# pvangoor/eqvio

Measured on AMD Instinct MI355X. Metric: EqF vision updates/sec @ N=200 landmarks, higher is better.
Workload: dtype f64; 1 GPU; synthetic 'hover' world, 200 tracked landmarks (state dim 621, 400 measurement rows), InvDepth chart, fast Riccati, IMU 200 Hz / camera 20 Hz (10 observer steps per frame), EuRoC pinhole intrinsics, one independent filter per GPU (replicas); landmarks=200, state_dim=621, parallelism=replicas x1

## Files before the change

eqvio_amd/capi.py:

```python
import ctypes as C
import os

import numpy as np

_HERE = os.path.dirname(os.path.abspath(__file__))
LIB_DIR = os.environ.get("EQVIO_AMD_LIB_DIR") or os.path.join(_HERE, "lib")

COORD_EUCLIDEAN, COORD_INVDEPTH, COORD_NORMAL = 0, 1, 2
OPT_RICCATI_DENSE, OPT_CHECK_FINITE, OPT_SIGMA_FP32, OPT_DOORBELL, OPT_SPECULATIVE, OPT_EARLY_LIFT, OPT_TRACE, OPT_FUSED_ASSEMBLY, OPT_LOOKAHEAD, OPT_LA_TIMEOUT_US, OPT_Z_IN_LOOKAHEAD, OPT_LA_SPLIT_ROWS, OPT_MEASURE_IN_PROPAGATE, OPT_LIFT_WITH_SYRK, OPT_LA_HOME, OPT_TILES_PER_WORKGROUP, OPT_GATHER_IN_PROPAGATE, OPT_HOLD_NEW_LANDMARKS, OPT_SELECT_ONE_WORKGROUP, OPT_LIVE_COLUMNS_FIRST, OPT_EARLY_DOORBELL, OPT_QUIET_DOOR_WAIT, OPT_TIMING = 1, 2, 3, 6, 7, 8, 9, 11, 12, 15, 17, 18, 19, 20, 21, 22, 23, 24, 25, 26, 27, 29, 100

c_double_p = C.POINTER(C.c_double)
c_int_p = C.POINTER(C.c_int)


class Camera(C.Structure):

    _fields_ = [
        ("model", C.c_int),
        ("width", C.c_int),
        ("height", C.c_int),
        ("fx", C.c_double),
        ("fy", C.c_double),
        ("cx", C.c_double),
        ("cy", C.c_double),
        ("dist", C.c_double * 5),
    ]

    @staticmethod
    def pinhole(fx, fy, cx, cy, width, height):
        cam = Camera()
        cam.model, cam.width, cam.height = 0, int(width), int(height)
        cam.fx, cam.fy, cam.cx, cam.cy = fx, fy, cx, cy
        return cam

    @staticmethod
    def radtan(fx, fy, cx, cy, width, height, k1, k2, p1, p2, k3=0.0):
        cam = Camera.pinhole(fx, fy, cx, cy, width, height)
        cam.model = 1
        cam.dist[:] = [k1, k2, p1, p2, k3]
        return cam

    @staticmethod
    def equidistant(fx, fy, cx, cy, width, height, k1, k2, k3, k4):
        cam = Camera.pinhole(fx, fy, cx, cy, width, height)
        cam.model = 2
        cam.dist[:] = [k1, k2, k3, k4, 0.0]
        return cam

    def project(self, p):
        out = np.zeros(2)
        _load_sim_protos().eqvio_camera_project(C.byref(self), _dp(_f64(p)), _dp(out))
        return out

    def undistort(self, y):
        out = np.zeros(3)
        _load_sim_protos().eqvio_camera_undistort(C.byref(self), _dp(_f64(y)), _dp(out))
        return out

    def jacobian(self, p):
        out = np.zeros(6)
        _load_sim_protos().eqvio_camera_jacobian(C.byref(self), _dp(_f64(p)), _dp(out))
        return out.reshape(2, 3)


_SETTINGS_DOUBLES = [
    "biasOmegaProcessVariance", "biasAccelProcessVariance", "attitudeProcessVariance", "positionProcessVariance",
    "velocityProcessVariance", "cameraAttitudeProcessVariance", "cameraPositionProcessVariance", "pointProcessVariance",
    "velGyrNoise", "velAccNoise", "velGyrBiasWalk", "velAccBiasWalk",
    "measurementNoise", "outlierThresholdAbs", "outlierThresholdProb", "featureRetention",
    "initialAttitudeVariance", "initialPositionVariance", "initialVelocityVariance", "initialCameraAttitudeVariance",
    "initialCameraPositionVariance", "initialPointVariance", "initialPointDepthVariance", "initialBiasOmegaVariance",
    "initialBiasAccelVariance", "initialSceneDepth",
]
_SETTINGS_INTS = [
    "useDiscreteInnovationLift", "useDiscreteVelocityLift", "useDiscreteStateMatrix", "fastRiccati", "useMedianDepth",
    "useFeaturePredictions", "useEquivariantOutput", "removeLostLandmarks", "coordinateChoice",
]


class Settings(C.Structure):

    _fields_ = [(n, C.c_double) for n in _SETTINGS_DOUBLES] + [(n, C.c_int) for n in _SETTINGS_INTS] + [("cameraOffset", C.c_double * 7)]

    @staticmethod
    def defaults():
        s = Settings()
        vals = dict(
            biasOmegaProcessVariance=0.001, biasAccelProcessVariance=0.001, attitudeProcessVariance=0.001, positionProcessVariance=0.001,
            velocityProcessVariance=0.001, cameraAttitudeProcessVariance=0.001, cameraPositionProcessVariance=0.001, pointProcessVariance=0.001,
            velGyrNoise=1e-4, velAccNoise=1e-3, velGyrBiasWalk=1e-5, velAccBiasWalk=1e-3,
            measurementNoise=2.0, outlierThresholdAbs=1e8, outlierThresholdProb=1e8, featureRetention=0.3,
            initialAttitudeVariance=1e-4, initialPositionVariance=1e-4, initialVelocityVariance=1e-2, initialCameraAttitudeVariance=1e-5,
            initialCameraPositionVariance=1e-4, initialPointVariance=1.0, initialPointDepthVariance=-1.0, initialBiasOmegaVariance=0.1,
            initialBiasAccelVariance=0.1, initialSceneDepth=1.0,
            useDiscreteInnovationLift=1, useDiscreteVelocityLift=1, useDiscreteStateMatrix=0, fastRiccati=0, useMedianDepth=1,
            useFeaturePredictions=0, useEquivariantOutput=1, removeLostLandmarks=1, coordinateChoice=COORD_EUCLIDEAN,
        )
        for k, v in vals.items():
            setattr(s, k, v)
        s.cameraOffset[:] = [1, 0, 0, 0, 0, 0, 0]
        return s

    def state_gain_diag8(self):
        return np.array([self.biasOmegaProcessVariance, self.biasAccelProcessVariance, self.attitudeProcessVariance, self.positionProcessVariance,
                         self.velocityProcessVariance, self.cameraAttitudeProcessVariance, self.cameraPositionProcessVariance, self.pointProcessVariance])

    def input_gain_diag12(self):
        v = [self.velGyrNoise**2, self.velAccNoise**2, self.velGyrBiasWalk**2, self.velAccBiasWalk**2]
        return np.repeat(np.array(v), 3)

    def initial_cov_diag(self, N):
        v = [self.initialBiasOmegaVariance, self.initialBiasAccelVariance, self.initialAttitudeVariance, self.initialPositionVariance,
             self.initialVelocityVariance, self.initialCameraAttitudeVariance, self.initialCameraPositionVariance]
        d = np.concatenate([np.repeat(np.array(v), 3), np.full(3 * N, self.initialPointVariance)])
        if self.initialPointDepthVariance > 0:
            d[21 + 2::3] = self.initialPointDepthVariance
        return d


def _dp(a):
    return a.ctypes.data_as(c_double_p)


def _ip(a):
    return a.ctypes.data_as(c_int_p)


def _f64(a):
    return np.ascontiguousarray(a, dtype=np.float64)


def _i32(a):
    return np.ascontiguousarray(a, dtype=np.int32)


class EqfError(RuntimeError):
    def __init__(self, code, msg):
        super().__init__(f"eqf_hip error {code}: {msg}")
        self.code = code


_lib = None


def load_eqf_lib():
    global _lib
    if _lib is not None:
        return _lib
    path = os.path.join(LIB_DIR, "libeqf_hip.so")
    if not os.path.exists(path):
        raise RuntimeError(f"{path} not found: run `python -c 'import __graft_entry__ as g; g.build()'` — the EqF path has no CPU fallback")
    lib = C.CDLL(path)
    vp = C.c_void_p
    P = C.POINTER
    protos = {
        "eqf_error_string": (C.c_char_p, [C.c_int]),
        "eqf_kernel_name": (C.c_char_p, [C.c_int]),
        "eqf_create": (C.c_int, [P(vp), C.c_int, C.c_int, C.c_int]),
        "eqf_destroy": (None, [vp]),
        "eqf_set_option": (C.c_int, [vp, C.c_int, C.c_int]),
        "eqf_get_option": (C.c_int, [vp, C.c_int, C.POINTER(C.c_int)]),
        "eqf_lookahead_selftest": (C.c_int, [vp]),
        "eqf_lookahead_home": (C.c_int, [vp, C.POINTER(C.c_int), C.POINTER(C.c_long)]),
        "eqf_device_to_itself": (C.c_int, [vp]),
        "eqf_early_doorbell_stats": (C.c_int, [vp, C.POINTER(C.c_long), C.c_int]),
        "eqf_synchronize": (C.c_int, [vp]),
        "eqf_num_landmarks": (C.c_int, [vp]),
        "eqf_get_ids": (C.c_int, [vp, c_int_p, C.c_int]),
        "eqf_stream": (vp, [vp]),
        "eqf_set_state": (C.c_int, [vp, c_double_p, c_double_p, c_int_p, c_double_p, c_double_p, C.c_int]),
        "eqf_get_state": (C.c_int, [vp, c_double_p, c_double_p, c_int_p, c_double_p, c_double_p, C.c_int]),
        "eqf_set_sigma": (C.c_int, [vp, c_double_p, C.c_int]),
        "eqf_set_sigma_diag": (C.c_int, [vp, c_double_p, C.c_int]),
        "eqf_get_sigma": (C.c_int, [vp, c_double_p, C.c_int]),
        "eqf_get_sigma_block": (C.c_int, [vp, C.c_int, C.c_int, C.c_int, C.c_int, c_double_p]),
        "eqf_state_estimate": (C.c_int, [vp, c_double_p, c_int_p, c_double_p, C.c_int]),
        "eqf_add_landmarks": (C.c_int, [vp, c_int_p, c_double_p, C.c_int, C.c_double]),
        "eqf_remove_landmarks": (C.c_int, [vp, c_int_p, C.c_int]),
        "eqf_remove_unmeasured_landmarks": (C.c_int, [vp, c_int_p, C.c_int, c_int_p, c_int_p]),
        "eqf_find_unknown_ids": (C.c_int, [vp, c_int_p, C.c_int, c_int_p, c_int_p]),
        "eqf_same_as_mapped": (C.c_int, [vp, c_int_p, C.c_int]),
        "eqf_update_unsettled": (C.c_int, [vp]),
        "eqf_remove_invalid_at_update": (C.c_int, [vp]),
        "eqf_add_landmarks_held": (C.c_int, [vp, c_int_p, c_double_p, C.c_int, C.c_double]),
        "eqf_hold_supported": (C.c_int, [vp]),
        "eqf_hold_stats": (C.c_int, [vp, C.POINTER(C.c_long), C.c_int]),
        "eqf_live_columns_stats": (C.c_int, [vp, C.POINTER(C.c_long), C.c_int]),
        "eqf_own_hardware_queue": (C.c_int, [vp]),
        "eqf_remove_invalid_landmarks": (C.c_int, [vp]),
        "eqf_integrate_riccati_fast": (C.c_int, [vp, c_double_p, C.c_double, c_double_p, c_double_p]),
        "eqf_integrate_riccati_accurate": (C.c_int, [vp, c_double_p, C.c_double, c_double_p, c_double_p]),
        "eqf_integrate_riccati_discrete": (C.c_int, [vp, c_double_p, C.c_double, c_double_p, c_double_p]),
        "eqf_integrate_observer": (C.c_int, [vp, c_double_p, c_double_p, C.c_int, C.c_int]),
        "eqf_outlier_stats": (C.c_int, [vp, P(Camera), c_int_p, c_double_p, C.c_int, c_double_p, c_double_p, c_double_p]),
        "eqf_propagate_fast": (C.c_int, [vp, c_double_p, C.c_double, c_double_p, c_double_p, c_double_p, c_double_p, C.c_int, C.c_int]),
        "eqf_stage_measurement": (C.c_int, [vp, c_int_p, c_double_p, C.c_int]),
        "eqf_trace_read": (C.c_int, [vp, C.POINTER(C.c_ulonglong), C.POINTER(C.c_longlong), C.POINTER(C.c_uint)]),
        "eqf_host_wait_stats": (C.c_int, [vp, C.POINTER(C.c_long), c_double_p, C.c_int]),
        "eqf_stats_then_update": (C.c_int, [vp, C.POINTER(Camera), c_int_p, c_double_p, C.c_int, C.c_double, C.c_double, C.c_double, C.c_int, C.c_int, c_double_p, c_double_p,
                                  c_double_p, c_int_p]),
        "eqf_stats_select_update": (C.c_int, [vp, C.POINTER(Camera), c_int_p, c_double_p, C.c_int, C.c_double, C.c_double, C.c_int, C.c_double, C.c_int, C.c_int, c_double_p,
                                    c_double_p, c_double_p, c_int_p, c_int_p, c_int_p]),
        "eqf_vision_update": (C.c_int, [vp, P(Camera), c_int_p, c_double_p, C.c_int, C.c_double, C.c_int, C.c_int]),
        "eqf_last_gamma": (C.c_int, [vp, c_double_p, C.c_int]),
        "eqf_compute_nees": (C.c_int, [vp, c_double_p, c_int_p, c_double_p, C.c_int, c_double_p]),
        "eqf_nees_lu_fallbacks": (C.c_int, [vp, C.POINTER(C.c_long)]),
        "eqf_speculation_stats": (C.c_int, [vp, C.POINTER(C.c_long), C.POINTER(C.c_long), C.POINTER(C.c_long), C.c_int]),
        "eqf_measure_in_propagate_stats": (C.c_int, [vp, C.POINTER(C.c_long), C.c_int]),
        "eqf_z_in_lookahead_stats": (C.c_int, [vp, C.POINTER(C.c_long), C.c_int]),
        "eqf_gather_stats": (C.c_int, [vp, C.POINTER(C.c_long), C.c_int]),
        "eqf_selection_stats": (C.c_int, [vp, C.POINTER(C.c_long), C.POINTER(C.c_long), C.c_int]),
        "eqf_output_cov_all": (C.c_int, [vp, P(Camera), c_double_p]),
        "eqf_lookahead_stats": (C.c_int, [vp, C.POINTER(C.c_long), C.POINTER(C.c_long), C.c_int]),
        "eqf_debug_matrices_AB": (C.c_int, [vp, c_double_p, c_double_p, c_double_p]),
        "eqf_debug_get_W": (C.c_int, [vp, c_double_p, C.c_int, C.c_int]),
        "eqf_debug_syrk_order": (C.c_int, [C.c_int, c_int_p]),
        "eqf_debug_lookahead_stamps": (C.c_int, [vp, C.POINTER(C.c_ulonglong)]),
        "eqf_debug_matrix_C": (C.c_int, [vp, P(Camera), c_int_p, c_double_p, C.c_int, C.c_int, c_double_p, c_double_p]),
        "eqf_mfma_f64_peak": (C.c_int, [vp, c_double_p]),
        "eqf_mfma_f64_peak_clock": (C.c_int, [vp, C.POINTER(C.c_double), C.POINTER(C.c_double)]),
        "eqf_last_kernel_times": (C.c_int, [vp, c_int_p, P(C.c_float), C.c_int]),
    }
    for name, (res, args) in protos.items():
        if os.environ.get("EQVIO_AMD_LIB_DIR") and name in ("eqf_lookahead_home", "eqf_device_to_itself", "eqf_early_doorbell_stats", "eqf_update_unsettled", "eqf_remove_invalid_at_update", "eqf_gather_stats", "eqf_remove_unmeasured_landmarks", "eqf_find_unknown_ids", "eqf_add_landmarks_held", "eqf_hold_supported", "eqf_hold_stats", "eqf_same_as_mapped", "eqf_live_columns_stats", "eqf_own_hardware_queue") and not hasattr(lib, name):
            continue
        fn = getattr(lib, name)
        fn.restype = res
        fn.argtypes = args
    lib._declared = sorted(protos)
    _lib = lib
    return lib


class EqfCore:

    def __init__(self, max_landmarks, coordinate_choice=COORD_EUCLIDEAN, device=0):
        self.lib = load_eqf_lib()
        self.h = C.c_void_p()
        self._chk0(self.lib.eqf_create(C.byref(self.h), device, max_landmarks, coordinate_choice))
        self._cap0 = max_landmarks + 16

    def _chk0(self, rc):
        if rc != 0:
            raise EqfError(rc, self.lib.eqf_error_string(rc).decode())

    def close(self):
        if self.h:
            self.lib.eqf_destroy(self.h)
            self.h = C.c_void_p()

    def __del__(self):
        try:
            self.close()
        except Exception:
            pass

    @property
    def N(self):
        return self.lib.eqf_num_landmarks(self.h)

    @property
    def n(self):
        return 21 + 3 * self.N

    @property
    def cap(self):
        return max(self._cap0, self.N + 16)

    def set_option(self, opt, val):
        self._chk0(self.lib.eqf_set_option(self.h, opt, val))

    def get_option(self, opt):
        v = C.c_int()
        self._chk0(self.lib.eqf_get_option(self.h, opt, C.byref(v)))
        return v.value

    def lookahead_selftest(self):
        return self.lib.eqf_lookahead_selftest(self.h)

    def synchronize(self):
        self._chk0(self.lib.eqf_synchronize(self.h))

    def stream(self):
        return self.lib.eqf_stream(self.h)

    def set_state(self, xi0_sensor, X_sensor, ids, q0, Q):
        xi0_sensor, X_sensor, ids, q0, Q = _f64(xi0_sensor), _f64(X_sensor), _i32(ids), _f64(q0), _f64(Q)
        self._chk0(self.lib.eqf_set_state(self.h, _dp(xi0_sensor), _dp(X_sensor), _ip(ids), _dp(q0), _dp(Q), len(ids)))

    def get_state(self):
        xi0, Xs = np.zeros(23), np.zeros(23)
        ids, q0, Q = np.zeros(self.cap, np.int32), np.zeros(3 * self.cap), np.zeros(5 * self.cap)
        N = self.lib.eqf_get_state(self.h, _dp(xi0), _dp(Xs), _ip(ids), _dp(q0), _dp(Q), self.cap)
        if N < 0:
            self._chk0(N)
        return xi0, Xs, ids[:N].copy(), q0[: 3 * N].reshape(N, 3).copy(), Q[: 5 * N].reshape(N, 5).copy()

    def set_sigma(self, S):
        S = np.asfortranarray(S, dtype=np.float64)
        self._chk0(self.lib.eqf_set_sigma(self.h, S.ctypes.data_as(c_double_p), S.shape[0]))

    def set_sigma_diag(self, d):
        d = _f64(d)
        self._chk0(self.lib.eqf_set_sigma_diag(self.h, _dp(d), len(d)))

    def get_sigma(self):
        n = self.n
        out = np.zeros((n, n), order="F")
        self._chk0(self.lib.eqf_get_sigma(self.h, out.ctypes.data_as(c_double_p), n))
        return out

    def get_sigma_block(self, r0, c0, rows, cols):
        out = np.zeros((rows, cols), order="F")
        self._chk0(self.lib.eqf_get_sigma_block(self.h, r0, c0, rows, cols, out.ctypes.data_as(c_double_p)))
        return out

    def state_estimate(self):
        s = np.zeros(23)
        ids, p = np.zeros(self.cap, np.int32), np.zeros(3 * self.cap)
        N = self.lib.eqf_state_estimate(self.h, _dp(s), _ip(ids), _dp(p), self.cap)
        if N < 0:
            self._chk0(N)
        return s, ids[:N].copy(), p[: 3 * N].reshape(N, 3).copy()

    def add_landmarks(self, ids, p, var):
        ids, p = _i32(ids), _f64(p)
        self._chk0(self.lib.eqf_add_landmarks(self.h, _ip(ids), _dp(p), len(ids), var))

    def add_landmarks_held(self, ids, p, var):
        ids, p = _i32(ids), _f64(p)
        rc = self.lib.eqf_add_landmarks_held(self.h, _ip(ids), _dp(p), len(ids), var)
        if rc == -6:
            return False
        self._chk0(rc)
        return True

    def remove_landmarks(self, indices):
        indices = _i32(indices)
        self._chk0(self.lib.eqf_remove_landmarks(self.h, _ip(indices), len(indices)))

    def remove_invalid_landmarks(self):
        rc = self.lib.eqf_remove_invalid_landmarks(self.h)
        if rc < 0:
            self._chk0(rc)
        return rc

    def integrate_riccati_fast(self, imu13, dt, Qdiag12, Pdiag8):
        imu13, Qd, Pd = _f64(imu13), _f64(Qdiag12), _f64(Pdiag8)
        self._chk0(self.lib.eqf_integrate_riccati_fast(self.h, _dp(imu13), dt, _dp(Qd), _dp(Pd)))

    def integrate_riccati_accurate(self, imu13, dt, Qdiag12, Pdiag8):
        imu13, Qd, Pd = _f64(imu13), _f64(Qdiag12), _f64(Pdiag8)
        self._chk0(self.lib.eqf_integrate_riccati_accurate(self.h, _dp(imu13), dt, _dp(Qd), _dp(Pd)))

    def integrate_riccati_discrete(self, imu13, dt, Qdiag12, Pdiag8):
        imu13, Qdiag12, Pdiag8 = _f64(imu13), _f64(Qdiag12), _f64(Pdiag8)
        self._chk0(self.lib.eqf_integrate_riccati_discrete(self.h, _dp(imu13), dt, _dp(Qdiag12), _dp(Pdiag8)))

    def integrate_observer(self, imu13_k, dt_k, discrete=True):
        imu13_k, dt_k = _f64(imu13_k).reshape(-1, 13), _f64(dt_k).reshape(-1)
        self._chk0(self.lib.eqf_integrate_observer(self.h, _dp(imu13_k), _dp(dt_k), len(dt_k), int(discrete)))

    def outlier_stats(self, cam, ids, y):
        ids, y = _i32(ids), _f64(y)
        N = self.N
        a, p, d = np.zeros(N), np.zeros(N), np.zeros(N)
        self._chk0(self.lib.eqf_outlier_stats(self.h, C.byref(cam), _ip(ids), _dp(y), len(ids), _dp(a), _dp(p), _dp(d)))
        return a, p, d

    def output_cov_all(self, cam):
        out = np.zeros(4 * self.N)
        self._chk0(self.lib.eqf_output_cov_all(self.h, C.byref(cam), _dp(out)))
        return out.reshape(self.N, 2, 2)

    def vision_update(self, cam, ids, y, meas_var, use_equivariant=True, discrete=False):
        ids, y = _i32(ids), _f64(y)
        self._chk0(self.lib.eqf_vision_update(self.h, C.byref(cam), _ip(ids), _dp(y), len(ids), meas_var, int(use_equivariant), int(discrete)))
# ... 402 lines not shown
```

eqvio_amd/csrc/eqf_hip.hip:

```cpp
#include "eqf_hip.h"
#include "eqf_kernels.hpp"
#include "eqf_lookahead.hpp"
#include "eqf_batch.hpp"
#include "eqf_batch.h"
#include "host_prof.hpp"
#include <algorithm>
#include <atomic>
#include <chrono>
#include <condition_variable>
#include <mutex>
#include <cstdio>
#include <cstdlib>
#include <cstring>
#include <string>
#include <vector>
#include <unistd.h>
#include <fcntl.h>
#include <signal.h>
#include <sys/mman.h>
#include <cerrno>

using namespace eqf;

namespace {
// ... 5 lines not shown
    KN_PROP_MAIN,
    KN_MEASURE,
    KN_STATS,
    KN_BUILD_Z,
    KN_CHOL_PANEL,
    KN_CHOL_UPDATE,
    KN_GAMMA,
    KN_SYRK,
    KN_LIFT,
    KN_DENSE_GEMM,
    KN_MISC,
    KN_CHOL_LOOKAHEAD,
    KN_COUNT
};
const char* kNames[KN_COUNT] = {"k_assemble_AB", "k_observer",    "k_propagate_G", "k_propagate_main", "k_measure", "k_outlier_stats", "k_build_Z",
                                "k_chol_step",   "k_chol_first", "k_gamma",       "k_syrk_sub",       "k_lift",    "k_gemm_nt",       "misc", "k_chol_lookahead"};

int roundup(int x, int m) { return (x + m - 1) / m * m; }
int pick_ld(int x) {
    int ld = roundup(x, 16);
    if (ld % 128 == 0)
        ld += 16;
    return ld;
}

struct SensorState {
    V3 bgyr, bacc;
    Pose pose;
    V3 vel;
    Pose cam;
};
struct GroupSensor {
    V3 bgyr, bacc;
    Pose A;
    V3 w;
    Pose B;
};
SensorState unpack_sensor(const double* s) {
    SensorState r;
    r.bgyr = v3(s[0], s[1], s[2]);
    r.bacc = v3(s[3], s[4], s[5]);
    r.pose = Pose{Qt{s[6], s[7], s[8], s[9]}, v3(s[10], s[11], s[12])};
    r.vel = v3(s[13], s[14], s[15]);
    r.cam = Pose{Qt{s[16], s[17], s[18], s[19]}, v3(s[20], s[21], s[22])};
    return r;
}
void pack_pose(const Pose& p, double* q, double* x) {
    q[0] = p.R.w;
    q[1] = p.R.x;
    q[2] = p.R.y;
    q[3] = p.R.z;
    x[0] = p.x.x;
    x[1] = p.x.y;
    x[2] = p.x.z;
}
void pack_v3(V3 v, double* d) {
    d[0] = v.x;
    d[1] = v.y;
    d[2] = v.z;
}
void pack_sensor(const SensorState& r, double* s) {
    pack_v3(r.bgyr, s);
    pack_v3(r.bacc, s + 3);
    pack_pose(r.pose, s + 6, s + 10);
    pack_v3(r.vel, s + 13);
    pack_pose(r.cam, s + 16, s + 20);
}
GroupSensor unpack_group(const double* s) {
    GroupSensor g;
    g.bgyr = v3(s[0], s[1], s[2]);
    g.bacc = v3(s[3], s[4], s[5]);
    g.A = Pose{Qt{s[6], s[7], s[8], s[9]}, v3(s[10], s[11], s[12])};
    g.w = v3(s[13], s[14], s[15]);
    g.B = Pose{Qt{s[16], s[17], s[18], s[19]}, v3(s[20], s[21], s[22])};
    return g;
}
void pack_group(const GroupSensor& g, double* s) {
    pack_v3(g.bgyr, s);
    pack_v3(g.bacc, s + 3);
    pack_pose(g.A, s + 6, s + 10);
    pack_v3(g.w, s + 13);
    pack_pose(g.B, s + 16, s + 20);
}
SensorState sensor_action(const GroupSensor& X, const SensorState& s) {
    SensorState r;
    r.bgyr = s.bgyr + X.bgyr;
    r.bacc = s.bacc + X.bacc;
    r.pose = pose_mul(s.pose, X.A);
    r.vel = q_rot(q_inv(X.A.R), s.vel - X.w);
    r.cam = pose_mul(pose_mul(pose_inv(X.A), s.cam), X.B);
    return r;
}
GroupSensor group_mul(const GroupSensor& a, const GroupSensor& b) {
    GroupSensor r;
    r.bgyr = a.bgyr + b.bgyr;
    r.bacc = a.bacc + b.bacc;
    r.A = pose_mul(a.A, b.A);
    r.B = pose_mul(a.B, b.B);
    r.w = a.w + q_rot(a.A.R, b.w);
    return r;
}

}

struct eqf_ctx {
    int device = 0;
    hipStream_t stream = nullptr;
    hipStream_t stream2 = nullptr;
    hipEvent_t ev_assembled = nullptr, ev_observer = nullptr, ev_early = nullptr;
    bool ev_assembled_early = false;
    bool obs_pending = false;
    bool busy_common = false, busy_steps = false, busy_meas = false;
    int chart = 0;
    int Ncap = 0, ncap = 0, ld = 0;
    int mcap = 0, ldz = 0;
    int N = 0;
    std::vector<int> ids;
    SensorState xi0;
    GroupSensor X;
    double* d_st[2] = {nullptr, nullptr};
    double* d_lm[2] = {nullptr, nullptr};
    int stcur = 0, lmcur = 0;
    double* d_sigma[2] = {nullptr, nullptr};
    int cur = 0;
    double *d_Al = nullptr, *d_Bl = nullptr;
    Common* d_common = nullptr;
    ObsStep* d_steps = nullptr;
    double *d_C = nullptr, *d_ytil = nullptr, *d_y = nullptr;
    int *d_lmidx = nullptr, *d_measof = nullptr;
    double *d_Ebuf = nullptr, *d_Yl = nullptr, *d_Fl = nullptr, *d_PhiB = nullptr;
    int* d_expinfo = nullptr;
    double *d_Zn = nullptr, *d_Wn = nullptr;
    double* d_pub = nullptr;
    int* d_pubf = nullptr;
    int* d_pubfl = nullptr;
    int la_home = 0;
    long la_home_refused = 0;
    int opt_la_home = 1;
    long la_home_launches = 0;
    bool la_home_force = false;
    int reg_slot = -1;
    unsigned reg_checks = 0;
    char* d_puby = nullptr;
    int la_njcap = 0, la_seq = 0;
    unsigned long long* d_ladbg = nullptr;
    int opt_lookahead = 1;
    int opt_zb = 1;
    int opt_zb_large = 1;
    int opt_la_split = 1;
    int opt_prop_tpw = 1;
    int opt_gather = 1;
    int opt_early_door = 1;
    int opt_quiet_wait = 1;
    int opt_la_watch_ahead = 1;
    int early_seq_next = 0, early_armed_seq = 0;
    bool early_allowed = false;
    long early_rings = 0;
    bool unsettled = false, unsettled_wait = false;
    int settle_seq = 0, settle_N = 0;
    unsigned settle_gen = 0, settle_epoch = 0, est_epoch = 0;
    std::vector<int> settle_ids;
    std::vector<int> invalid_ids;
    int opt_hold = 1;
    int opt_sel_one = 1;
    int opt_live_first = 1;
    const int* la_live_cols = nullptr;
    long live_first_launches = 0;
    int n_held = 0;
    double held_var = 0.0;
    bool held_in_memory = false;
    double* h_held = nullptr;
    bool held_busy = false;
    long held_launches = 0;
    long gather_launches = 0;
    int opt_measure_prop = 1;
    int opt_lift_syrk = 1;
    bool pred_valid = false, me_valid = false;
    Cam pred_cam{}, me_cam{};
    int pred_star = 0, me_star = 0, me_M = 0;
    unsigned long me_gen = 0;
    long me_used = 0;
    bool obs_one_chunk = false;
    bool tail_zb = false;
    double tail_var = 0.0;
    long zb_launches = 0;
    int cu_count = 256;
    long la_book_timeouts = 0;
    std::vector<char> rm_drop;
    std::vector<int> rm_ids, rm_map;
    std::vector<double> rm_est;
    bool own_queue = false;
    bool counted_alive = false;
    int la_cus_held = 0;
    int la_selftest = 0;
    long long la_timeout_ticks = LA_TIMEOUT_TICKS;
    long la_launches = 0, la_fallbacks = 0;
    int la_consecutive_stalls = 0;
    int tail_M = 0;
    bool tail_la = false;
    int* d_perm = nullptr;
    static constexpr int kRing = 8;
    int ring_pos = 0;
    int ring_inflight = 0;
    bool reshape_pending = false;
    int dev_N = 0;
    std::vector<int> pend_map;
    std::vector<double> pend_p;
    std::vector<double> pend_var;
    char* h_rs_ring = nullptr;
    char* d_rs = nullptr;
    size_t rs_bytes = 0;
    int spec_backoff = 0, spec_backoff_len = 0;
    long spec_calls = 0, spec_queued = 0, spec_cancelled = 0;
    long nees_lu_fallbacks = 0;
    int ldzn = 0;
    double *d_Z = nullptr, *d_W = nullptr, *d_Linv = nullptr, *d_gamma = nullptr, *d_gpart = nullptr, *d_est = nullptr, *d_stats = nullptr, *d_scratch = nullptr, *d_F = nullptr, *d_tmp = nullptr;
    int* d_flags = nullptr;
    int* d_syrk_order = nullptr;
    std::vector<int> syrk_off;
    Common* h_common = nullptr;
    ObsStep* h_steps = nullptr;
    double* h_buf = nullptr;
    bool ocov_valid = false;
    Cam ocov_cam{};
    bool ocov_hint_valid = false;
    Cam ocov_hint{};
    size_t hbuf_doubles = 0;
    int* h_ibuf = nullptr;
    int* h_flags = nullptr;
    int* h_lmidx = nullptr;
    double* h_y = nullptr;
    double* h_ylm = nullptr;
    double* d_meas = nullptr;
    int* d_meas_idx = nullptr;
    bool stage_requested = false, stage_pending = false, staged_valid = false;
    int staged_M = 0;
    unsigned lm_gen = 0, staged_gen = 0;
    std::vector<int> staged_ids;
    std::vector<double> staged_y;
    std::vector<int> map_ids;
    unsigned map_gen = ~0u;
    int map_N = -1;
    bool map_all = false;
    bool map_ident = false;
    bool tail_ident = false;
    std::vector<std::pair<int, int>> lookup;
    std::vector<int> renum_scratch;
    unsigned lookup_gen = ~0u;
    trace_t* d_trace = nullptr;
    unsigned trace_frame = 0;
    std::vector<long long> h_trace;
    long wait_calls = 0, launch_calls = 0;
    double wait_seconds = 0.0, launch_seconds = 0.0;
    double* h_res = nullptr;
    double* h_ocov = nullptr;
    int* h_resflags = nullptr;
    int* h_sel = nullptr;
    long sel_frames = 0, sel_discarded = 0;
    static constexpr int kMaxSteps = kObsChunk;
    CommonK ck;
    int opt_dense = 0, opt_check = 0, opt_timing = 0, opt_f32 = 0, opt_early = 1, opt_fuse_asm = 1;
    bool sig32 = false;
    int opt_door = 1;
    int* d_door = nullptr;
    int* h_door = nullptr;
    unsigned door_seq = 0;
    int opt_spec = 1;
    int* d_spec = nullptr;
    std::vector<double> last_gamma;
    int n_at_update = 0;
    bool gamma_stale = false;
    std::vector<double> est_cache;
    bool est_valid = false;
    bool meas_valid = false;
    int meas_star = 0;
    std::vector<int> meas_ids;
    std::vector<std::pair<int, std::pair<hipEvent_t, hipEvent_t>>> tev;
    std::vector<int> tev_n;
    std::vector<hipEvent_t> evpool;
    size_t evused = 0;

    double* q0() { return d_st[stcur]; }
    double* Qq() { return d_lm[lmcur]; }
    double* Qa() { return d_lm[lmcur] + 4 * (size_t)Ncap; }
    double* sigma() { return d_sigma[cur]; }
    int n() const { return 21 + 3 * N; }
};

#define HIPCHK(expr)                                                                                   \
    do {                                                                                               \
        hipError_t _e = (expr);                                                                        \
        if (_e != hipSuccess) {                                                                        \
            std::fprintf(stderr, "[eqf_hip] %s failed: %s (%s:%d)\n", #expr, hipGetErrorString(_e), __FILE__, __LINE__); \
            return (int)_e;                                                                            \
        }                                                                                              \
    } while (0)

namespace {

hipEvent_t get_event(eqf_ctx* c) {
    if (c->evused == c->evpool.size()) {
        hipEvent_t e;
        hipEventCreate(&e);
        c->evpool.push_back(e);
    }
    return c->evpool[c->evused++];
}
constexpr int TR_FRAMES = 1024, TR_SLOTS = 48;
enum { TR_ASSEMBLE = 0, TR_PROPAGATE = 1, TR_BUILD_Z = 2, TR_STEP0 = 3, TR_LIFT = 40, TR_SYRK = 42 };
constexpr int TR_HOST = 8;
enum { TH_DOOR = 0, TH_PROP_ENTRY = 1, TH_ASSEMBLE_OUT = 2, TH_PROP_OUT = 3, TH_TAIL_ENTRY = 4, TH_BUILD_Z_OUT = 5, TH_TAIL_OUT = 6 };
void host_stamp(eqf_ctx* c, int k) {
    if (c->d_trace)
        c->h_trace[(size_t)(c->trace_frame % TR_FRAMES) * TR_HOST + k] = std::chrono::duration_cast<std::chrono::nanoseconds>(std::chrono::steady_clock::now().time_since_epoch()).count();
}
trace_t* trace_slot(eqf_ctx* c, int slot) { return c->d_trace ? c->d_trace + (size_t)(c->trace_frame % TR_FRAMES) * TR_SLOTS + slot : nullptr; }
struct KTimer {
    eqf_ctx* c;
    int which;
    hipEvent_t e0 = nullptr, e1 = nullptr;
    std::chrono::steady_clock::time_point h0;
    int nlaunch;
    bool on() const { return c->opt_timing == 1 || (c->opt_timing == 2 && (which == KN_CHOL_LOOKAHEAD || which == KN_CHOL_PANEL || which == KN_CHOL_UPDATE)); }
    KTimer(eqf_ctx* ctx, int w, int n = 1) : c(ctx), which(w), h0(std::chrono::steady_clock::now()), nlaunch(n) {
        if (on()) {
            e0 = get_event(c);
            e1 = get_event(c);
            hipEventRecord(e0, c->stream);
        }
    }
    ~KTimer() {
        if (on()) {
            hipEventRecord(e1, c->stream);
            c->tev.push_back({which, {e0, e1}});
            c->tev_n.push_back(nlaunch);
        }
        c->launch_calls += nlaunch - 1;
        ++c->launch_calls;
        c->launch_seconds += std::chrono::duration<double>(std::chrono::steady_clock::now() - h0).count();
    }
};
void timing_reset(eqf_ctx* c) {
    c->tev.clear();
    c->tev_n.clear();
    c->evused = 0;
}

int blocks(int n, int b) { return (n + b - 1) / b; }

int spin_stream(hipStream_t st) {
    for (;;) {
        const hipError_t e = hipStreamQuery(st);
        if (e == hipSuccess)
            return 0;
        if (e != hipErrorNotReady) {
            std::fprintf(stderr, "[eqf_hip] stream error: %s\n", hipGetErrorString(e));
            return (int)e;
        }
    }
}
namespace {
std::atomic<int> ctx_alive[64];
thread_local bool replaces_own_queue = false;
std::mutex la_gate_mutex;
std::condition_variable la_gate_cv;
int la_cus_booked[64] = {0};
}
namespace {
constexpr int REG_SLOTS = 64;
struct DeviceRegistry {
    std::atomic<int> pid[REG_SLOTS];
};
DeviceRegistry* registry_of(int device) {
    static std::mutex mu;
    static DeviceRegistry* maps[64] = {};
    std::lock_guard<std::mutex> g(mu);
    DeviceRegistry*& r = maps[device & 63];
    if (r)
        return r;
    char name[96];
    std::snprintf(name, sizeof(name), "/eqf_hip_contexts_u%u_d%d", (unsigned)getuid(), device);
    const int fd = shm_open(name, O_CREAT | O_RDWR, 0600);
    if (fd < 0)
        return nullptr;
    if (ftruncate(fd, sizeof(DeviceRegistry)) != 0) {
        close(fd);
        return nullptr;
    }
    void* p = mmap(nullptr, sizeof(DeviceRegistry), PROT_READ | PROT_WRITE, MAP_SHARED, fd, 0);
    close(fd);
    if (p == MAP_FAILED)
        return nullptr;
    r = static_cast<DeviceRegistry*>(p);
    return r;
}
bool pid_alive(int pid) { return pid > 0 && (kill(pid, 0) == 0 || errno == EPERM); }
}
static void registry_enter(eqf_ctx* c) {
    DeviceRegistry* r = registry_of(c->device);
    c->reg_slot = -1;
    if (!r)
        return;
    const int me = (int)getpid();
    for (int pass = 0; pass < 2 && c->reg_slot < 0; ++pass)
        for (int i = 0; i < REG_SLOTS && c->reg_slot < 0; ++i) {
            int cur = r->pid[i].load(std::memory_order_relaxed);
            if (cur != 0 && (pass == 0 || pid_alive(cur)))
                continue;
            if (r->pid[i].compare_exchange_strong(cur, me))
                c->reg_slot = i;
        }
}
static void registry_leave(eqf_ctx* c) {
    DeviceRegistry* r = c->reg_slot >= 0 ? registry_of(c->device) : nullptr;
    if (r)
        r->pid[c->reg_slot].store(0, std::memory_order_relaxed);
    c->reg_slot = -1;
}
static bool device_to_itself(eqf_ctx* c) {
    DeviceRegistry* r = c->reg_slot >= 0 ? registry_of(c->device) : nullptr;
    if (!r)
        return false;
    int others = 0;
    for (int i = 0; i < REG_SLOTS; ++i)
        others += (i != c->reg_slot && r->pid[i].load(std::memory_order_relaxed) != 0) ? 1 : 0;
    if (others == 0)
        return true;
    if ((++c->reg_checks & 0xfff) == 1) {
        for (int i = 0; i < REG_SLOTS; ++i) {
            int cur = r->pid[i].load(std::memory_order_relaxed);
            if (i != c->reg_slot && cur != 0 && cur != (int)getpid() && !pid_alive(cur))
                r->pid[i].compare_exchange_strong(cur, 0);
        }
    }
    return false;
}
static void la_release(eqf_ctx* c) {
    if (!c->la_cus_held)
        return;
    {
        std::lock_guard<std::mutex> g(la_gate_mutex);
        la_cus_booked[c->device & 63] -= c->la_cus_held;
    }
    c->la_cus_held = 0;
    la_gate_cv.notify_all();
}
static bool la_book(eqf_ctx* c, int workgroups) {
    la_release(c);
    std::unique_lock<std::mutex> g(la_gate_mutex);
    int& booked = la_cus_booked[c->device & 63];
    const auto bound = std::chrono::microseconds(std::max<long>(2000, 2 * (long)(c->la_timeout_ticks / 100)));
    if (!la_gate_cv.wait_for(g, bound, [&] { return booked == 0 || booked + workgroups <= c->cu_count; }))
        return false;
    booked += workgroups;
    c->la_cus_held = workgroups;
    return true;
}
struct LaBookingGuard {
    eqf_ctx* c;
    bool keep = false;
    ~LaBookingGuard() {
        if (!keep)
            la_release(c);
    }
};
int sync_ctx(eqf_ctx* c) {
    {
        int r = spin_stream(c->stream);
        if (r)
            return r;
    }
    if (c->obs_pending) {
        int r = spin_stream(c->stream2);
        if (r)
            return r;
        c->obs_pending = false;
    }
    c->busy_common = c->busy_steps = c->busy_meas = false;
    c->ring_inflight = 0;
    c->held_busy = false;
    la_release(c);
    return 0;
}
int door_wait(eqf_ctx* c, int which, int seq, bool* early = nullptr) {
    HP_SCOPE("abi.door_wait");
    volatile int* bell = reinterpret_cast<volatile int*>(c->h_door) + which;
    long spins_after_done = 0;
    const auto t0 = std::chrono::steady_clock::now();
    constexpr auto kQuietWait = std::chrono::milliseconds(2);
    volatile int* bell_early = (which == 1 && early && c->early_armed_seq == seq) ? reinterpret_cast<volatile int*>(c->h_door) + 3 : nullptr;
    if (early)
        *early = false;
    for (long it = 1;; ++it) {
        const bool rang_early = bell_early && *bell_early == seq && *bell != seq;
        if (rang_early)
            *early = true;
        if (*bell == seq || rang_early) {
            std::atomic_thread_fence(std::memory_order_acquire);
            c->busy_common = c->busy_steps = c->busy_meas = false;
            c->ring_inflight = 0;
            c->held_busy = false;
            if (!(which == 1 && c->unsettled_wait))
                ++c->wait_calls;
            c->wait_seconds += std::chrono::duration<double>(std::chrono::steady_clock::now() - t0).count();
            if (which == 1) {
                if (!c->unsettled_wait)
                    host_stamp(c, TH_DOOR);
                la_release(c);
            }
            return 0;
        }
        if (spins_after_done || ((it & 0xfff) == 0 && (!c->opt_quiet_wait || std::chrono::steady_clock::now() - t0 >= kQuietWait))) {
            const hipError_t e = hipStreamQuery(c->stream);
            if (e == hipSuccess) {
                if (++spins_after_done > 1000000) {
                    std::fprintf(stderr, "[eqf_hip] doorbell %d never rang (expected %d, have %d)\n", which, seq, (int)*bell);
                    la_release(c);
                    return (int)hipErrorUnknown;
                }
            } else if (e != hipErrorNotReady) {
                std::fprintf(stderr, "[eqf_hip] stream error: %s\n", hipGetErrorString(e));
                la_release(c);
                return (int)e;
            }
        }
    }
}
int join_observer(eqf_ctx* c) {
    c->ev_assembled_early = false;
    if (c->obs_pending) {
        HIPCHK(hipStreamWaitEvent(c->stream, c->ev_observer, 0));
        c->obs_pending = false;
    }
    return 0;
}

Cam make_cam(const eqvio_camera* c) {
    Cam k{c->fx, c->fy, c->cx, c->cy};
    k.model = c->model;
    for (int i = 0; i < 5; ++i)
        k.d[i] = c->dist[i];
    return k;
}
bool camera_ok(const eqvio_camera* c) { return c->model >= EQVIO_CAMERA_PINHOLE && c->model <= EQVIO_CAMERA_EQUIDISTANT; }

void compute_common_at(const GroupSensor& X, const SensorState& xi0, const double* imu13, Common& cm, CommonK& ck) {
    const SensorState xh = sensor_action(X, xi0);
    const V3 gyr = v3(imu13[1], imu13[2], imu13[3]) - xh.bgyr;
    const V6 U_I{gyr, xh.vel};
    const M3 R_A = q_mat(X.A.R);
    const M3 R_IC = q_mat(xh.cam.R);
    const M3 RTic = transpose(R_IC);
    auto put = [](const M3& A, double* d) {
        const double a[9] = {A.a00, A.a01, A.a02, A.a10, A.a11, A.a12, A.a20, A.a21, A.a22};
        std::memcpy(d, a, sizeof(a));
    };
    put(RTic * transpose(R_A), cm.Mv);
    put(RTic, cm.RTic);
    put(RTic * skew(xh.cam.x), cm.RTicSx);
    const V6 U1 = Ad_apply(pose_inv(xi0.cam), Ad_apply(X.A, U_I));
    const M6 adT = se3_adjoint(U1);
    const M6 CT = m6_mul(se3_Adjoint(pose_inv(X.B)), adT);
    std::memcpy(cm.CT, CT.a, sizeof(cm.CT));
    const V6 U_C = Ad_apply(pose_inv(xh.cam), U_I);
    pack_v3(U_C.v, cm.vC);
    std::memset(cm.Bs, 0, sizeof(cm.Bs));
    auto setB = [&](int r0, int c0, const M3& A) {
        const double a[9] = {A.a00, A.a01, A.a02, A.a10, A.a11, A.a12, A.a20, A.a21, A.a22};
        for (int i = 0; i < 3; ++i)
            for (int j = 0; j < 3; ++j)
                cm.Bs[(r0 + i) * 12 + c0 + j] = a[3 * i + j];
    };
    for (int i = 0; i < 6; ++i)
        cm.Bs[i * 12 + 6 + i] = 1.0;
    setB(6, 0, R_A);
    setB(9, 0, skew(X.A.x) * R_A);
    setB(12, 0, R_A * skew(xh.vel));
    setB(12, 3, R_A);
    std::memset(cm.Ass, 0, sizeof(cm.Ass));
    for (int r = 0; r < 21; ++r)
        for (int cc = 0; cc < 6; ++cc)
            cm.Ass[r * 21 + cc] = -cm.Bs[r * 12 + cc];
    for (int i = 0; i < 3; ++i)
        cm.Ass[(9 + i) * 21 + 12 + i] = 1.0;
    const V3 gdir = q_rot(q_inv(xi0.pose.R), v3(0, 0, 1));
    const M3 Gs = (-kGravity) * skew(gdir);
    const double g[9] = {Gs.a00, Gs.a01, Gs.a02, Gs.a10, Gs.a11, Gs.a12, Gs.a20, Gs.a21, Gs.a22};
    for (int i = 0; i < 3; ++i)
        for (int j = 0; j < 3; ++j)
            cm.Ass[(12 + i) * 21 + 6 + j] = g[3 * i + j];
    for (int i = 0; i < 6; ++i)
        for (int j = 0; j < 6; ++j)
            cm.Ass[(15 + i) * 21 + 15 + j] = adT.a[i * 6 + j];
    std::memcpy(ck.lm, cm.Mv, sizeof(double) * 66);
    put(R_A, ck.RA);
    put(skew(X.A.x) * R_A, ck.SxRA);
    put(R_A * skew(xh.vel), ck.RAsv);
    std::memcpy(ck.G, g, sizeof(g));
    std::memcpy(ck.adT, adT.a, sizeof(ck.adT));
}

void compute_common(const eqf_ctx* c, const double* imu13, Common& cm) { compute_common_at(c->X, c->xi0, imu13, cm, const_cast<eqf_ctx*>(c)->ck); }

int upload_common(eqf_ctx* c, const double* imu13) {
    compute_common(c, imu13, *c->h_common);
    return 0;
}
int launch_assemble(eqf_ctx* c, bool record_early = true) {
    KTimer t(c, KN_ASSEMBLE);
    int r = join_observer(c);
    if (r)
        return r;
    hipLaunchKernelGGL(k_assemble_AB, dim3(std::max(1, blocks(c->N, 64))), dim3(64), 0, c->stream, c->ck, c->N, c->Ncap, c->chart, c->d_common, c->q0(), c->Qq(),
                       c->Qa(), c->d_Al, c->d_Bl, trace_slot(c, TR_ASSEMBLE));
    if (record_early) {
        HIPCHK(hipEventRecord(c->ev_early, c->stream));
        c->ev_assembled_early = true;
    }
    return (int)hipGetLastError();
}
int keep_last_gamma(eqf_ctx* c) {
    if (!c->gamma_stale)
        return 0;
    const int ng = c->n_at_update;
    HIPCHK(hipMemcpyAsync(c->h_buf, c->d_gamma, sizeof(double) * ng, hipMemcpyDeviceToHost, c->stream));
    { int _r = sync_ctx(c); if (_r) return _r; }
    c->last_gamma.assign(c->h_buf, c->h_buf + ng);
    c->gamma_stale = false;
    return 0;
}
int read_flags(eqf_ctx* c) {
    HIPCHK(hipMemcpyAsync(c->h_flags, c->d_flags, 4 * sizeof(int), hipMemcpyDeviceToHost, c->stream));
    { int _r = sync_ctx(c); if (_r) return _r; }
    return 0;
}
void ensure_lookup(eqf_ctx* c) {
    if (c->lookup_gen != c->lm_gen || (int)c->lookup.size() != c->N) {
        c->lookup.resize(c->N);
        for (int i = 0; i < c->N; ++i)
            c->lookup[i] = {c->ids[i], i};
        std::sort(c->lookup.begin(), c->lookup.end());
        c->lookup_gen = c->lm_gen;
    }
}
int index_of(eqf_ctx* c, int id) {
    ensure_lookup(c);
    const auto it = std::lower_bound(c->lookup.begin(), c->lookup.end(), std::make_pair(id, -1));
    return (it != c->lookup.end() && it->first == id) ? it->second : -1;
}
// ... 258 lines not shown
            ctx_alive[c->device & 63].fetch_sub(1);
        c->counted_alive = false;
    }
    if (c && std::getenv("EQF_DEBUG_STATS"))
        std::fprintf(stderr, "[eqf_hip] look-ahead launches %ld (stalled %ld), of them with Z built inside %ld\n", c->la_launches, c->la_fallbacks, c->zb_launches);
    if (c && std::getenv("EQF_DEBUG_STATS") && c->early_rings)
        std::fprintf(stderr, "[eqf_hip] updates taken from the early doorbell: %ld\n", c->early_rings);
    if (!c)
        return;
    hipSetDevice(c->device);
    if (c->stream)
        hipStreamSynchronize(c->stream);
    if (c->stream2)
        hipStreamSynchronize(c->stream2);
    for (int b = 0; b < 2; ++b) {
        hipFree(c->d_sigma[b]);
        hipFree(c->d_lm[b]);
        hipFree(c->d_st[b]);
    }
    hipFree(c->d_Al);
    hipFree(c->d_Bl);
    hipFree(c->d_common);
    hipFree(c->d_steps);
    hipFree(c->d_C);
    hipFree(c->d_ytil);
    hipFree(c->d_y);
    hipFree(c->d_lmidx);
    hipFree(c->d_measof);
    hipFree(c->d_Z);
    hipFree(c->d_W);
    hipFree(c->d_Linv);
    hipFree(c->d_gamma);
    hipFree(c->d_gpart);
    hipFree(c->d_pub);
    hipFree(c->d_pubf);
    hipFree(c->d_pubfl);
    hipFree(c->d_puby);
    if (c->d_ladbg)
        hipFree(c->d_ladbg);
    if (c->d_trace)
        hipFree(c->d_trace);
    hipFree(c->d_est);
    hipFree(c->d_stats);
    hipFree(c->d_scratch);
    hipFree(c->d_flags);
    hipFree(c->d_syrk_order);
    if (c->d_Ebuf) {
        hipFree(c->d_Ebuf);
        hipFree(c->d_Yl);
        hipFree(c->d_Fl);
        hipFree(c->d_PhiB);
        hipFree(c->d_expinfo);
    }
    if (c->d_Zn)
        hipFree(c->d_Zn);
    if (c->d_Wn)
        hipFree(c->d_Wn);
    if (c->d_perm)
        hipFree(c->d_perm);
    if (c->d_F)
        hipFree(c->d_F);
    if (c->d_tmp)
        hipFree(c->d_tmp);
    hipHostFree(c->h_common);
    hipHostFree(c->h_steps);
    hipHostFree(c->h_buf);
    hipHostFree(c->h_ibuf);
    hipHostFree(c->h_rs_ring);
    hipFree(c->d_rs);
    hipHostFree(c->h_flags);
    hipHostFree(c->h_lmidx);
    hipHostFree(c->h_y);
    hipHostFree(c->h_ylm);
    hipFree(c->d_meas);
    hipFree(c->d_meas_idx);
    hipHostFree(c->h_res);
    if (c->h_ocov)
        hipHostFree(c->h_ocov);
    c->h_ocov = nullptr;
    hipHostFree(c->h_resflags);
    hipHostFree(c->h_sel);
    hipHostFree(c->h_held);
    hipHostFree(c->h_door);
    hipFree(c->d_door);
    hipFree(c->d_spec);
    if (c->ev_assembled)
        hipEventDestroy(c->ev_assembled);
    if (c->ev_observer)
        hipEventDestroy(c->ev_observer);
    if (c->ev_early)
        hipEventDestroy(c->ev_early);
    if (c->stream2)
        hipStreamDestroy(c->stream2);
    for (auto e : c->evpool)
        hipEventDestroy(e);
    if (c->stream)
        hipStreamDestroy(c->stream);
    delete c;
}

#define LAUNCH_TS(c, KERNEL, grid, block, stream, ...)                                                        \
    do {                                                                                                      \
        if ((c)->sig32) {                                                                                     \
            using TS = float;                                                                                 \
            hipLaunchKernelGGL(HIP_KERNEL_NAME(KERNEL<TS>), grid, block, 0, stream, __VA_ARGS__);             \
        } else {                                                                                              \
            using TS = double;                                                                                \
            hipLaunchKernelGGL(HIP_KERNEL_NAME(KERNEL<TS>), grid, block, 0, stream, __VA_ARGS__);             \
        }                                                                                                     \
    } while (0)

static int set_sigma_storage(eqf_ctx* c, bool f32) {
    if (c->sig32 == f32)
        return 0;
    const int n = c->n();
    double* in = c->d_sigma[c->cur];
    double* out = c->d_sigma[1 - c->cur];
    if (f32)
        hipLaunchKernelGGL(HIP_KERNEL_NAME(k_convert_sigma<double, float>), dim3(blocks(n, 256), n), dim3(256), 0, c->stream, n, c->ld, in, (float*)out);
    else
        hipLaunchKernelGGL(HIP_KERNEL_NAME(k_convert_sigma<float, double>), dim3(blocks(n, 256), n), dim3(256), 0, c->stream, n, c->ld, (const float*)in, out);
    HIPCHK(hipGetLastError());
    c->cur = 1 - c->cur;
    c->sig32 = f32;
    return 0;
}

static int round_sigma(eqf_ctx* c, const int* spec, int spec_seq) {
    if ((c->opt_f32 != 1 && c->opt_f32 != 3) || c->n() == 0)
        return 0;
    const int n = c->n();
    hipLaunchKernelGGL(k_round_f32, dim3(blocks(n, 256), n), dim3(256), 0, c->stream, n, c->ld, c->sigma(), spec, spec_seq, c->opt_f32 == 3 ? 1 : 0);
    HIPCHK(hipGetLastError());
    return 0;
}

int eqf_get_option(const eqf_ctx* c, int option, int* value) {
    if (!c || !value)
        return EQF_E_BAD_ARG;
    switch (option) {
    case EQF_OPT_RICCATI_DENSE: *value = c->opt_dense; return 0;
    case EQF_OPT_CHECK_FINITE: *value = c->opt_check; return 0;
    case EQF_OPT_SPECULATIVE: *value = c->opt_spec; return 0;
    case EQF_OPT_DOORBELL: *value = c->opt_door; return 0;
    case EQF_OPT_EARLY_LIFT: *value = c->opt_early; return 0;
    case EQF_OPT_FUSED_ASSEMBLY: *value = c->opt_fuse_asm; return 0;
    case EQF_OPT_Z_IN_LOOKAHEAD: *value = c->opt_zb ? (c->opt_zb_large ? 1 : 2) : 0; return 0;
    case EQF_OPT_LA_SPLIT_ROWS: *value = c->opt_la_split; return 0;
    case EQF_OPT_TILES_PER_WORKGROUP: *value = c->opt_prop_tpw; return 0;
    case EQF_OPT_GATHER_IN_PROPAGATE: *value = c->opt_gather; return 0;
    case EQF_OPT_HOLD_NEW_LANDMARKS: *value = c->opt_hold; return 0;
    case EQF_OPT_EARLY_DOORBELL: *value = c->opt_early_door; return 0;
    case EQF_OPT_QUIET_DOOR_WAIT: *value = c->opt_quiet_wait; return 0;
    case EQF_OPT_SELECT_ONE_WORKGROUP: *value = c->opt_sel_one; return 0;
    case EQF_OPT_LIVE_COLUMNS_FIRST: *value = c->opt_live_first; return 0;
    case EQF_OPT_LA_HOME: *value = c->opt_la_home; return 0;
    case EQF_OPT_MEASURE_IN_PROPAGATE: *value = c->opt_measure_prop; return 0;
    case EQF_OPT_LIFT_WITH_SYRK: *value = c->opt_lift_syrk; return 0;
    case EQF_OPT_LOOKAHEAD: *value = c->opt_lookahead; return 0;
    case EQF_OPT_LA_TIMEOUT_US: *value = (int)(c->la_timeout_ticks / 100); return 0;
    case EQF_OPT_TRACE: *value = c->d_trace ? 1 : 0; return 0;
    case EQF_OPT_SIGMA_FP32: *value = c->opt_f32; return 0;
    case 100: *value = c->opt_timing; return 0;
    case 102: *value = c->opt_la_watch_ahead; return 0;
    default: return EQF_E_BAD_ARG;
    }
}
int eqf_set_option(eqf_ctx* c, int option, int value) {
    if (!c)
        return EQF_E_BAD_ARG;
    switch (option) {
    case EQF_OPT_RICCATI_DENSE:
        if (value && c->sig32)
            return EQF_E_UNSUPPORTED;
        c->opt_dense = value;
        return 0;
    case EQF_OPT_CHECK_FINITE:
        c->opt_check = value;
        return 0;
    case EQF_OPT_SPECULATIVE:
        c->opt_spec = value;
        return 0;
    case EQF_OPT_DOORBELL:
        c->opt_door = value;
        return 0;
    case EQF_OPT_EARLY_LIFT:
        c->opt_early = value;
        return 0;
    case EQF_OPT_FUSED_ASSEMBLY:
        c->opt_fuse_asm = value;
        return 0;
    case EQF_OPT_Z_IN_LOOKAHEAD:
        c->opt_zb = value ? 1 : 0, c->opt_zb_large = value == 2 ? 0 : 1;
        return 0;
    case EQF_OPT_LA_SPLIT_ROWS:
        c->opt_la_split = value ? 1 : 0;
        return 0;
    case EQF_OPT_LA_HOME:
        c->opt_la_home = value < 0 ? 0 : std::min(value, 2);
        return 0;
    case EQF_OPT_TILES_PER_WORKGROUP:
        if (value < 0 || value > 8)
            return EQF_E_BAD_ARG;
        c->opt_prop_tpw = value;
        return 0;
    case EQF_OPT_GATHER_IN_PROPAGATE:
        c->opt_gather = value ? 1 : 0;
        return 0;
    case EQF_OPT_HOLD_NEW_LANDMARKS:
        c->opt_hold = value ? 1 : 0;
        return 0;
    case EQF_OPT_SELECT_ONE_WORKGROUP:
        c->opt_sel_one = value ? 1 : 0;
        return 0;
    case EQF_OPT_LIVE_COLUMNS_FIRST:
        c->opt_live_first = value ? 1 : 0;
        return 0;
    case EQF_OPT_EARLY_DOORBELL:
        c->opt_early_door = value ? 1 : 0;
        return 0;
    case EQF_OPT_QUIET_DOOR_WAIT:
        c->opt_quiet_wait = value ? 1 : 0;
        return 0;
    case EQF_OPT_MEASURE_IN_PROPAGATE:
        c->opt_measure_prop = value ? 1 : 0;
        c->me_valid = false;
        return 0;
    case EQF_OPT_LIFT_WITH_SYRK:
        c->opt_lift_syrk = value ? 1 : 0;
        return 0;
    case EQF_OPT_LOOKAHEAD:
        c->opt_lookahead = value;
        c->la_consecutive_stalls = 0;
        return 0;
    case EQF_OPT_LA_TIMEOUT_US:
        if (value < 0)
            return EQF_E_BAD_ARG;
        c->la_timeout_ticks = 100ll * value;
        return 0;
    case EQF_OPT_TRACE: {
        { int _r = sync_ctx(c); if (_r) return _r; }
        if (value && !c->d_trace) {
            HIPCHK(hipMalloc(&c->d_trace, sizeof(trace_t) * TR_FRAMES * TR_SLOTS));
            HIPCHK(hipMemset(c->d_trace, 0, sizeof(trace_t) * TR_FRAMES * TR_SLOTS));
            if (!c->d_ladbg) {
                HIPCHK(hipMalloc(&c->d_ladbg, 96 * 8 * sizeof(unsigned long long)));
                HIPCHK(hipMemset(c->d_ladbg, 0, 96 * 8 * sizeof(unsigned long long)));
            }
            c->h_trace.assign((size_t)TR_FRAMES * TR_HOST, 0);
        } else if (!value && c->d_trace) {
            hipFree(c->d_trace);
            c->d_trace = nullptr;
        }
        return 0;
    }
    case EQF_OPT_SIGMA_FP32: {
        if (value < 0 || value > 3)
            return EQF_E_BAD_ARG;
        if (value == 2 && c->opt_dense)
            return EQF_E_UNSUPPORTED;
        c->opt_f32 = value;
        { int _e = enter(c); if (_e) return _e; }
        const int rc = set_sigma_storage(c, value == 2);
        return rc ? rc : round_sigma(c);
    }
    case 100:
        c->opt_timing = value;
        timing_reset(c);
        return 0;
    case 102:
        c->opt_la_watch_ahead = value ? 1 : 0;
        return 0;
    default:
        return EQF_E_BAD_ARG;
    }
}
int eqf_synchronize(eqf_ctx* c) {
    if (!c)
        return EQF_E_BAD_ARG;
    { int _r = settle_update(c); if (_r) return _r; }
    { int _r = sync_ctx(c); if (_r) return _r; }
    return 0;
}
int eqf_num_landmarks(const eqf_ctx* c) { return c->N; }
int eqf_get_ids(const eqf_ctx* c, int* ids, int cap) {
    if (!c || (!ids && c->N > 0))
        return EQF_E_BAD_ARG;
    if (c->N > cap)
        return EQF_E_CAPACITY;
    for (int i = 0; i < c->N; ++i)
        ids[i] = c->ids[i];
    return c->N;
}
void* eqf_stream(eqf_ctx* c) { return (void*)c->stream; }

int eqf_set_state(eqf_ctx* c, const double* xi0_sensor, const double* X_sensor, const int* ids, const double* q0, const double* Q, int N) {
    if (!c || N < 0 || (N > 0 && (!ids || !q0 || !Q)))
        return EQF_E_BAD_ARG;
    { int _e = enter(c); if (_e) return _e; }
    if (N > c->Ncap) {
        const int rc = grow_capacity(c, std::max(N, 2 * c->Ncap));
        if (rc)
            return rc;
    }
    { int _r = sync_ctx(c); if (_r) return _r; }
    c->est_valid = false, ++c->est_epoch;
    c->meas_valid = false;
    c->n_held = 0, c->held_in_memory = false;
    c->xi0 = unpack_sensor(xi0_sensor);
    c->X = unpack_group(X_sensor);
    c->ids.assign(ids, ids + N);
    c->N = N;
    c->dev_N = N;
    ++c->lm_gen;
    if (N > 0) {
        std::memcpy(c->h_buf, q0, sizeof(double) * 3 * N);
        std::memcpy(c->h_buf + 3 * N, Q, sizeof(double) * 5 * N);
        HIPCHK(hipMemcpyAsync(c->d_scratch, c->h_buf, sizeof(double) * 8 * N, hipMemcpyHostToDevice, c->stream));
        hipLaunchKernelGGL(k_scatter_landmarks, dim3(blocks(N, 64)), dim3(64), 0, c->stream, N, 0, c->Ncap, c->d_scratch, c->d_scratch + 3 * N, c->q0(), c->Qq(),
                           c->Qa());
        HIPCHK(hipGetLastError());
        { int _r = sync_ctx(c); if (_r) return _r; }
    }
    return 0;
}

int eqf_get_state(eqf_ctx* c, double* xi0_sensor, double* X_sensor, int* ids, double* q0, double* Q, int cap) {
    if (!c)
        return EQF_E_BAD_ARG;
    if (xi0_sensor)
        pack_sensor(c->xi0, xi0_sensor);
    if (X_sensor)
        pack_group(c->X, X_sensor);
    const int N = c->N;
    if (N > cap)
        return EQF_E_CAPACITY;
    if (N > 0) {
        { int _e = enter(c); if (_e) return _e; }
        { int _r = join_observer(c); if (_r) return _r; }
        hipLaunchKernelGGL(k_gather_landmarks_aos, dim3(blocks(N, 64)), dim3(64), 0, c->stream, N, c->Ncap, c->q0(), c->Qq(), c->Qa(), c->d_scratch);
        HIPCHK(hipGetLastError());
        HIPCHK(hipMemcpyAsync(c->h_buf, c->d_scratch, sizeof(double) * 8 * N, hipMemcpyDeviceToHost, c->stream));
        { int _r = sync_ctx(c); if (_r) return _r; }
        for (int i = 0; i < N; ++i) {
            if (ids)
                ids[i] = c->ids[i];
            if (q0)
                std::memcpy(q0 + 3 * i, c->h_buf + 8 * i, sizeof(double) * 3);
            if (Q)
                std::memcpy(Q + 5 * i, c->h_buf + 8 * i + 3, sizeof(double) * 5);
        }
    }
    return N;
}

int eqf_set_sigma(eqf_ctx* c, const double* sig, int n) {
    if (!c || !sig || n != c->n())
        return EQF_E_BAD_ARG;
    { int _e = enter(c); if (_e) return _e; }
    { int _r = sync_ctx(c); if (_r) return _r; }
    std::memcpy(c->h_buf, sig, sizeof(double) * (size_t)n * n);
    if (c->sig32) {
        double* stage = c->d_sigma[1 - c->cur];
        HIPCHK(hipMemcpy2DAsync(stage, sizeof(double) * c->ld, c->h_buf, sizeof(double) * n, sizeof(double) * n, n, hipMemcpyHostToDevice, c->stream));
        hipLaunchKernelGGL(HIP_KERNEL_NAME(k_convert_sigma<double, float>), dim3(blocks(n, 256), n), dim3(256), 0, c->stream, n, c->ld, stage, (float*)c->sigma());
        HIPCHK(hipGetLastError());
    } else {
        HIPCHK(hipMemcpy2DAsync(c->sigma(), sizeof(double) * c->ld, c->h_buf, sizeof(double) * n, sizeof(double) * n, n, hipMemcpyHostToDevice, c->stream));
    }
    { int _r = round_sigma(c); if (_r) return _r; }
    { int _r = sync_ctx(c); if (_r) return _r; }
    return 0;
}
int eqf_set_sigma_diag(eqf_ctx* c, const double* diag, int n) {
    if (!c || !diag || n != c->n())
        return EQF_E_BAD_ARG;
    { int _e = enter(c); if (_e) return _e; }
    { int _r = sync_ctx(c); if (_r) return _r; }
    { int _r = keep_last_gamma(c); if (_r) return _r; }
    std::memcpy(c->h_buf, diag, sizeof(double) * n);
    HIPCHK(hipMemcpyAsync(c->d_gamma, c->h_buf, sizeof(double) * n, hipMemcpyHostToDevice, c->stream));
    LAUNCH_TS(c, k_set_diag, dim3(blocks(n, 256), n), dim3(256), c->stream, n, c->ld, c->d_gamma, (TS*)c->sigma());
    HIPCHK(hipGetLastError());
    { int _r = round_sigma(c); if (_r) return _r; }
    { int _r = sync_ctx(c); if (_r) return _r; }
    return 0;
}
int eqf_get_sigma_block(eqf_ctx* c, int r0, int c0, int rows, int cols, double* out) {
    if (!c || !out || r0 < 0 || c0 < 0 || rows < 0 || cols < 0 || r0 + rows > c->n() || c0 + cols > c->n())
        return EQF_E_BAD_ARG;
    if (rows == 0 || cols == 0)
        return 0;
    { int _e = enter(c); if (_e) return _e; }
    const double* src = c->sigma();
    if (c->sig32) {
        const int n = c->n();
        double* stage = c->d_sigma[1 - c->cur];
        hipLaunchKernelGGL(HIP_KERNEL_NAME(k_convert_sigma<float, double>), dim3(blocks(n, 256), n), dim3(256), 0, c->stream, n, c->ld, (const float*)c->sigma(), stage);
        HIPCHK(hipGetLastError());
        src = stage;
    }
    HIPCHK(hipMemcpy2DAsync(c->h_buf, sizeof(double) * rows, src + r0 + (size_t)c0 * c->ld, sizeof(double) * c->ld, sizeof(double) * rows, cols,
                            hipMemcpyDeviceToHost, c->stream));
    { int _r = sync_ctx(c); if (_r) return _r; }
    std::memcpy(out, c->h_buf, sizeof(double) * (size_t)rows * cols);
    return 0;
}
int eqf_get_sigma(eqf_ctx* c, double* sig, int n) {
    if (!c || n != c->n())
        return EQF_E_BAD_ARG;
    return eqf_get_sigma_block(c, 0, 0, n, n, sig);
}

static int fetch_estimates(eqf_ctx* c) {
    { int _r = settle_update(c); if (_r) return _r; }
    const int N = c->N;
    if (N == 0)
        return 0;
    if (c->est_valid && (int)c->est_cache.size() == 4 * N) {
        std::memcpy(c->h_buf, c->est_cache.data(), sizeof(double) * 4 * N);
        return 0;
    }
    { int _e = enter(c); if (_e) return _e; }
    { int _r = join_observer(c); if (_r) return _r; }
    const bool with_ocov = c->ocov_hint_valid && !c->sig32;
    const bool use_door = c->opt_door && !c->opt_check && !c->obs_pending;
    const int door_seq = use_door ? (int)(++c->door_seq) : 0;
    int* const dcount = use_door ? c->d_door + 2 : nullptr;
    hipLaunchKernelGGL(k_estimate, dim3(blocks(N, 64)), dim3(64), 0, c->stream, N, c->Ncap, c->q0(), c->Qq(), c->Qa(), c->h_buf, with_ocov ? (int*)nullptr : dcount, c->h_door + 2, door_seq);
    HIPCHK(hipGetLastError());
    if (with_ocov) {
        if (!c->h_ocov)
            HIPCHK(hipHostMalloc(&c->h_ocov, sizeof(double) * 4 * (size_t)c->Ncap));
        hipLaunchKernelGGL(HIP_KERNEL_NAME(k_output_cov<double>), dim3(blocks(N, 64)), dim3(64), 0, c->stream, N, c->Ncap, c->ld, c->chart, c->ocov_hint, c->q0(), c->Qq(), c->Qa(),
                           (const double*)c->sigma(), c->h_ocov, dcount, c->h_door + 2, door_seq);
        HIPCHK(hipGetLastError());
    }
    { int _r = use_door ? door_wait(c, 2, door_seq) : sync_ctx(c); if (_r) return _r; }
    if (with_ocov)
        c->ocov_valid = true, c->ocov_cam = c->ocov_hint;
    return 0;
}

int eqf_state_estimate(eqf_ctx* c, double* sensor, int* ids, double* p, int cap) {
    if (!c)
        return EQF_E_BAD_ARG;
    if (sensor)
        pack_sensor(sensor_action(c->X, c->xi0), sensor);
    const int N = c->N;
    if (N > cap)
        return EQF_E_CAPACITY;
    if (N > 0 && (ids || p)) {
        HIPCHK(hipSetDevice(c->device));
        int rc = fetch_estimates(c);
        if (rc)
            return rc;
        for (int i = 0; i < N; ++i) {
            if (ids)
                ids[i] = c->ids[i];
            if (p) {
                p[3 * i] = c->h_buf[i];
                p[3 * i + 1] = c->h_buf[N + i];
                p[3 * i + 2] = c->h_buf[2 * N + i];
            }
        }
    }
    return N;
}

static int grow_capacity(eqf_ctx* c, int new_cap) {
    int rc = keep_last_gamma(c);
    if (rc)
        return rc;
    const int N = c->N, n = c->n();
    double xi0s[23], Xs[23];
    std::vector<int> ids(std::max(N, 1));
    std::vector<double> q0(3 * (size_t)std::max(N, 1)), Q(5 * (size_t)std::max(N, 1)), S((size_t)n * n);
    rc = eqf_get_state(c, xi0s, Xs, ids.data(), q0.data(), Q.data(), std::max(N, 1));
    if (rc < 0)
        return rc;
    rc = eqf_get_sigma(c, S.data(), n);
    if (rc)
        return rc;
    eqf_ctx* t = nullptr;
    replaces_own_queue = c->own_queue;
    rc = eqf_create(&t, c->device, new_cap, c->chart);
    replaces_own_queue = false;
    if (rc)
        return rc == EQF_E_NO_DEVICE ? rc : EQF_E_CAPACITY;
    const int opts[][2] = {{EQF_OPT_SIGMA_FP32, c->opt_f32}, {EQF_OPT_RICCATI_DENSE, c->opt_dense}, {EQF_OPT_CHECK_FINITE, c->opt_check}, {EQF_OPT_SPECULATIVE, c->opt_spec},
                           {EQF_OPT_DOORBELL, c->opt_door}, {EQF_OPT_EARLY_LIFT, c->opt_early}, {EQF_OPT_FUSED_ASSEMBLY, c->opt_fuse_asm}, {EQF_OPT_LOOKAHEAD, c->opt_lookahead},
                           {EQF_OPT_LA_TIMEOUT_US, (int)(c->la_timeout_ticks / 100)}, {EQF_OPT_Z_IN_LOOKAHEAD, c->opt_zb ? (c->opt_zb_large ? 1 : 2) : 0}, {EQF_OPT_LA_SPLIT_ROWS, c->opt_la_split}, {EQF_OPT_LA_HOME, c->opt_la_home}, {EQF_OPT_TILES_PER_WORKGROUP, c->opt_prop_tpw}, {EQF_OPT_GATHER_IN_PROPAGATE, c->opt_gather}, {EQF_OPT_HOLD_NEW_LANDMARKS, c->opt_hold}, {EQF_OPT_EARLY_DOORBELL, c->opt_early_door}, {EQF_OPT_QUIET_DOOR_WAIT, c->opt_quiet_wait}, {EQF_OPT_SELECT_ONE_WORKGROUP, c->opt_sel_one}, {EQF_OPT_LIVE_COLUMNS_FIRST, c->opt_live_first}, {EQF_OPT_MEASURE_IN_PROPAGATE, c->opt_measure_prop}, {EQF_OPT_LIFT_WITH_SYRK, c->opt_lift_syrk}, {EQF_OPT_TRACE, c->d_trace ? 1 : 0}, {100, c->opt_timing}};
    for (const auto& o : opts)
        if ((rc = eqf_set_option(t, o[0], o[1])) != 0)
            break;
    if (!rc)
        rc = eqf_set_state(t, xi0s, Xs, ids.data(), q0.data(), Q.data(), N);
    if (!rc)
        rc = eqf_set_sigma(t, S.data(), n);
    if (rc) {
        eqf_destroy(t);
        return rc;
    }
    t->last_gamma = c->last_gamma, t->n_at_update = c->n_at_update;
    t->spec_calls = c->spec_calls, t->spec_queued = c->spec_queued, t->spec_cancelled = c->spec_cancelled, t->spec_backoff = c->spec_backoff, t->spec_backoff_len = c->spec_backoff_len;
    t->nees_lu_fallbacks = c->nees_lu_fallbacks, t->wait_calls = c->wait_calls, t->launch_calls = c->launch_calls, t->wait_seconds = c->wait_seconds, t->launch_seconds = c->launch_seconds;
    t->la_launches = c->la_launches, t->la_fallbacks = c->la_fallbacks, t->la_home_launches = c->la_home_launches, t->la_home_refused = c->la_home_refused, t->la_book_timeouts = c->la_book_timeouts, t->zb_launches = c->zb_launches, t->la_consecutive_stalls = c->la_consecutive_stalls, t->early_rings = c->early_rings;
    t->la_selftest = c->la_selftest < 0 ? -1 : (t->la_selftest != 0 ? t->la_selftest : c->la_selftest);
    t->me_used = c->me_used, t->pred_valid = c->pred_valid, t->pred_cam = c->pred_cam, t->pred_star = c->pred_star;
    t->n_held = c->n_held, t->held_var = c->held_var, t->held_in_memory = c->n_held > 0;
    t->lm_gen = c->lm_gen + 1;
    std::swap(*c, *t);
    eqf_destroy(t);
    return 0;
}

static void pend_begin(eqf_ctx* c) {
    if (!c->reshape_pending) {
        c->pend_map.resize(c->dev_N);
        for (int i = 0; i < c->dev_N; ++i)
            c->pend_map[i] = i;
        c->pend_p.clear();
        c->pend_var.clear();
        c->reshape_pending = true;
    }
}
static void materialise_held(eqf_ctx* c) {
    if (c->n_held == 0 || c->held_in_memory)
        return;
    pend_begin(c);
    for (int t = 0; t < c->n_held; ++t) {
        c->pend_map.push_back(-((int)c->pend_var.size() + 1));
        c->pend_p.insert(c->pend_p.end(), c->h_held + 1 + 3 * t, c->h_held + 4 + 3 * t);
        c->pend_var.push_back(c->held_var);
    }
    c->held_in_memory = true;
}
static int flush_reshape(eqf_ctx* c) {
    if (!c->reshape_pending)
        return 0;
    HP_SCOPE("abi.flush_reshape");
    const int Nnew = (int)c->pend_map.size(), knew = (int)c->pend_var.size();
    bool identity = knew == 0 && Nnew == c->dev_N;
    for (int i = 0; identity && i < Nnew; ++i)
        identity = c->pend_map[i] == i;
    if (identity) {
        c->reshape_pending = false;
        return 0;
    }
    { int _r = join_observer(c); if (_r) return _r; }
    bool pure_append = knew > 0 && knew <= APPEND_MAX && Nnew - knew == c->dev_N;
    for (int i = 0; pure_append && i < Nnew; ++i)
        pure_append = c->pend_map[i] == (i < c->dev_N ? i : -(i - c->dev_N + 1));
    if (pure_append) {
        AppendArgs aa;
        for (int t = 0; t < knew; ++t) {
            aa.p[t][0] = c->pend_p[3 * t], aa.p[t][1] = c->pend_p[3 * t + 1], aa.p[t][2] = c->pend_p[3 * t + 2];
            aa.var[t] = c->pend_var[t];
        }
        {
            KTimer t(c, KN_MISC);
            const int nn = 21 + 3 * Nnew;
            LAUNCH_TS(c, k_append_inplace, dim3(blocks(nn, 256), 3 * knew + 1), dim3(256), c->stream, c->dev_N, knew, c->Ncap, c->ld, aa, (TS*)c->sigma(), c->d_st[c->stcur], c->d_lm[c->lmcur]);
            HIPCHK(hipGetLastError());
        }
        c->dev_N = Nnew;
        c->reshape_pending = false;
        return round_sigma(c);
    }
    if (Nnew <= RESHAPE_ARG_MAP && knew <= RESHAPE_ARG_NEW && c->Ncap < 32768) {
        ReshapeArgs ra;
        for (int i = 0; i < Nnew; ++i)
            ra.map[i] = (short)c->pend_map[i];
        for (int t = 0; t < knew; ++t) {
            ra.p[3 * t] = c->pend_p[3 * t], ra.p[3 * t + 1] = c->pend_p[3 * t + 1], ra.p[3 * t + 2] = c->pend_p[3 * t + 2];
            ra.var[t] = c->pend_var[t];
        }
        const int nnew = 21 + 3 * Nnew;
        {
            KTimer t(c, KN_MISC);
            LAUNCH_TS(c, k_reshape_args, dim3(blocks(nnew, 256), nnew + blocks(Nnew, 256)), dim3(256), c->stream, Nnew, c->Ncap, c->ld, ra, (const TS*)c->d_sigma[c->cur],
                      (TS*)c->d_sigma[1 - c->cur], (const double*)c->d_st[c->stcur], (const double*)c->d_lm[c->lmcur], c->d_st[1 - c->stcur], c->d_lm[1 - c->lmcur]);
            HIPCHK(hipGetLastError());
        }
        c->cur = 1 - c->cur;
        c->lmcur = 1 - c->lmcur;
        c->stcur = 1 - c->stcur;
        c->dev_N = Nnew;
        c->reshape_pending = false;
        return knew ? round_sigma(c) : 0;
    }
    if (c->ring_inflight >= eqf_ctx::kRing) {
        const int r = sync_ctx(c);
        if (r)
            return r;
    }
    ++c->ring_inflight;
    char* slot = c->h_rs_ring + (size_t)(c->ring_pos++ % eqf_ctx::kRing) * c->rs_bytes;
    const size_t off_p = (sizeof(int) * (size_t)c->Ncap + 15) & ~(size_t)15, off_v = off_p + sizeof(double) * 3 * (size_t)c->Ncap;
    std::memcpy(slot, c->pend_map.data(), sizeof(int) * Nnew);
    if (knew) {
        std::memcpy(slot + off_p, c->pend_p.data(), sizeof(double) * 3 * knew);
        std::memcpy(slot + off_v, c->pend_var.data(), sizeof(double) * knew);
    }
    HIPCHK(hipMemcpyAsync(c->d_rs, slot, knew ? off_v + sizeof(double) * knew : sizeof(int) * std::max(Nnew, 1), hipMemcpyHostToDevice, c->stream));
    const int nnew = 21 + 3 * Nnew;
    {
        KTimer t(c, KN_MISC);
        LAUNCH_TS(c, k_reshape, dim3(blocks(nnew, 256), nnew + blocks(Nnew, 256)), dim3(256), c->stream, Nnew, c->Ncap, c->ld, (const int*)c->d_rs, (const double*)(c->d_rs + off_p),
                  (const double*)(c->d_rs + off_v), (const TS*)c->d_sigma[c->cur], (TS*)c->d_sigma[1 - c->cur], (const double*)c->d_st[c->stcur], (const double*)c->d_lm[c->lmcur],
                  c->d_st[1 - c->stcur], c->d_lm[1 - c->lmcur]);
        HIPCHK(hipGetLastError());
    }
    c->cur = 1 - c->cur;
    c->lmcur = 1 - c->lmcur;
    c->stcur = 1 - c->stcur;
    c->dev_N = Nnew;
    c->reshape_pending = false;
    return knew ? round_sigma(c) : 0;
}

int eqf_add_landmarks(eqf_ctx* c, const int* ids, const double* p, int k, double var) {
    HP_SCOPE("abi.add_landmarks");
    if (!c || k < 0 || (k > 0 && (!ids || !p)))
        return EQF_E_BAD_ARG;
    if (k == 0)
        return 0;
    if (c->n_held > 0)
        return EQF_E_UNSUPPORTED;
    HIPCHK(hipSetDevice(c->device));
    if (c->N + k > c->Ncap) {
        const int rc = grow_capacity(c, std::max(c->N + k, 2 * c->Ncap));
        if (rc)
            return rc;
    }
    pend_begin(c);
    for (int t = 0; t < k; ++t) {
        c->pend_map.push_back(-((int)c->pend_var.size() + 1));
        c->pend_p.insert(c->pend_p.end(), p + 3 * t, p + 3 * t + 3);
        c->pend_var.push_back(var);
    }
    if (c->est_valid) {
        const int N = c->N;
        std::vector<double> e(4 * (size_t)(N + k));
        for (int pl = 0; pl < 4; ++pl) {
// ... 640 lines not shown
        rc = normal_congruence(c, +1, dt, Pdiag8);
        if (rc)
            return rc;
    }
    return round_sigma(c);
}

static void observer_host_step(GroupSensor& X, const SensorState& xi0, const double* imu, double dt, int discreteLift, ObsStep& st) {
    {
        const SensorState xh = sensor_action(X, xi0);
        const V3 gyr = v3(imu[1], imu[2], imu[3]) - xh.bgyr;
        const V3 acc = v3(imu[4], imu[5], imu[6]) - xh.bacc;
        const V3 gbv = v3(imu[7], imu[8], imu[9]), abv = v3(imu[10], imu[11], imu[12]);
        const V3 gdir = q_rot(q_inv(xh.pose.R), v3(0, 0, 1));
        GroupSensor L;
        st.discrete = discreteLift ? 1 : 0;
        st.dt = dt;
        if (discreteLift) {
            L.bgyr = dt * gbv;
            L.bacc = dt * abv;
            L.A.R = so3_exp(dt * gyr);
            V3 x = dt * q_rot(xh.pose.R, xh.vel) + (0.5 * dt * dt) * (q_rot(xh.pose.R, acc) + v3(0, 0, -kGravity));
            L.A.x = q_rot(q_inv(xh.pose.R), x);
            L.B = pose_mul(pose_mul(pose_inv(xh.cam), L.A), xh.cam);
            const V3 bodyVelDiff = acc - kGravity * gdir;
            L.w = xh.vel - (xh.vel + dt * bodyVelDiff);
            st.Tinv = pose_mul(pose_mul(pose_inv(xh.cam), pose_inv(L.A)), xh.cam);
            st.omC = v3(0, 0, 0);
            st.vC = v3(0, 0, 0);
        } else {
            const V6 U_A{gyr, xh.vel};
            const V6 U_B = Ad_apply(pose_inv(xh.cam), U_A);
            const V3 u_w = -acc + kGravity * gdir;
            L.bgyr = dt * gbv;
            L.bacc = dt * abv;
            const M3 V = so3_V(dt * U_A.w);
            L.A = Pose{so3_exp(dt * U_A.w), V * (dt * U_A.v)};
            L.w = V * (dt * u_w);
            L.B = se3_exp(dt * U_B.w, dt * U_B.v);
            st.Tinv = pose_identity();
            st.omC = U_B.w;
            st.vC = U_B.v;
        }
        X = group_mul(X, L);
    }
}
static void observer_host_steps(eqf_ctx* c, const double* imu13_k, const double* dt_k, int chunk, int discreteLift, ObsSteps& steps_arg) {
    for (int s = 0; s < chunk; ++s)
        observer_host_step(c->X, c->xi0, imu13_k + 13 * s, dt_k[s], discreteLift, steps_arg.s[s]);
}
static int observer_launch(eqf_ctx* c, const ObsSteps& steps_arg, int chunk) {
    if (c->N == 0)
        return 0;
    if (!c->stream2)
        HIPCHK(hipStreamCreateWithFlags(&c->stream2, hipStreamNonBlocking));
    if (c->obs_pending)
        HIPCHK(hipStreamWaitEvent(c->stream2, c->ev_observer, 0));
    if (!c->ev_assembled_early)
        HIPCHK(hipEventRecord(c->ev_assembled, c->stream));
    HIPCHK(hipStreamWaitEvent(c->stream2, c->ev_assembled_early ? c->ev_early : c->ev_assembled, 0));
    c->ev_assembled_early = false;
    hipLaunchKernelGGL(k_observer, dim3(blocks(c->N, 64)), dim3(64), 0, c->stream2, steps_arg, c->N, c->Ncap, chunk, c->q0(), c->Qq(), c->Qa());
    HIPCHK(hipGetLastError());
    HIPCHK(hipEventRecord(c->ev_observer, c->stream2));
    c->obs_pending = true;
    return 0;
}
int eqf_integrate_observer(eqf_ctx* c, const double* imu13_k, const double* dt_k, int k, int discreteLift) {
    if (c && c->n_held > 0)
        return EQF_E_UNSUPPORTED;
    if (!c || k < 0 || (k > 0 && (!imu13_k || !dt_k)))
        return EQF_E_BAD_ARG;
    if (k == 0)
        return 0;
    { int _e = enter(c); if (_e) return _e; }
    c->est_valid = false, ++c->est_epoch;
    c->meas_valid = false;
    c->me_valid = false;
    int done = 0;
    while (done < k) {
        const int chunk = std::min(k - done, eqf_ctx::kMaxSteps);
        ObsSteps steps_arg;
        observer_host_steps(c, imu13_k + 13 * done, dt_k + done, chunk, discreteLift, steps_arg);
        const int rc = observer_launch(c, steps_arg, chunk);
        if (rc)
            return rc;
        done += chunk;
    }
    return 0;
}

static int stage_prepare(eqf_ctx* c);
int eqf_propagate_fast(eqf_ctx* c, const double* imu13_mean, double dt_total, const double* Qdiag12, const double* Pdiag8, const double* imu13_k, const double* dt_k,
                       int k, int discreteLift) {
    HP_SCOPE("abi.propagate_fast");
    if (!c || !imu13_mean || !Qdiag12 || !Pdiag8 || k < 0 || (k > 0 && (!imu13_k || !dt_k)))
        return EQF_E_BAD_ARG;
    GatherArgs gather{};
    bool use_gather = false;
    const bool fused_kernel = c->opt_fuse_asm && !c->opt_dense && !c->sig32 && c->chart != EQVIO_COORD_NORMAL && k > 0 && c->N > 0;
    if (c->n_held > 0 && !fused_kernel)
        return EQF_E_UNSUPPORTED;
    const int Nprop = c->N - c->n_held;
    const bool hold_here = c->n_held > 0 && !c->held_in_memory;
    if (fused_kernel && c->opt_gather && (c->reshape_pending || hold_here) && c->pend_var.empty() && c->dev_N <= GATHER_MAXN &&
        (!c->reshape_pending || ((int)c->pend_map.size() == Nprop && c->dev_N >= Nprop))) {
        bool ok = true;
        if (c->reshape_pending) {
            int prev = -1;
            for (int i = 0; i < Nprop && ok; ++i) {
                const int o = c->pend_map[i];
                ok = o > prev && o < c->dev_N;
                if (ok)
                    gather.surv[o >> 6] |= 1ull << (o & 63);
                prev = o;
            }
            gather.n = c->dev_N - Nprop;
        } else
            ok = c->dev_N == Nprop;
        if (ok && (gather.n > 0 || hold_here)) {
            use_gather = true;
            if (hold_here)
                gather.held = c->h_held;
        }
    }
    if (use_gather) {
        HIPCHK(hipSetDevice(c->device));
        c->ocov_valid = false;
    } else {
        int _e = enter(c, false);
        if (_e)
            return _e;
    }
    ++c->trace_frame;
    host_stamp(c, TH_PROP_ENTRY);
    int rc;
    {
        HP_SCOPE("pf.upload_common");
        rc = upload_common(c, imu13_mean);
    }
    if (rc)
        return rc;
    const bool fuse = c->opt_fuse_asm && !c->opt_dense;
    rc = fuse ? join_observer(c) : launch_assemble(c, false);
    if (rc)
        return rc;
    host_stamp(c, TH_ASSEMBLE_OUT);
    {
        HP_SCOPE("pf.stage_prepare");
        rc = stage_prepare(c);
    }
    if (rc)
        return rc;
    std::vector<ObsSteps> chunks;
    std::vector<int> counts;
    HP_SCOPE("pf.observer_steps_and_launch");
    for (int done = 0; done < k;) {
        const int chunk = std::min(k - done, eqf_ctx::kMaxSteps);
        chunks.emplace_back();
        observer_host_steps(c, imu13_k + 13 * done, dt_k + done, chunk, discreteLift, chunks.back());
        counts.push_back(chunk);
        done += chunk;
    }
    if (k > 0) {
        c->est_valid = false, ++c->est_epoch;
        c->meas_valid = false;
    }
    const bool ride = !c->opt_dense && !chunks.empty() && c->N > 0;
    c->obs_one_chunk = chunks.size() == 1;
    {
        HP_SCOPE("pf.launch");
        if (use_gather && !(ride && fuse)) {
            materialise_held(c);
            rc = flush_reshape(c);
            if (rc)
                return rc;
            use_gather = false;
        }
        rc = riccati_after_assemble(c, dt_total, Qdiag12, Pdiag8, ride ? &chunks[0] : nullptr, ride ? counts[0] : 0, fuse, use_gather ? &gather : nullptr);
    }
    if (rc)
        return rc;
    host_stamp(c, TH_PROP_OUT);
    for (size_t q = ride ? 1 : 0; q < chunks.size() && Nprop > 0; ++q) {
        c->ev_assembled_early = false;
        hipLaunchKernelGGL(k_observer, dim3(blocks(Nprop, 64)), dim3(64), 0, c->stream, chunks[q], Nprop, c->Ncap, counts[q], c->q0(), c->Qq(), c->Qa());
        HIPCHK(hipGetLastError());
    }
    return settle_update(c);
}

static int launch_chain(eqf_ctx* c, int rows, int m, int ldz, double* Z, double* W, bool first_tile_done = false, const int* spec = nullptr, int spec_seq = 0,
                        double* gpart = nullptr) {
    constexpr int NB = 32;
    if (!first_tile_done) {
        KTimer t(c, KN_CHOL_UPDATE);
        hipLaunchKernelGGL(k_chol_first, dim3(1), dim3(256), 0, c->stream, std::min(NB, m), ldz, Z, c->d_Linv, c->d_flags);
        HIPCHK(hipGetLastError());
    }
    int step = 0;
    KTimer t(c, KN_CHOL_PANEL, blocks(m, NB));
    for (int kb = 0; kb < m; kb += NB, ++step) {
        const int w = std::min(NB, m - kb);
        const int c0 = kb + w;
        double* Lin = c->d_Linv + 1024 * (step & 1);
        double* Lout = c->d_Linv + 1024 * ((step + 1) & 1);
        const int gx = blocks(rows - c0, 32);
        const int nyS = c0 < m ? blocks(m - c0, 32) : 1;
        double* gp = (gpart && c0 >= m) ? gpart : nullptr;
        {
            auto launch = [&](auto kern) {
                hipLaunchKernelGGL(kern, dim3(gx, nyS + (gp ? GAMMA_G : 0)), dim3(256), 0, c->stream, rows, m, kb, w, ldz, Z, W, Lin, Lout, c->d_flags, c0 < m ? 1 : 0, nyS, spec,
                                   spec_seq, gp, c->ld, gpart && step < 32 ? trace_slot(c, TR_STEP0 + step) : nullptr);
            };
            if (gp)
                launch(k_chol_step<true>);
            else
                launch(k_chol_step<false>);
        }
        HIPCHK(hipGetLastError());
    }
    return 0;
}

static bool lookahead_eligible(const eqf_ctx* c, int m) {
    const int NJ = blocks(m, 32);
    const int NI = (2 * NJ - 1) + blocks(c->n() + 1, 16) + 1;
    return c->opt_lookahead && c->la_selftest >= 0 && c->d_pub && NJ >= 3 && NJ <= c->la_njcap && NI <= c->cu_count;
}
constexpr int LA_SPLIT_FROM = 16;
static int la_split_extra(const eqf_ctx* c, int NJ, int base) {
    const int extra = NJ > LA_SPLIT_FROM + 1 ? 2 * (NJ - LA_SPLIT_FROM) : 0;
    return (c->opt_la_split && base + extra <= c->cu_count) ? extra : 0;
}
static int launch_lookahead(eqf_ctx* c, int rows, int m, int ldz, const int* spec, int spec_seq, int zb = 0, const MeasFuse* zb_mf = nullptr) {
    LaArgs a{};
    a.rows = rows;
    a.m = m;
    a.ldz = ldz;
    a.NJ = blocks(m, 32);
    a.NI = (2 * a.NJ - 1) + blocks(rows - m, 16);
    const int extra = la_split_extra(c, a.NJ, a.NI);
    a.split_from = extra ? LA_SPLIT_FROM : a.NJ;
    a.watch_ahead = c->opt_la_watch_ahead;
    const int nT = a.NI - (2 * a.NJ - 1);
    const bool home = c->opt_la_home && a.NJ <= 16 && c->cu_count == 256 && c->d_pubfl &&
                      (c->opt_la_home == 2 || c->la_home_force || (a.NJ >= 6 && device_to_itself(c)));
    a.home = home ? c->la_home : -1;
    a.pubfl = c->d_pubfl;
    const int home_grid = 8 * std::max(2 * a.NJ - 1, blocks(nT + (zb >= 2 ? 1 : 0), 7));
    if (home)
        ++c->la_home_launches;
    if (++c->la_seq <= 0)
        c->la_seq = 1;
    a.seq = c->la_seq;
    if (c->opt_early_door && c->early_seq_next) {
        a.early_cnt = c->d_door + 3, a.early_door = c->h_door + 3, a.early_gamma_host = c->h_res + 7 * (size_t)c->Ncap;
        a.early_seq = c->early_seq_next, a.early_spec = spec, a.early_spec_seq = spec_seq;
        c->early_armed_seq = c->early_seq_next;
    }
    c->early_seq_next = 0;
    a.timeout_ticks = c->la_timeout_ticks;
    a.Z = c->d_Z;
    a.W = c->d_W;
    a.Linv0 = c->d_Linv;
    a.pub = c->d_pub;
    a.pubf = c->d_pubf;
    a.puby = c->d_puby;
    a.gamma = c->d_gamma;
    a.flags = c->d_flags;
    a.spec = spec;
    a.spec_seq = spec_seq;
    a.live_cols = a.NJ <= 16 ? c->la_live_cols : nullptr;
    if (a.live_cols)
        ++c->live_first_launches;
    a.tr_steps = trace_slot(c, TR_STEP0);
    a.dbg = c->d_trace ? c->d_ladbg : nullptr;
    KTimer t(c, KN_CHOL_LOOKAHEAD);
    if (zb) {
        const bool large = a.NJ > 16;
        a.zb_sig = (const double*)c->sigma(), a.zb_ld = c->ld, a.zb_M = m / 2, a.zb_Mcap = c->Ncap, a.zb_var = c->tail_var;
        a.zb_C = c->d_C, a.zb_ytil = c->d_ytil, a.zb_lmidx = c->d_lmidx, a.zb_linv0 = c->d_Linv;
        a.zb_ident = (zb != 2 && c->tail_ident) ? 1 : 0;
        a.tr_zb = trace_slot(c, TR_BUILD_Z);
        ++c->zb_launches;
        if (zb == 2) {
            a.zb_mf = *zb_mf;
            a.spec = nullptr;
            if (home)
                hipLaunchKernelGGL(HIP_KERNEL_NAME(k_chol_lookahead<4, 2, true>), dim3(home_grid), dim3(LA_T), 0, c->stream, a);
            else
                hipLaunchKernelGGL(HIP_KERNEL_NAME(k_chol_lookahead<4, 2>), dim3(a.NI + 1), dim3(LA_T), 0, c->stream, a);
        } else if (zb == 3) {
            a.zb_mf = *zb_mf;
            a.spec = nullptr;
            if (large)
                hipLaunchKernelGGL(HIP_KERNEL_NAME(k_chol_lookahead<8, 3>), dim3(a.NI + extra + 1), dim3(LA_T), 0, c->stream, a);
            else if (home)
                hipLaunchKernelGGL(HIP_KERNEL_NAME(k_chol_lookahead<4, 3, true>), dim3(home_grid), dim3(LA_T), 0, c->stream, a);
            else
                hipLaunchKernelGGL(HIP_KERNEL_NAME(k_chol_lookahead<4, 3>), dim3(a.NI + 1), dim3(LA_T), 0, c->stream, a);
        } else if (large)
            hipLaunchKernelGGL(HIP_KERNEL_NAME(k_chol_lookahead<8, 1>), dim3(a.NI + extra), dim3(LA_T), 0, c->stream, a);
        else if (home)
            hipLaunchKernelGGL(HIP_KERNEL_NAME(k_chol_lookahead<4, 1, true>), dim3(home_grid), dim3(LA_T), 0, c->stream, a);
        else
            hipLaunchKernelGGL(HIP_KERNEL_NAME(k_chol_lookahead<4, 1>), dim3(a.NI), dim3(LA_T), 0, c->stream, a);
    } else if (a.NJ <= 16) {
// ... 533 lines not shown
    } else if (discreteCorr) {
        D.A = se3_exp(gw, gv);
        D.w = xi0.vel - q_rot(D.A.R, xi0.vel + gvel);
        D.B = pose_mul(pose_mul(pose_mul(pose_inv(xi0.cam), D.A), xi0.cam), se3_exp(cw, cv));
    } else {
        const V3 u_w = -gvel - cross(gw, xi0.vel);
        const V6 UB0 = Ad_apply(pose_inv(xi0.cam), V6{gw, gv});
        const M3 V = so3_V(gw);
        D.A = Pose{so3_exp(gw), V * gv};
        D.w = V * u_w;
        D.B = se3_exp(cw + UB0.w, cv + UB0.v);
    }
    return D;
}
static int apply_sensor_lift(eqf_ctx* c, int discreteCorr) {
    std::memcpy(c->h_buf, c->h_res + 7 * (size_t)c->Ncap, sizeof(double) * 21);
    const double* g = c->h_buf;
    const GroupSensor D = sensor_lift_delta(g, c->xi0, c->chart, discreteCorr);
    c->X = group_mul(D, c->X);
    if (c->opt_check) {
        const int r = read_flags(c);
        if (r)
            return r;
    }
    if (c->h_flags[1])
        return EQF_E_NONFINITE;
    for (int i = 0; i < 21; ++i)
        if (!(g[i] - g[i] == 0.0))
            return EQF_E_NONFINITE;
    return 0;
}

int eqf_vision_update(eqf_ctx* c, const eqvio_camera* cam, const int* ids, const double* y, int M, double meas_var, int useEqv, int discreteCorr) {
    if (!c || !cam || M < 0 || (M > 0 && (!ids || !y)) || !camera_ok(cam))
        return EQF_E_BAD_ARG;
    if (M == 0)
        return 0;
    if (M > c->N)
        return EQF_E_BAD_ARG;
    { int _e = enter(c); if (_e) return _e; }
    const bool reuse = c->meas_valid && c->meas_star == (useEqv ? 1 : 0) && (int)c->meas_ids.size() == M && std::equal(ids, ids + M, c->meas_ids.begin()) &&
                       std::memcmp(c->h_y, y, sizeof(double) * 2 * M) == 0;
    int rc = 0;
    if (!reuse) {
        rc = stage_measurement(c, ids, y, M);
        if (rc)
            return rc;
    }
    c->meas_valid = false;
    if (!reuse) {
        KTimer t(c, KN_MEASURE);
        hipLaunchKernelGGL(k_measure, dim3(blocks(M, 64)), dim3(64), 0, c->stream, M, c->Ncap, c->Ncap, c->chart, make_cam(cam), useEqv, c->h_lmidx, c->h_y, c->q0(), c->Qq(),
                           c->Qa(), c->d_C, c->d_ytil, c->d_lmidx, c->d_flags);
        HIPCHK(hipGetLastError());
    }
    const bool use_door = c->opt_door && !c->opt_check && !c->obs_pending;
    const int door_seq = (int)(++c->door_seq);
    rc = launch_update_tail(c, ids, M, meas_var, discreteCorr, nullptr, 0, use_door, door_seq);
    if (rc)
        return rc;
    rc = use_door ? door_wait(c, 1, door_seq) : sync_ctx(c);
    if (rc)
        return rc;
    return finish_update(c, discreteCorr);
}

int eqf_stage_measurement(eqf_ctx* c, const int* ids, const double* y, int M) {
    HP_SCOPE("abi.stage_measurement");
    if (!c || M < 0 || (M > 0 && (!ids || !y)))
        return EQF_E_BAD_ARG;
    c->stage_requested = c->stage_pending = c->staged_valid = false;
    if (M == 0 || c->N == 0 || M > c->N)
        return 0;
    c->staged_ids.assign(ids, ids + M);
    c->staged_y.assign(y, y + 2 * M);
    c->staged_M = M;
    c->stage_requested = true;
    return 0;
}
static int stage_prepare(eqf_ctx* c) {
    if (!c->stage_requested)
        return 0;
    c->stage_requested = false;
    const int M = c->staged_M;
    if (c->N == 0 || M > c->N)
        return 0;
    if (c->busy_meas) {
        int r = sync_ctx(c);
        if (r)
            return r;
    }
    int* lmidx = c->h_lmidx;
    int* measof = c->h_lmidx + c->Ncap;
    const int rc = map_measurement(c, c->staged_ids.data(), M, false, lmidx, measof);
    if (rc)
        return 0;
    for (int j = 0; j < M; ++j)
        if (lmidx[j] < 0)
            return 0;
    std::memcpy(c->h_y, c->staged_y.data(), sizeof(double) * 2 * M);
    pack_by_landmark(c, measof, c->staged_y.data());
    c->staged_gen = c->lm_gen;
    c->stage_pending = true;
    return 0;
}

static int stats_then_update(eqf_ctx* c, const eqvio_camera* cam, const int* ids, const double* y, int M, double thrAbs, double thrProb, double meas_var, int useEqv,
                             int discreteCorr, double* absErr, double* probErr, double* depth2, int* updated, int max_outliers, int* removed_idx, int* n_removed) {
    HP_SCOPE("abi.stats_then_update");
    if (!c || !cam || !updated || M <= 0 || !ids || !y || !camera_ok(cam))
        return EQF_E_BAD_ARG;
    ++c->spec_calls;
    *updated = 0;
    c->pred_cam = make_cam(cam), c->pred_star = useEqv ? 1 : 0, c->pred_valid = true;
    const int N = c->N;
    if (N == 0 || M > N) {
        *updated = -1;
        return 0;
    }
    { int _e = enter(c); if (_e) return _e; }
    host_stamp(c, TH_TAIL_ENTRY);
    { int _r = join_observer(c); if (_r) return _r; }
    bool speculate = c->opt_spec && !c->opt_check && !c->obs_pending;
    if (speculate && c->opt_spec == 1 && c->spec_backoff > 0) {
        --c->spec_backoff;
        speculate = false;
    }
    const bool use_door = c->opt_door && !c->opt_check && !c->obs_pending;
    const bool same_as_staged = c->staged_valid && c->staged_gen == c->lm_gen && c->staged_M == M && std::equal(ids, ids + M, c->staged_ids.begin()) &&
                                std::memcmp(c->staged_y.data(), y, sizeof(double) * 2 * M) == 0;
    const bool staged = speculate && same_as_staged;
    c->staged_valid = c->stage_pending = c->stage_requested = false;
    int* lmidx = c->h_lmidx;
    int* measof = c->h_lmidx + c->Ncap;
    int rc = 0;
    if (!same_as_staged) {
        if (c->busy_meas) {
            int r = sync_ctx(c);
            if (r)
                return r;
        }
        rc = map_measurement(c, ids, M, false, lmidx, measof);
        if (rc)
            return rc;
        for (int j = 0; j < M; ++j)
            if (lmidx[j] < 0) {
                *updated = -1;
                return 0;
            }
        std::memcpy(c->h_y, y, sizeof(double) * 2 * M);
    }
    HP_SCOPE("stu.after_map");
    const int seq = (int)(++c->door_seq);
    auto copy_stats = [&]() {
        if (absErr)
            std::memcpy(absErr, c->h_res, sizeof(double) * N);
        if (probErr)
            std::memcpy(probErr, c->h_res + N, sizeof(double) * N);
        if (depth2)
            std::memcpy(depth2, c->h_res + 2 * N, sizeof(double) * N);
    };
    c->meas_star = useEqv ? 1 : 0;
    c->meas_ids.assign(ids, ids + M);
    c->busy_meas = true;
    if (!speculate && max_outliers >= 0 && N <= SEL_MAXN) {
        const bool live_first = N <= SEL_ONE_WG && c->opt_sel_one && c->opt_live_first && blocks(2 * M, 32) <= 16 && blocks(2 * M, 32) >= 3;
        if (N <= SEL_ONE_WG && c->opt_sel_one) {
            KTimer t(c, KN_STATS);
            LAUNCH_TS(c, k_stats_select, dim3(1), dim3(512), c->stream, N, c->Ncap, c->ld, c->chart, make_cam(cam),
                      same_as_staged ? (const double*)(c->d_meas + 2 * (size_t)c->Ncap)  : pack_by_landmark(c, measof, y), c->q0(), c->Qq(), c->Qa(),
                      (const TS*)c->sigma(), c->h_res, useEqv ? 1 : 0, c->d_C, c->d_ytil, c->d_lmidx, c->d_flags, thrAbs, thrProb, max_outliers, M, c->h_sel, live_first ? c->d_spec + 2 : (int*)nullptr);
            HIPCHK(hipGetLastError());
        } else {
            KTimer t(c, KN_STATS);
            LAUNCH_TS(c, k_outlier_stats, dim3(blocks(N, 64)), dim3(64), c->stream, N, c->Ncap, c->ld, c->chart, make_cam(cam), same_as_staged ? (const double*)c->h_ylm : pack_by_landmark(c, measof, y), c->q0(), c->Qq(),
                      c->Qa(), (const TS*)c->sigma(), c->h_res, useEqv ? 1 : 0, c->d_C, c->d_ytil, c->d_lmidx, c->d_flags, (int*)nullptr, c->h_door, seq, thrAbs, thrProb,
                      (int*)nullptr, seq, c->d_stats);
            HIPCHK(hipGetLastError());
            hipLaunchKernelGGL(k_select_outliers, dim3(1), dim3(256), 0, c->stream, N, c->Ncap, M, c->d_stats, thrAbs, thrProb, max_outliers, c->d_lmidx, c->d_C, c->d_ytil, c->h_sel);
            HIPCHK(hipGetLastError());
        }
        c->meas_valid = false;
        c->early_allowed = c->opt_early_door != 0;
        rc = launch_update_tail(c, ids, M, meas_var, discreteCorr, nullptr, 0, use_door, seq, nullptr, live_first);
        if (rc)
            return rc;
        host_stamp(c, TH_TAIL_OUT);
        bool early = false;
        rc = use_door ? door_wait(c, 1, seq, &early) : sync_ctx(c);
        if (rc)
            return rc;
        copy_stats();
        ++c->sel_frames;
        if (c->h_sel[c->Ncap] == 0)
            c->spec_backoff = c->spec_backoff_len = 0;
        rc = early ? finish_update_early(c, discreteCorr, seq) : finish_update(c, discreteCorr);
        if (rc)
            return rc;
        *updated = 1;
        std::vector<int> idx;
        for (int i = 0; i < N; ++i)
            if (c->h_sel[i])
                idx.push_back(i);
        if (n_removed)
            *n_removed = (int)idx.size();
        if (removed_idx)
            std::copy(idx.begin(), idx.end(), removed_idx);
        c->sel_discarded += (long)idx.size();
        return idx.empty() ? 0 : eqf_remove_landmarks(c, idx.data(), (int)idx.size());
    }
    if (!speculate) {
        {
            KTimer t(c, KN_STATS);
            LAUNCH_TS(c, k_outlier_stats, dim3(blocks(N, 64)), dim3(64), c->stream, N, c->Ncap, c->ld, c->chart, make_cam(cam), same_as_staged ? (const double*)c->h_ylm : pack_by_landmark(c, measof, y), c->q0(), c->Qq(),
                      c->Qa(), (const TS*)c->sigma(), c->h_res, useEqv ? 1 : 0, c->d_C, c->d_ytil, c->d_lmidx, c->d_flags, use_door ? c->d_door : nullptr, c->h_door, seq, thrAbs,
                      thrProb, (int*)nullptr, seq, (double*)nullptr);
            HIPCHK(hipGetLastError());
        }
        c->meas_valid = true;
        rc = use_door ? door_wait(c, 0, seq) : sync_ctx(c);
        if (rc)
            return rc;
        copy_stats();
        bool candidate = false;
        for (int i = 0; i < N && !candidate; ++i)
            candidate = c->h_res[i] > thrAbs || c->h_res[N + i] > thrProb;
        if (!candidate)
            c->spec_backoff = c->spec_backoff_len = 0;
        return 0;
    }
    MeasFuse mf{};
    mf.enabled = 1;
    mf.N = N, mf.Ncap = c->Ncap, mf.chart = c->chart, mf.star = useEqv ? 1 : 0;
    mf.cam = make_cam(cam);
    if (staged)
        mf.y = c->d_meas, mf.lmidx = c->d_meas_idx, mf.ylm = c->d_meas + 2 * (size_t)c->Ncap;
    else
        mf.y = c->h_y, mf.lmidx = lmidx, mf.ylm = pack_by_landmark(c, measof, y);
    mf.q0 = c->q0(), mf.Qq = c->Qq(), mf.Qa = c->Qa();
    mf.out = c->h_res;
    mf.C = c->d_C, mf.ytil = c->d_ytil, mf.lmidx_dev = c->d_lmidx;
    mf.thrAbs = thrAbs, mf.thrProb = thrProb;
    mf.spec_w = c->d_spec, mf.spec_seq = seq;
    c->meas_valid = false;
    c->early_allowed = c->opt_early_door != 0;
    rc = launch_update_tail(c, ids, M, meas_var, discreteCorr, c->d_spec, seq, use_door, seq, &mf);
    if (rc)
        return rc;
    host_stamp(c, TH_TAIL_OUT);
    bool early = false;
    rc = use_door ? door_wait(c, 1, seq, &early) : sync_ctx(c);
    if (rc)
        return rc;
    copy_stats();
    ++c->spec_queued;
    if (early) {
        c->spec_backoff = c->spec_backoff_len = 0;
        rc = finish_update_early(c, discreteCorr, seq);
        if (rc == 0)
            *updated = 1;
        return rc;
    }
    if (c->h_resflags[2]) {
        ++c->spec_cancelled;
        c->spec_backoff_len = std::min(max_outliers >= 0 ? 256 : 16, std::max(1, 2 * c->spec_backoff_len));
        c->spec_backoff = c->spec_backoff_len;
        c->meas_valid = true;
        return 0;
    }
    c->spec_backoff = c->spec_backoff_len = 0;
    rc = finish_update(c, discreteCorr);
    if (rc == 0)
        *updated = 1;
    return rc;
}

int eqf_stats_then_update(eqf_ctx* c, const eqvio_camera* cam, const int* ids, const double* y, int M, double thrAbs, double thrProb, double meas_var, int useEqv,
                          int discreteCorr, double* absErr, double* probErr, double* depth2, int* updated) {
    return stats_then_update(c, cam, ids, y, M, thrAbs, thrProb, meas_var, useEqv, discreteCorr, absErr, probErr, depth2, updated, -1, nullptr, nullptr);
}
int eqf_stats_select_update(eqf_ctx* c, const eqvio_camera* cam, const int* ids, const double* y, int M, double thrAbs, double thrProb, int max_outliers, double meas_var,
                            int useEqv, int discreteCorr, double* absErr, double* probErr, double* depth2, int* updated, int* removed_idx, int* n_removed) {
    if (max_outliers < 0 || !n_removed)
        return EQF_E_BAD_ARG;
    *n_removed = 0;
    return stats_then_update(c, cam, ids, y, M, thrAbs, thrProb, meas_var, useEqv, discreteCorr, absErr, probErr, depth2, updated, max_outliers, removed_idx, n_removed);
}
int eqf_selection_stats(eqf_ctx* c, long* frames, long* discarded, int reset) {
    if (!c)
        return EQF_E_BAD_ARG;
    if (frames)
        *frames = c->sel_frames;
    if (discarded)
        *discarded = c->sel_discarded;
    if (reset)
        c->sel_frames = c->sel_discarded = 0;
    return 0;
}

int eqf_last_gamma(eqf_ctx* c, double* out, int cap) {
    if (!c || !out)
        return EQF_E_BAD_ARG;
    { int _r = keep_last_gamma(c); if (_r) return _r; }
    if ((int)c->last_gamma.size() > cap)
        return EQF_E_CAPACITY;
    std::memcpy(out, c->last_gamma.data(), sizeof(double) * c->last_gamma.size());
    return (int)c->last_gamma.size();
}

int eqf_compute_nees(eqf_ctx* c, const double* ts, const int* tids, const double* tp, int ntrue, double* nees) {
    if (!c || !ts || !nees || ntrue < 0 || (ntrue > 0 && (!tids || !tp)))
        return EQF_E_BAD_ARG;
    { int _e = enter(c); if (_e) return _e; }
    const int N = c->N, n = c->n();
    const int np = n + (n & 1);
    std::vector<double> q0(3 * (size_t)N + 3), Q(5 * (size_t)N + 5);
    std::vector<int> ids(N + 1);
    double s0[23], g0[23];
    int rc = eqf_get_state(c, s0, g0, ids.data(), q0.data(), Q.data(), N);
    if (rc < 0)
        return rc;
    std::vector<double> eps(np, 0.0);
    nees_sensor_error(c->xi0, c->X, c->chart, ts, eps.data());
    for (int i = 0; i < N; ++i) {
        int jt = -1;
        for (int t = 0; t < ntrue; ++t)
            if (tids[t] == ids[i]) {
                jt = t;
                break;
            }
        if (jt < 0)
            return EQF_E_BAD_ARG;
        const V3 ptrue = v3(tp[3 * jt], tp[3 * jt + 1], tp[3 * jt + 2]);
        const Qt qi{Q[5 * i], Q[5 * i + 1], Q[5 * i + 2], Q[5 * i + 3]};
        const V3 pe = Q[5 * i + 4] * q_rot(qi, ptrue);
        const V3 q0i = v3(q0[3 * i], q0[3 * i + 1], q0[3 * i + 2]);
        const V3 e = c->chart == EQVIO_COORD_NORMAL ? normal_chart(pe, q0i) : point_chart(c->chart == EQVIO_COORD_INVDEPTH, pe, q0i);
        pack_v3(e, eps.data() + 21 + 3 * i);
    }
    if (!c->d_Zn) {
        const int npcap = c->ncap + 1;
        c->ldzn = pick_ld(npcap + 1);
        HIPCHK(hipMalloc(&c->d_Zn, sizeof(double) * (size_t)c->ldzn * npcap));
        HIPCHK(hipMalloc(&c->d_Wn, sizeof(double) * (size_t)c->ldzn * npcap));
        HIPCHK(hipMalloc(&c->d_perm, sizeof(int) * 2 * (size_t)(c->ncap + 2)));
    }
    { int _r = keep_last_gamma(c); if (_r) return _r; }
    { int _r = sync_ctx(c); if (_r) return _r; }
    std::memcpy(c->h_buf, eps.data(), sizeof(double) * np);
    HIPCHK(hipMemcpyAsync(c->d_gamma, c->h_buf, sizeof(double) * np, hipMemcpyHostToDevice, c->stream));
    HIPCHK(hipMemsetAsync(c->d_flags, 0, sizeof(int) * 4, c->stream));
    LAUNCH_TS(c, k_build_nees, dim3(blocks(np + 1, 256), np), dim3(256), c->stream, n, np, c->ld, c->ldzn, (const TS*)c->sigma(), c->d_gamma, c->d_Zn);
    HIPCHK(hipGetLastError());
    rc = launch_chain(c, np + 1, np, c->ldzn, c->d_Zn, c->d_Wn);
    if (rc)
        return rc;
    hipLaunchKernelGGL(k_sumsq_row, dim3(1), dim3(256), 0, c->stream, np, c->ldzn, c->d_Wn, np, c->d_stats);
    HIPCHK(hipGetLastError());
    HIPCHK(hipMemcpyAsync(c->h_buf, c->d_stats, sizeof(double), hipMemcpyDeviceToHost, c->stream));
    rc = read_flags(c);
    if (rc)
        return rc;
    if (c->h_flags[0]) {
        ++c->nees_lu_fallbacks;
        std::memcpy(c->h_buf, eps.data(), sizeof(double) * np);
        HIPCHK(hipMemcpyAsync(c->d_gamma, c->h_buf, sizeof(double) * np, hipMemcpyHostToDevice, c->stream));
        LAUNCH_TS(c, k_build_nees, dim3(blocks(np + 1, 256), np), dim3(256), c->stream, n, np, c->ld, c->ldzn, (const TS*)c->sigma(), c->d_gamma, c->d_Zn);
        hipLaunchKernelGGL(k_iota, dim3(blocks(np, 256)), dim3(256), 0, c->stream, np, c->d_perm);
        const int pstride = c->ncap + 2;
        for (int k = 0; k < np; ++k)
            hipLaunchKernelGGL(k_ge_step, dim3(std::max(1, blocks(np - k - 1, GE_ROWS))), dim3(256), 0, c->stream, np, c->ldzn, k, c->d_Zn, c->d_perm + (k & 1) * pstride,
                               c->d_perm + ((k + 1) & 1) * pstride);
        hipLaunchKernelGGL(k_ge_back, dim3(1), dim3(1024), sizeof(double) * (np + 16), c->stream, n, np, c->ldzn, c->d_Zn, c->d_perm + (np & 1) * pstride, c->d_gamma, c->d_stats);
        HIPCHK(hipGetLastError());
        HIPCHK(hipMemcpyAsync(c->h_buf, c->d_stats, sizeof(double), hipMemcpyDeviceToHost, c->stream));
        { int _r = sync_ctx(c); if (_r) return _r; }
    }
    *nees = c->h_buf[0] / (double)n;
    return 0;
}

int eqf_debug_get_W(eqf_ctx* c, double* out, int rows, int cols) {
    if (!c || !out || rows <= 0 || cols <= 0 || rows > c->ldz || cols > c->mcap)
        return EQF_E_BAD_ARG;
    { int _r = sync_ctx(c); if (_r) return _r; }
    HIPCHK(hipMemcpy2D(out, sizeof(double) * rows, c->d_W, sizeof(double) * c->ldz, sizeof(double) * rows, cols, hipMemcpyDeviceToHost));
    return 0;
}

int eqf_debug_lookahead_stamps(eqf_ctx* c, unsigned long long* out768) {
    if (!c || !out768 || !c->d_ladbg)
        return EQF_E_BAD_ARG;
    { int _r = sync_ctx(c); if (_r) return _r; }
    HIPCHK(hipMemcpy(out768, c->d_ladbg, 96 * 8 * sizeof(unsigned long long), hipMemcpyDeviceToHost));
    return 0;
}

int eqf_measure_in_propagate_stats(eqf_ctx* c, long* used, int reset) {
    if (!c || !used)
        return EQF_E_BAD_ARG;
    *used = c->me_used;
    if (reset)
        c->me_used = 0;
    return 0;
}
int eqf_z_in_lookahead_stats(eqf_ctx* c, long* launches, int reset) {
    if (!c || !launches)
        return EQF_E_BAD_ARG;
    *launches = c->zb_launches;
    if (reset)
        c->zb_launches = 0;
    return 0;
}
int eqf_gather_stats(eqf_ctx* c, long* launches, int reset) {
    if (!c || !launches)
        return EQF_E_BAD_ARG;
    *launches = c->gather_launches;
    if (reset)
        c->gather_launches = 0;
    return 0;
}
int eqf_speculation_stats(eqf_ctx* c, long* calls, long* queued, long* cancelled, int reset) {
    if (!c || !calls || !queued || !cancelled)
        return EQF_E_BAD_ARG;
    *calls = c->spec_calls;
    *queued = c->spec_queued;
    *cancelled = c->spec_cancelled;
    if (reset)
        c->spec_calls = c->spec_queued = c->spec_cancelled = 0;
    return 0;
}

int eqf_debug_syrk_order(int nt, int* tile_of_block) {
    if (nt < 1 || nt > 4095 || !tile_of_block)
        return EQF_E_BAD_ARG;
    build_syrk_order(nt, tile_of_block);
    return 0;
}
int eqf_lookahead_stats(eqf_ctx* c, long* launches, long* fallbacks, int reset) {
// ... 916 lines not shown
```

eqvio_amd/host/VIOFilter.cpp:

```cpp
#include "VIOFilter.hpp"
#include "../csrc/host_prof.hpp"
#include <optional>
#include <algorithm>
#include <cmath>
#include <cstring>
#include <numeric>

namespace eqvio_amd {
namespace { constexpr double GRAVITY_CONSTANT_ = 9.80665; }

using namespace eqf;

thread_local LoopTimer loopTimer;

void LoopTimer::startTiming(const std::string& label) { timerStartPoints.at(label) = timer_clock::now(); }
void LoopTimer::endTiming(const std::string& label) {
    const timer_clock::time_point now = timer_clock::now();
    currentLoopTimingData.timings[label] = now - timerStartPoints.at(label);
}
void LoopTimer::startLoop() {
    for (const auto& kv : timerStartPoints)
        currentLoopTimingData.timings[kv.first] = timer_duration(0);
    currentLoopTimingData.loopTimeStart = timer_clock::now() - timerOrigin;
}
// ... 186 lines not shown
    check(eqf_get_sigma(ctx, S.d.data(), S.r), "eqf_get_sigma");
    return S;
}
void VIO_eqf::setSigma(const MatrixXd& S) { settleInvalid(); check(eqf_set_sigma(ctx, S.d.data(), S.r), "eqf_set_sigma"); }
void VIO_eqf::setSigmaDiag(const std::vector<double>& diag) { settleInvalid(); check(eqf_set_sigma_diag(ctx, diag.data(), (int)diag.size()), "eqf_set_sigma_diag"); }

bool VIO_eqf::addNewLandmarks(std::vector<Landmark>& newLandmarks, double var, bool held) {
    if (!held)
        settleInvalid();
    const int k = (int)newLandmarks.size();
    if (k == 0)
        return true;
    std::vector<int> ids(k);
    std::vector<double> p(3 * k);
    for (int i = 0; i < k; ++i) {
        ids[i] = newLandmarks[i].id;
        p[3 * i] = newLandmarks[i].p.x;
        p[3 * i + 1] = newLandmarks[i].p.y;
        p[3 * i + 2] = newLandmarks[i].p.z;
    }
    if (held) {
        const int rc = eqf_add_landmarks_held(ctx, ids.data(), p.data(), k, var);
        if (rc == EQF_E_UNSUPPORTED)
            return false;
        check(rc, "eqf_add_landmarks_held");
    } else
        check(eqf_add_landmarks(ctx, ids.data(), p.data(), k, var), "eqf_add_landmarks");
    ids_.insert(ids_.end(), ids.begin(), ids.end());
    return true;
}
void VIO_eqf::removeLandmarksByIndex(const std::vector<int>& idx) {
    settleInvalid();
    if (idx.empty())
        return;
    check(eqf_remove_landmarks(ctx, idx.data(), (int)idx.size()), "eqf_remove_landmarks");
    std::vector<char> drop(ids_.size(), 0);
    for (int i : idx)
        drop[i] = 1;
    std::vector<int> kept;
    for (size_t i = 0; i < ids_.size(); ++i)
        if (!drop[i])
            kept.push_back(ids_[i]);
    ids_ = kept;
}
bool VIO_eqf::removeUnmeasured(const std::vector<int>& measurementIds) {
    scratchIdx_.resize(ids_.size() + 1);
    int n = 0;
    const int rc = eqf_remove_unmeasured_landmarks(ctx, measurementIds.data(), (int)measurementIds.size(), scratchIdx_.data(), &n);
    if (rc == EQF_E_BAD_ARG)
        return false;
    check(rc, "eqf_remove_unmeasured_landmarks");
    if (n > 0) {
        size_t w = 0;
        int t = 0;
        for (size_t i = 0; i < ids_.size(); ++i) {
            if (t < n && scratchIdx_[t] == (int)i) {
                ++t;
                continue;
            }
            ids_[w++] = ids_[i];
        }
        ids_.resize(w);
    }
    return true;
}
bool VIO_eqf::sameAsMapped(const std::vector<int>& measurementIds) const { return eqf_same_as_mapped(ctx, measurementIds.data(), (int)measurementIds.size()) == 1; }
bool VIO_eqf::findUnknownIds(const std::vector<int>& measurementIds, std::vector<int>& unknownJ, int& n) const {
    unknownJ.resize(measurementIds.size() + 1);
    const int rc = eqf_find_unknown_ids(ctx, measurementIds.data(), (int)measurementIds.size(), unknownJ.data(), &n);
    if (rc == EQF_E_BAD_ARG)
        return false;
    check(rc, "eqf_find_unknown_ids");
    return true;
}
void VIO_eqf::removeLandmarkByIndex(const int& idx) { removeLandmarksByIndex({idx}); }
void VIO_eqf::removeLandmarkById(const int& id) {
    const auto it = std::find(ids_.begin(), ids_.end(), id);
    if (it == ids_.end())
        throw std::out_of_range("VIO_eqf::removeLandmarkById: unknown id");
    removeLandmarkByIndex((int)std::distance(ids_.begin(), it));
}
int VIO_eqf::settleInvalid() const {
    if (!invalidPending_)
        return 0;
    invalidPending_ = false;
    const int rc = eqf_remove_invalid_at_update(ctx);
    if (rc < 0)
        check(rc, "eqf_remove_invalid_at_update");
    if (rc > 0) {
        ids_.resize(eqf_num_landmarks(ctx));
        eqf_get_ids(ctx, ids_.data(), (int)ids_.size());
    }
    return rc;
}
void VIO_eqf::removeInvalidLandmarks() {
    if (eqf_update_unsettled(ctx) == 1) {
        invalidPending_ = true;
        return;
    }
    settleInvalid();
    const int rc = eqf_remove_invalid_landmarks(ctx);
    if (rc < 0)
        check(rc, "eqf_remove_invalid_landmarks");
    if (rc > 0) {
        ids_.resize(eqf_num_landmarks(ctx));
        eqf_get_ids(ctx, ids_.data(), (int)ids_.size());
    }
}
std::array<double, 9> VIO_eqf::getLandmarkCovById(const int& id) const {
    settleInvalid();
    const auto it = std::find(ids_.begin(), ids_.end(), id);
    if (it == ids_.end())
        throw std::out_of_range("VIO_eqf::getLandmarkCovById: unknown id");
    const int i = (int)std::distance(ids_.begin(), it);
    std::array<double, 9> blk{};
    check(eqf_get_sigma_block(ctx, 21 + 3 * i, 21 + 3 * i, 3, 3, blk.data()), "eqf_get_sigma_block");
    return blk;
}
void VIO_eqf::integrateObserverStates(const std::vector<IMUVelocity>& imus, const std::vector<double>& dts, bool discreteLift) {
    settleInvalid();
    const int k = (int)imus.size();
    if (k == 0)
        return;
    std::vector<double> flat(13 * (size_t)k);
    for (int i = 0; i < k; ++i)
        imus[i].pack(flat.data() + 13 * i);
    check(eqf_integrate_observer(ctx, flat.data(), dts.data(), k, discreteLift ? 1 : 0), "eqf_integrate_observer");
}
void VIO_eqf::integrateObserverState(const IMUVelocity& imu, const double& dt, const bool& discreteLift) {
    settleInvalid();
    integrateObserverStates({imu}, {dt}, discreteLift);
}
void VIO_eqf::integrateRiccatiStateAccurate(const IMUVelocity& v, const double& dt, const std::array<double, 12>& Qd, const std::array<double, 8>& Pd8) {
    settleInvalid();
    double imu[13];
    v.pack(imu);
    check(eqf_integrate_riccati_accurate(ctx, imu, dt, Qd.data(), Pd8.data()), "integrateRiccatiStateAccurate");
}
void VIO_eqf::integrateRiccatiStateDiscrete(const IMUVelocity& v, const double& dt, const std::array<double, 12>& Qd, const std::array<double, 8>& Pd8) {
    settleInvalid();
    double imu[13];
    v.pack(imu);
    check(eqf_integrate_riccati_discrete(ctx, imu, dt, Qd.data(), Pd8.data()), "integrateRiccatiStateDiscrete");
}
void VIO_eqf::propagateFast(const IMUVelocity& mean, const double& dtTotal, const std::array<double, 12>& Qd, const std::array<double, 8>& Pd8,
                            const std::vector<IMUVelocity>& imus, const std::vector<double>& dts, bool discreteLift) {
    double m13[13];
    mean.pack(m13);
    std::vector<double> all(13 * imus.size());
    for (size_t i = 0; i < imus.size(); ++i)
        imus[i].pack(all.data() + 13 * i);
    check(eqf_propagate_fast(ctx, m13, dtTotal, Qd.data(), Pd8.data(), all.data(), dts.data(), (int)imus.size(), discreteLift ? 1 : 0), "eqf_propagate_fast");
}
void VIO_eqf::integrateRiccatiStateFast(const IMUVelocity& imu, const double& dt, const std::array<double, 12>& Qd, const std::array<double, 8>& Pd8) {
    settleInvalid();
    double v[13];
    imu.pack(v);
    check(eqf_integrate_riccati_fast(ctx, v, dt, Qd.data(), Pd8.data()), "eqf_integrate_riccati_fast");
}
void VIO_eqf::performVisionUpdate(const VisionMeasurement& m, double var, const bool& useEqv, const bool& discreteCorrection) {
    settleInvalid();
    if (m.camCoordinates.empty())
        return;
    const FlatMeas fm(m);
    const std::vector<int>& ids = fm.ids;
    const std::vector<double>& y = fm.y;
    check(eqf_vision_update(ctx, &m.cameraPtr->c, ids.data(), y.data(), (int)ids.size(), var, useEqv ? 1 : 0, discreteCorrection ? 1 : 0), "eqf_vision_update");
}
VIOState VIO_eqf::stateEstimate() const {
    settleInvalid();
    const int N = numLandmarks();
    double s[23];
    std::vector<int> ids(N + 1);
    std::vector<double> p(3 * N + 3);
    const int rc = eqf_state_estimate(ctx, s, ids.data(), p.data(), N);
    if (rc < 0)
        check(rc, "eqf_state_estimate");
    VIOState xi;
    xi.sensor = unpackSensor(s);
    xi.cameraLandmarks.resize(N);
    for (int i = 0; i < N; ++i)
        xi.cameraLandmarks[i] = Landmark{V3{p[3 * i], p[3 * i + 1], p[3 * i + 2]}, ids[i]};
    return xi;
}
double VIO_eqf::computeNEES(const VIOState& trueState) const {
    settleInvalid();
    double s[23];
    packSensor(trueState.sensor, s);
    const int Nt = (int)trueState.cameraLandmarks.size();
    std::vector<int> ids(Nt + 1);
    std::vector<double> p(3 * Nt + 3);
    for (int i = 0; i < Nt; ++i) {
        ids[i] = trueState.cameraLandmarks[i].id;
        p[3 * i] = trueState.cameraLandmarks[i].p.x;
        p[3 * i + 1] = trueState.cameraLandmarks[i].p.y;
        p[3 * i + 2] = trueState.cameraLandmarks[i].p.z;
    }
    double nees = 0;
    check(eqf_compute_nees(ctx, s, ids.data(), p.data(), Nt, &nees), "eqf_compute_nees");
    return nees;
}
void VIO_eqf::outlierStats(const VisionMeasurement& m, std::vector<double>& absErr, std::vector<double>& probErr, std::vector<double>& depth2) const {
    settleInvalid();
    const int N = numLandmarks();
    absErr.assign(N, -1.0);
    probErr.assign(N, -1.0);
    depth2.assign(N, 0.0);
    if (N == 0)
        return;
    const FlatMeas fm(m);
    const std::vector<int>& ids = fm.ids;
    const std::vector<double>& y = fm.y;
    check(eqf_outlier_stats(ctx, &m.cameraPtr->c, ids.data(), y.data(), (int)ids.size(), absErr.data(), probErr.data(), depth2.data()), "eqf_outlier_stats");
}
void VIO_eqf::stageMeasurement(const VisionMeasurement& m) {
    if (m.camCoordinates.empty() || numLandmarks() == 0)
        return;
    const FlatMeas fm(m.flatHint());
    const std::vector<int>& ids = fm.ids;
    const std::vector<double>& y = fm.y;
    check(eqf_stage_measurement(ctx, ids.data(), y.data(), (int)ids.size()), "eqf_stage_measurement");
}
int VIO_eqf::statsThenUpdate(const VisionMeasurement& m, double thrAbs, double thrProb, double var, bool useEqv, bool discreteCorrection, std::vector<double>& absErr,
                              std::vector<double>& probErr, std::vector<double>& depth2, long maxOutliers) {
    settleInvalid();
    const int N = numLandmarks();
    absErr.assign(N, -1.0);
    probErr.assign(N, -1.0);
    depth2.assign(N, 0.0);
    const FlatMeas fm(m);
    const std::vector<int>& ids = fm.ids;
    const std::vector<double>& y = fm.y;
    int updated = 0;
    if (maxOutliers < 0) {
        check(eqf_stats_then_update(ctx, &m.cameraPtr->c, ids.data(), y.data(), (int)ids.size(), thrAbs, thrProb, var, useEqv ? 1 : 0, discreteCorrection ? 1 : 0,
                                    absErr.data(), probErr.data(), depth2.data(), &updated),
              "eqf_stats_then_update");
        return updated;
    }
    std::vector<int> removed(N + 1);
    int nRemoved = 0;
    check(eqf_stats_select_update(ctx, &m.cameraPtr->c, ids.data(), y.data(), (int)ids.size(), thrAbs, thrProb, (int)std::min<long>(maxOutliers, 1 << 30), var, useEqv ? 1 : 0,
                                  discreteCorrection ? 1 : 0, absErr.data(), probErr.data(), depth2.data(), &updated, removed.data(), &nRemoved),
          "eqf_stats_select_update");
    if (nRemoved > 0) {
        std::vector<char> drop(ids_.size(), 0);
        for (int t = 0; t < nRemoved; ++t)
            drop[removed[t]] = 1;
        std::vector<int> kept;
        for (size_t i = 0; i < ids_.size(); ++i)
            if (!drop[i])
                kept.push_back(ids_[i]);
        ids_ = kept;
    }
    return updated;
}

VIOFilter::Settings::Settings(const eqvio_settings& s) {
    biasOmegaProcessVariance = s.biasOmegaProcessVariance;
    biasAccelProcessVariance = s.biasAccelProcessVariance;
    attitudeProcessVariance = s.attitudeProcessVariance;
    positionProcessVariance = s.positionProcessVariance;
    velocityProcessVariance = s.velocityProcessVariance;
    cameraAttitudeProcessVariance = s.cameraAttitudeProcessVariance;
    cameraPositionProcessVariance = s.cameraPositionProcessVariance;
    pointProcessVariance = s.pointProcessVariance;
    velGyrNoise = s.velGyrNoise;
    velAccNoise = s.velAccNoise;
    velGyrBiasWalk = s.velGyrBiasWalk;
    velAccBiasWalk = s.velAccBiasWalk;
    measurementNoise = s.measurementNoise;
    outlierThresholdAbs = s.outlierThresholdAbs;
    outlierThresholdProb = s.outlierThresholdProb;
    featureRetention = s.featureRetention;
    initialAttitudeVariance = s.initialAttitudeVariance;
    initialPositionVariance = s.initialPositionVariance;
    initialVelocityVariance = s.initialVelocityVariance;
    initialCameraAttitudeVariance = s.initialCameraAttitudeVariance;
    initialCameraPositionVariance = s.initialCameraPositionVariance;
    initialPointVariance = s.initialPointVariance;
    initialPointDepthVariance = s.initialPointDepthVariance;
    initialBiasOmegaVariance = s.initialBiasOmegaVariance;
    initialBiasAccelVariance = s.initialBiasAccelVariance;
    initialSceneDepth = s.initialSceneDepth;
    useDiscreteInnovationLift = s.useDiscreteInnovationLift != 0;
    useDiscreteVelocityLift = s.useDiscreteVelocityLift != 0;
    useDiscreteStateMatrix = s.useDiscreteStateMatrix != 0;
    fastRiccati = s.fastRiccati != 0;
    useMedianDepth = s.useMedianDepth != 0;
    useFeaturePredictions = s.useFeaturePredictions != 0;
    useEquivariantOutput = s.useEquivariantOutput != 0;
    removeLostLandmarks = s.removeLostLandmarks != 0;
    if (s.coordinateChoice < 0 || s.coordinateChoice > 2)
        throw std::runtime_error("Invalid coordinate choice. Valid choices are Euclidean, InvDepth, Normal.");
    coordinateChoice = (CoordinateChoice)s.coordinateChoice;
    cameraOffset = unpackPose(s.cameraOffset);
}
std::vector<double> VIOFilter::Settings::constructInitialStateCovarianceDiag(const size_t& N) const {
    std::vector<double> d(21 + 3 * N, initialPointVariance);
    const double v[7] = {initialBiasOmegaVariance, initialBiasAccelVariance, initialAttitudeVariance, initialPositionVariance,
                         initialVelocityVariance,  initialCameraAttitudeVariance, initialCameraPositionVariance};
    for (int b = 0; b < 7; ++b)
        for (int k = 0; k < 3; ++k)
            d[3 * b + k] = v[b];
    if (initialPointDepthVariance > 0)
        for (size_t i = 0; i < N; ++i)
            d[21 + 3 * i + 2] = initialPointDepthVariance;
    return d;
}
std::array<double, 8> VIOFilter::Settings::constructStateGainDiag8() const {
    return {biasOmegaProcessVariance, biasAccelProcessVariance,      attitudeProcessVariance,       positionProcessVariance,
            velocityProcessVariance,  cameraAttitudeProcessVariance, cameraPositionProcessVariance, pointProcessVariance};
}
std::array<double, 12> VIOFilter::Settings::constructInputGainDiag() const {
    std::array<double, 12> q{};
    const double v[4] = {velGyrNoise * velGyrNoise, velAccNoise * velAccNoise, velGyrBiasWalk * velGyrBiasWalk, velAccBiasWalk * velAccBiasWalk};
    for (int b = 0; b < 4; ++b)
        for (int k = 0; k < 3; ++k)
            q[3 * b + k] = v[b];
    return q;
}

VIOFilter::~VIOFilter() = default;

VIOFilter::VIOFilter(const VIOFilter::Settings& s) {
    settings = std::make_unique<VIOFilter::Settings>(s);
    filterState.create(s.device, s.maxLandmarks, s.coordinateChoice);
    VIOState xi0;
    xi0.sensor.cameraOffset = s.cameraOffset;
    filterState.set(xi0, VIOGroup());
    filterState.setSigmaDiag(settings->constructInitialStateCovarianceDiag());
}
VIOFilter::VIOFilter(const VIOState& xi0, const VIOFilter::Settings& s, const double& time) {
    settings = std::make_unique<VIOFilter::Settings>(s);
    filterState.create(s.device, std::max<int>(s.maxLandmarks, (int)xi0.cameraLandmarks.size()), s.coordinateChoice);
    VIOGroup X;
    for (const Landmark& lm : xi0.cameraLandmarks) {
        X.Q.emplace_back(SOT3());
        X.id.emplace_back(lm.id);
    }
    filterState.set(xi0, X);
    filterState.setSigmaDiag(settings->constructInitialStateCovarianceDiag(xi0.cameraLandmarks.size()));
    filterState.currentTime = time;
    initialisedFlag = true;
}
void VIOFilter::processIMUData(const IMUVelocity& imu) {
    if (!initialisedFlag)
        initialiseFromIMUData(imu);
    velocityBuffer.emplace_back(imu);
}
void VIOFilter::initialiseFromIMUData(const IMUVelocity& imu) {
    VIOState xi0 = filterState.xi0();
    const VIOGroup X = filterState.X();
    xi0.sensor.inputBias.fill(0.0);
    xi0.sensor.pose = pose_identity();
    xi0.sensor.velocity = V3{0, 0, 0};
    initialisedFlag = true;
    xi0.sensor.pose.R = so3_from_vectors(normalized(imu.acc), V3{0, 0, 1});
    filterState.set(xi0, X);
    filterState.currentTime = imu.stamp;
}
void VIOFilter::setState(const VIOState& xi) {
    VIOGroup X;
    X.id = xi.getIds();
    X.Q.assign(X.id.size(), SOT3());
    filterState.set(xi, X);
    const int N = (int)xi.cameraLandmarks.size();
    std::vector<double> d = settings->constructInitialStateCovarianceDiag(0);
    d.resize(21 + 3 * N, 1.0 * settings->initialPointVariance);
    filterState.setSigmaDiag(d);
    initialisedFlag = true;
}
void VIOFilter::setLandmarks(const std::vector<Landmark>& lms) {
    MatrixXd S = filterState.Sigma();
    const std::vector<double> full = settings->constructInitialStateCovarianceDiag(lms.size());
    const int k = 3 * (int)lms.size();
    if (21 + k != S.r)
        throw std::invalid_argument("VIOFilter::setLandmarks: landmark count differs from the filter state");
    for (int j = 0; j < k; ++j)
        for (int i = 0; i < k; ++i)
            S(21 + i, 21 + j) = (i == j) ? full[21 + i] : 0.0;
    VIOState xi0 = filterState.xi0();
    VIOGroup X = filterState.X();
    xi0.cameraLandmarks = lms;
    X.Q.assign(lms.size(), SOT3());
    X.id.clear();
    for (const Landmark& lm : lms)
        X.id.emplace_back(lm.id);
    filterState.set(xi0, X);
    filterState.setSigma(S);
}
void VIOFilter::augmentLandmarkStates(const std::vector<int>& newIds, const VIOState& provided) {
    removeOldLandmarks(newIds);
    std::vector<Landmark> newLandmarks;
    const std::vector<int>& have = filterState.ids();
    for (const int& id : newIds) {
        if (std::find(have.begin(), have.end(), id) != have.end())
            continue;
        const auto it2 = std::find_if(provided.cameraLandmarks.begin(), provided.cameraLandmarks.end(), [&id](const Landmark& lm) { return lm.id == id; });
        if (it2 == provided.cameraLandmarks.end())
            throw std::out_of_range("augmentLandmarkStates: id missing from the provided state");
        newLandmarks.emplace_back(*it2);
    }
    filterState.addNewLandmarks(newLandmarks, settings->initialPointVariance);
}
bool VIOFilter::integrateUpToTime(const double& newTime) {
    if (newTime <= filterState.currentTime || filterState.currentTime < 0 || velocityBuffer.empty())
        return false;
    std::vector<double> dts(velocityBuffer.size());
    for (size_t i = 0; i < velocityBuffer.size(); ++i) {
        const double t0 = std::max(velocityBuffer.at(i).stamp, filterState.currentTime);
        const double t1 = i + 1 < velocityBuffer.size() ? std::min(velocityBuffer.at(i + 1).stamp, newTime) : newTime;
        dts[i] = std::max(t1 - t0, 0.0);
    }
    if (settings->fastRiccati) {
        double accumulatedTime = 0;
        IMUVelocity accumulatedVelocity = IMUVelocity::Zero();
        for (size_t i = 0; i < velocityBuffer.size(); ++i) {
            accumulatedTime += dts[i];
            accumulatedVelocity = accumulatedVelocity + velocityBuffer.at(i) * dts[i];
        }
        accumulatedVelocity = accumulatedVelocity * (1.0 / accumulatedTime);
        filterState.propagateFast(accumulatedVelocity, accumulatedTime, settings->constructInputGainDiag(), settings->constructStateGainDiag8(), velocityBuffer, dts,
                                  settings->useDiscreteVelocityLift);
    } else {
        for (size_t i = 0; i < velocityBuffer.size(); ++i) {
            if (dts[i] > 0) {
                if (settings->useDiscreteStateMatrix)
                    filterState.integrateRiccatiStateDiscrete(velocityBuffer.at(i), dts[i], settings->constructInputGainDiag(), settings->constructStateGainDiag8());
                else
                    filterState.integrateRiccatiStateAccurate(velocityBuffer.at(i), dts[i], settings->constructInputGainDiag(), settings->constructStateGainDiag8());
            }
            filterState.integrateObserverState(velocityBuffer.at(i), dts[i], settings->useDiscreteVelocityLift);
        }
    }
    filterState.currentTime = newTime;
    auto it = std::find_if(velocityBuffer.begin(), velocityBuffer.end(), [this](const IMUVelocity& v) { return v.stamp >= this->filterState.currentTime; });
    if (it != velocityBuffer.begin()) {
        --it;
        velocityBuffer.erase(velocityBuffer.begin(), it);
    }
    return true;
}
void VIOFilter::processVisionData(const VisionMeasurement& measurement) {
    HP_SCOPE("processVisionData");
    std::optional<VisionMeasurement::Validated> oneWalk;
    loopTimer.startTiming("propagation");
    const bool willIntegrate = !(measurement.stamp <= filterState.currentTime || filterState.currentTime < 0 || velocityBuffer.empty());
    bool quiet = false;
    if (initialisedFlag && willIntegrate && settings->fastRiccati)
        quiet = filterState.sameAsMapped(*measurement.flatHint().first);
    if (!quiet)
        oneWalk.emplace(measurement);
    bool removedEarly = initialisedFlag && willIntegrate && settings->removeLostLandmarks;
    if (removedEarly && !quiet) {
        HP_SCOPE("pv.removeOldLandmarks");
        removeOldLandmarks(measurement.flatIds());
    }
    bool heldAdd = quiet;
    if (!quiet && initialisedFlag && willIntegrate && settings->fastRiccati && !settings->useMedianDepth && filterState.holdSupported()) {
        HP_SCOPE("pv.addNewLandmarks");
        heldAdd = addNewLandmarks(measurement, nullptr, true);
    }
    if (initialisedFlag && settings->fastRiccati) {
        HP_SCOPE("pv.stageMeasurement");
        filterState.stageMeasurement(measurement);
    }
    bool integrationFlag;
    {
        HP_SCOPE("pv.integrateUpToTime");
        integrationFlag = integrateUpToTime(measurement.stamp);
    }
    if (quiet) {
        const size_t before = measurement.flatRebuilds();
        oneWalk.emplace(measurement);
        if (measurement.flatRebuilds() != before)
            removedEarly = false, heldAdd = false;
    }
    if (filterState.settleInvalid() > 0)
        heldAdd = false;
    if (!integrationFlag || !initialisedFlag)
        return;
    loopTimer.endTiming("propagation");

    loopTimer.startTiming("preprocessing");
    if (settings->removeLostLandmarks && !removedEarly) {
        HP_SCOPE("pv.removeOldLandmarks");
        removeOldLandmarks(measurement.flatIds());
    }
    const bool earlyAdd = !settings->useMedianDepth;
    if (earlyAdd && !heldAdd) {
        HP_SCOPE("pv.addNewLandmarks");
        addNewLandmarks(measurement, nullptr);
    }
    std::vector<double> depth2;
    bool haveStats = false;
    std::vector<double> absErr, probErr;
    if (!measurement.camCoordinates.empty() && filterState.numLandmarks() > 0) {
        HP_SCOPE("pv.statsThenUpdate");
        const long maxOutliers = earlyAdd ? (long)(size_t)((1.0 - settings->featureRetention) * measurement.camCoordinates.size()) : -1;
        const int r = filterState.statsThenUpdate(measurement, settings->outlierThresholdAbs, settings->outlierThresholdProb, settings->constructOutputGainVar(),
                                                  settings->useEquivariantOutput, settings->useDiscreteInnovationLift, absErr, probErr, depth2, maxOutliers);
        if (r == 1) {
            loopTimer.endTiming("preprocessing");
            loopTimer.startTiming("correction");
            filterState.removeInvalidLandmarks();
            loopTimer.endTiming("correction");
            return;
        }
        haveStats = (r == 0);
    }
    VisionMeasurement matchedMeasurement = measurement;
    removeOutliers(matchedMeasurement, depth2, haveStats ? &absErr : nullptr, haveStats ? &probErr : nullptr);
    if (!earlyAdd)
        addNewLandmarks(matchedMeasurement, &depth2);
    loopTimer.endTiming("preprocessing");

    if (matchedMeasurement.camCoordinates.empty())
        return;

    loopTimer.startTiming("correction");
    if (!settings->removeLostLandmarks) {
    }
    filterState.performVisionUpdate(matchedMeasurement, settings->constructOutputGainVar(), settings->useEquivariantOutput, settings->useDiscreteInnovationLift);
    filterState.removeInvalidLandmarks();
    loopTimer.endTiming("correction");
}
VIOState VIOFilter::stateEstimate() const { return filterState.stateEstimate(); }
const VIO_eqf& VIOFilter::viewEqFState() const { return filterState; }
double VIOFilter::getTime() const { return filterState.currentTime; }
VIOState integrateSystemFunction(const VIOState& state, const IMUVelocity& velocity, const double& dt) {
    VIOState ns;
    const VIOSensorState& s = state.sensor;
    const V3 gyr = velocity.gyr - V3{s.inputBias[0], s.inputBias[1], s.inputBias[2]};
    const V3 acc = velocity.acc - V3{s.inputBias[3], s.inputBias[4], s.inputBias[5]};
    const V3 dbg = dt * velocity.gyrBiasVel, dba = dt * velocity.accBiasVel;
    ns.sensor.inputBias = {s.inputBias[0] + dbg.x, s.inputBias[1] + dbg.y, s.inputBias[2] + dbg.z, s.inputBias[3] + dba.x, s.inputBias[4] + dba.y, s.inputBias[5] + dba.z};
    const V3 gravity{0, 0, -GRAVITY_CONSTANT_};
    Pose poseChange;
    poseChange.R = eqf::so3_exp(dt * gyr);
    const V3 inertialStep = dt * eqf::q_rot(s.pose.R, s.velocity) + (0.5 * dt * dt) * (eqf::q_rot(s.pose.R, acc) + gravity);
    poseChange.x = eqf::q_rot(eqf::q_inv(s.pose.R), inertialStep);
    ns.sensor.pose = eqf::pose_mul(s.pose, poseChange);
    const V3 inertialVelocityDiff = eqf::q_rot(s.pose.R, acc) + gravity;
    ns.sensor.velocity = eqf::q_rot(eqf::q_inv(ns.sensor.pose.R), eqf::q_rot(s.pose.R, s.velocity) + dt * inertialVelocityDiff);
    const Pose cameraPoseChangeInv = eqf::pose_mul(eqf::pose_mul(eqf::pose_inv(s.cameraOffset), eqf::pose_inv(poseChange)), s.cameraOffset);
    ns.cameraLandmarks.resize(state.cameraLandmarks.size());
    for (size_t i = 0; i < state.cameraLandmarks.size(); ++i)
        ns.cameraLandmarks[i] = Landmark{eqf::pose_act(cameraPoseChangeInv, state.cameraLandmarks[i].p), state.cameraLandmarks[i].id};
    ns.sensor.cameraOffset = s.cameraOffset;
    return ns;
}
VIOState VIO_eqf::predictState(const double& stamp, const std::vector<IMUVelocity>& imuVelocities) const {
    VIOState statePrediction = stateEstimate();
    for (size_t i = 0; i < imuVelocities.size(); ++i) {
        const double t0 = std::max(imuVelocities.at(i).stamp, this->currentTime);
        const double t1 = i + 1 < imuVelocities.size() ? std::min(imuVelocities.at(i + 1).stamp, stamp) : stamp;
        const double dt = std::max(t1 - t0, 0.0);
        statePrediction = integrateSystemFunction(statePrediction, imuVelocities.at(i), dt);
    }
    return statePrediction;
}
VisionMeasurement VIOFilter::getFeaturePredictions(const GICameraPtr& camPtr, const double& stamp) {
    VisionMeasurement r;
    if (settings->useFeaturePredictions) {
        const VIOState pred = filterState.predictState(stamp, velocityBuffer);
        for (const Landmark& lm : pred.cameraLandmarks) {
            double u, v;
            camPtr->projectPoint(lm.p, u, v);
            r.camCoordinates[lm.id] = {u, v};
        }
        r.cameraPtr = camPtr;
    }
    return r;
}
bool VIOFilter::addNewLandmarks(const VisionMeasurement& measurement, const std::vector<double>* depth2, bool held) {
    std::vector<Landmark> newLandmarks;
    {
        const auto fv = measurement.flat();
        const std::vector<int>& mids = *fv.first;
        const std::vector<double>& my = *fv.second;
        int n = 0;
        if (filterState.findUnknownIds(mids, unknownScratch_, n)) {
            if (n == 0)
                return true;
            newLandmarks.reserve(n);
            for (int t = 0; t < n; ++t) {
                const int j = unknownScratch_[t];
                const V3 bearing = measurement.cameraPtr->undistortPoint(my[2 * j], my[2 * j + 1]);
                newLandmarks.emplace_back(Landmark{bearing, mids[j]});
            }
            const double initialDepth = settings->useMedianDepth ? getMedianSceneDepth(depth2) : settings->initialSceneDepth;
            for (Landmark& blm : newLandmarks)
                blm.p = initialDepth * blm.p;
            return filterState.addNewLandmarks(newLandmarks, settings->initialPointVariance, held);
        }
    }
    if (held)
        return false;
    const std::vector<int>& stateIds = filterState.ids();
    std::vector<int> sortedCopy;
    if (!std::is_sorted(stateIds.begin(), stateIds.end())) {
        sortedCopy = stateIds;
        std::sort(sortedCopy.begin(), sortedCopy.end());
    }
    const std::vector<int>& have = sortedCopy.empty() ? stateIds : sortedCopy;
    const auto flatView = measurement.flat();
    const std::vector<int>& mids = *flatView.first;
    const std::vector<double>& my = *flatView.second;
    const bool merge = std::is_sorted(mids.begin(), mids.end());
    size_t h = 0;
    for (size_t j = 0; j < mids.size(); ++j) {
        const int ccId = mids[j];
        bool known;
        if (merge) {
            while (h < have.size() && have[h] < ccId)
                ++h;
            known = h < have.size() && have[h] == ccId;
        } else
            known = std::binary_search(have.begin(), have.end(), ccId);
        if (!known) {
            const V3 bearing = measurement.cameraPtr->undistortPoint(my[2 * j], my[2 * j + 1]);
            newLandmarks.emplace_back(Landmark{bearing, ccId});
        }
    }
    if (newLandmarks.empty())
        return true;
    const double initialDepth = settings->useMedianDepth ? getMedianSceneDepth(depth2) : settings->initialSceneDepth;
    for (Landmark& blm : newLandmarks)
        blm.p = initialDepth * blm.p;
    return filterState.addNewLandmarks(newLandmarks, settings->initialPointVariance);
}
void VIOFilter::removeOldLandmarks(const std::vector<int>& measurementIds) {
    if (filterState.removeUnmeasured(measurementIds))
        return;
    const std::vector<int>& have = filterState.ids();
    std::vector<int> lost;
    bool bothSorted;
    {
        HP_SCOPE("ro.sorted");
        bothSorted = std::is_sorted(measurementIds.begin(), measurementIds.end()) && std::is_sorted(have.begin(), have.end());
    }
    const bool sorted = bothSorted || std::is_sorted(measurementIds.begin(), measurementIds.end());
    if (bothSorted) {
        {
            HP_SCOPE("ro.merge");
            size_t q = 0;
            for (int i = 0; i < (int)have.size(); ++i) {
                while (q < measurementIds.size() && measurementIds[q] < have[i])
                    ++q;
                if (q == measurementIds.size() || measurementIds[q] != have[i])
                    lost.push_back(i);
            }
        }
        HP_SCOPE("ro.removeByIndex");
// ... 92 lines not shown
```

eqvio_amd/host/VIOFilter.hpp:

```cpp
#pragma once
#include "../csrc/eqf_math.hpp"
#include "eqf_hip.h"
#include <array>
#include <chrono>
#include <map>
#include <memory>
#include <stdexcept>
#include <string>
#include <vector>

namespace eqvio_amd {

using eqf::Pose;
using eqf::Qt;
using eqf::V3;

class LoopTimer {
  public:
    using timer_clock = std::chrono::steady_clock;
    using timer_duration = std::chrono::duration<double>;
    struct LoopTimingData {
        timer_duration loopTimeStart{};
        std::map<std::string, timer_duration> timings;
    };
// ... 4 lines not shown
    const LoopTimingData& getLoopTimingData() const { return currentLoopTimingData; }

  protected:
    const timer_clock::time_point timerOrigin = timer_clock::now();
    std::map<std::string, timer_clock::time_point> timerStartPoints;
    LoopTimingData currentLoopTimingData;
};
extern thread_local LoopTimer loopTimer;

struct Landmark {
    V3 p{0, 0, 0};
    int id = -1;
};
struct VIOSensorState {
    std::array<double, 6> inputBias{};
    Pose pose = eqf::pose_identity();
    V3 velocity{0, 0, 0};
    Pose cameraOffset = eqf::pose_identity();
    V3 gravityDir() const { return eqf::q_rot(eqf::q_inv(pose.R), V3{0, 0, 1}); }
    static constexpr int CompDim = 21;
};
struct VIOState {
    VIOSensorState sensor;
    std::vector<Landmark> cameraLandmarks;
    std::vector<int> getIds() const;
    int Dim() const { return VIOSensorState::CompDim + 3 * (int)cameraLandmarks.size(); }
};
struct SOT3 {
    Qt R = eqf::q_identity();
    double a = 1.0;
};
struct VIOGroup {
    std::array<double, 6> beta{};
    Pose A = eqf::pose_identity();
    V3 w{0, 0, 0};
    Pose B = eqf::pose_identity();
    std::vector<SOT3> Q;
    std::vector<int> id;
};
struct IMUVelocity {
    double stamp = 0;
    V3 gyr{0, 0, 0}, acc{0, 0, 0}, gyrBiasVel{0, 0, 0}, accBiasVel{0, 0, 0};
    static IMUVelocity Zero() { return IMUVelocity(); }
    IMUVelocity operator+(const IMUVelocity& other) const;
    IMUVelocity operator*(const double& c) const;
    void pack(double* v13) const;
};
struct Camera {
    eqvio_camera c{};
    eqf::Cam model() const {
        eqf::Cam k{c.fx, c.fy, c.cx, c.cy};
        k.model = c.model;
        for (int i = 0; i < 5; ++i)
            k.d[i] = c.dist[i];
        return k;
    }
    void projectPoint(V3 p, double& u, double& v) const { eqf::cam_project(model(), p, u, v); }
    V3 undistortPoint(double u, double v) const { return eqf::cam_undistort(model(), u, v); }
};
using GICameraPtr = std::shared_ptr<const Camera>;
VIOState integrateSystemFunction(const VIOState& state, const IMUVelocity& velocity, const double& dt);
struct VisionMeasurement {
    double stamp = 0;
    std::map<int, std::array<double, 2>> camCoordinates;
    GICameraPtr cameraPtr;
    std::vector<int> getIds() const;
    std::pair<const std::vector<int>*, const std::vector<double>*> flat() const { return refreshFlat(), std::make_pair(&flatIds_, &flatY_); }
    const std::vector<int>& flatIds() const { return refreshFlat(), flatIds_; }
    const std::vector<double>& flatY() const { return refreshFlat(), flatY_; }
    void invalidateFlat() const { flatIds_.clear(), flatY_.clear(), flatN_ = (size_t)-1; }
    size_t flatRebuilds() const { return flatRebuilds_; }
    std::pair<const std::vector<int>*, const std::vector<double>*> flatHint() const {
        if (flatN_ != camCoordinates.size() || flatIds_.size() != camCoordinates.size())
            refreshFlat();
        return std::make_pair(&flatIds_, &flatY_);
    }

    struct Validated {
        const VisionMeasurement& m;
        explicit Validated(const VisionMeasurement& meas) : m(meas) {
            m.refreshFlat();
            m.flatTrusted_.on = true;
        }
        ~Validated() { m.flatTrusted_.on = false; }
        Validated(const Validated&) = delete;
        Validated& operator=(const Validated&) = delete;
    };

  private:
    void refreshFlat() const;
    struct Trust {
        bool on = false;
        Trust() = default;
        Trust(const Trust&) {}
        Trust& operator=(const Trust&) {
            on = false;
            return *this;
        }
    };
    mutable Trust flatTrusted_;
    mutable std::vector<int> flatIds_;
    mutable std::vector<double> flatY_;
    mutable size_t flatN_ = (size_t)-1;
    mutable size_t flatRebuilds_ = 0;
};

enum class CoordinateChoice { Euclidean = 0, InvDepth = 1, Normal = 2 };

struct MatrixXd {
    int r = 0, c = 0;
    std::vector<double> d;
    int rows() const { return r; }
    int cols() const { return c; }
    double& operator()(int i, int j) { return d[(size_t)j * r + i]; }
    const double& operator()(int i, int j) const { return d[(size_t)j * r + i]; }
};

struct VIO_eqf {
    eqf_ctx* ctx = nullptr;
    CoordinateChoice coordinateChoice = CoordinateChoice::Euclidean;
    double currentTime = -1;

    VIO_eqf() = default;
    VIO_eqf(const VIO_eqf&) = delete;
    VIO_eqf& operator=(const VIO_eqf&) = delete;
    ~VIO_eqf();
    void create(int device, int maxLandmarks, CoordinateChoice cc);

    VIOState xi0() const;
    VIOGroup X() const;
    MatrixXd Sigma() const;
    const std::vector<int>& ids() const { return ids_; }
    int numLandmarks() const { return (int)ids_.size(); }
    void set(const VIOState& xi0, const VIOGroup& X);
    void setSigma(const MatrixXd& S);
    void setSigmaDiag(const std::vector<double>& diag);

    bool addNewLandmarks(std::vector<Landmark>& newLandmarks, double newLandmarkVar, bool held = false);
    bool holdSupported() const { return eqf_hold_supported(ctx) == 1; }
    void removeLandmarkByIndex(const int& idx);
    void removeLandmarkById(const int& id);
    void removeLandmarksByIndex(const std::vector<int>& idx);
    void removeInvalidLandmarks();
    int settleInvalid() const;
    bool removeUnmeasured(const std::vector<int>& measurementIds);
    bool sameAsMapped(const std::vector<int>& measurementIds) const;
    bool findUnknownIds(const std::vector<int>& measurementIds, std::vector<int>& unknownJ, int& n) const;
    std::array<double, 9> getLandmarkCovById(const int& id) const;
    void integrateObserverState(const IMUVelocity& imuVelocity, const double& dt, const bool& discreteLift = true);
    void integrateObserverStates(const std::vector<IMUVelocity>& imus, const std::vector<double>& dts, bool discreteLift);
    void integrateRiccatiStateFast(const IMUVelocity& imuVelocity, const double& dt, const std::array<double, 12>& inputGainDiag, const std::array<double, 8>& stateGainDiag8);
    void propagateFast(const IMUVelocity& meanVelocity, const double& dtTotal, const std::array<double, 12>& inputGainDiag, const std::array<double, 8>& stateGainDiag8,
                       const std::vector<IMUVelocity>& imus, const std::vector<double>& dts, bool discreteLift);
    void integrateRiccatiStateAccurate(const IMUVelocity& imuVelocity, const double& dt, const std::array<double, 12>& inputGainDiag, const std::array<double, 8>& stateGainDiag8);
    void integrateRiccatiStateDiscrete(const IMUVelocity& imuVelocity, const double& dt, const std::array<double, 12>& inputGainDiag, const std::array<double, 8>& stateGainDiag8);
    void performVisionUpdate(const VisionMeasurement& measurement, double outputGainVar, const bool& useEquivariantOutput = true, const bool& discreteCorrection = false);
    VIOState stateEstimate() const;
    VIOState predictState(const double& stamp, const std::vector<IMUVelocity>& imuVelocities) const;
    double computeNEES(const VIOState& trueState) const;
    void outlierStats(const VisionMeasurement& measurement, std::vector<double>& absErr, std::vector<double>& probErr, std::vector<double>& depth2) const;
    void stageMeasurement(const VisionMeasurement& measurement);
    int statsThenUpdate(const VisionMeasurement& measurement, double thrAbs, double thrProb, double outputGainVar, bool useEquivariantOutput, bool discreteCorrection,
                         std::vector<double>& absErr, std::vector<double>& probErr, std::vector<double>& depth2, long maxOutliers = -1);

  private:
    mutable std::vector<int> ids_;
    mutable bool invalidPending_ = false;
    std::vector<int> scratchIdx_;
    void check(int rc, const char* what) const;
};

class VIOFilter {
  protected:
    VIO_eqf filterState;
    bool initialisedFlag = false;
    std::vector<IMUVelocity> velocityBuffer;

    bool integrateUpToTime(const double& newTime);
    bool addNewLandmarks(const VisionMeasurement& measurement, const std::vector<double>* depth2, bool held = false);
    void removeOldLandmarks(const std::vector<int>& measurementIds);
    void removeOutliers(VisionMeasurement& measurement, std::vector<double>& depth2, const std::vector<double>* absErrIn = nullptr,
                        const std::vector<double>* probErrIn = nullptr);
    double getMedianSceneDepth(const std::vector<double>* depth2) const;
    std::vector<int> unknownScratch_;

  public:
    struct Settings;
    std::unique_ptr<VIOFilter::Settings> settings;

    VIOFilter() = default;
    explicit VIOFilter(const VIOFilter::Settings& settings);
    VIOFilter(const VIOState& xi0, const VIOFilter::Settings& settings, const double& time = 0.0);
    ~VIOFilter();

    void initialiseFromIMUData(const IMUVelocity& imuVelocity);
    void setState(const VIOState& xi);
    void setLandmarks(const std::vector<Landmark>& cameraLandmarks);
    void augmentLandmarkStates(const std::vector<int>& newIds, const VIOState& providedState);
    void processIMUData(const IMUVelocity& imuVelocity);
    void processVisionData(const VisionMeasurement& measurement);
    double getTime() const;
    bool isInitialised() const { return initialisedFlag; }
    VisionMeasurement getFeaturePredictions(const GICameraPtr& camPtr, const double& stamp = -1);
    VIOState stateEstimate() const;
    const VIO_eqf& viewEqFState() const;
    VIO_eqf& eqfState() { return filterState; }
};

struct VIOFilter::Settings {
    double biasOmegaProcessVariance = 0.001, biasAccelProcessVariance = 0.001, attitudeProcessVariance = 0.001, positionProcessVariance = 0.001,
           velocityProcessVariance = 0.001, cameraAttitudeProcessVariance = 0.001, cameraPositionProcessVariance = 0.001, pointProcessVariance = 0.001;
    double velGyrNoise = 1e-4, velAccNoise = 1e-3, velGyrBiasWalk = 1e-5, velAccBiasWalk = 1e-3;
    double measurementNoise = 2.0, outlierThresholdAbs = 1e8, outlierThresholdProb = 1e8, featureRetention = 0.3;
    double initialAttitudeVariance = 1.0e-4, initialPositionVariance = 1.0e-4, initialVelocityVariance = 1.0e-2, initialCameraAttitudeVariance = 1.0e-5,
           initialCameraPositionVariance = 1.0e-4, initialPointVariance = 1.0, initialPointDepthVariance = -1.0, initialBiasOmegaVariance = 0.1,
           initialBiasAccelVariance = 0.1, initialSceneDepth = 1.0;
    bool useDiscreteInnovationLift = true, useDiscreteVelocityLift = true, useDiscreteStateMatrix = false, fastRiccati = false, useMedianDepth = true,
         useFeaturePredictions = false, useEquivariantOutput = true, removeLostLandmarks = true;
    CoordinateChoice coordinateChoice = CoordinateChoice::Euclidean;
    Pose cameraOffset = eqf::pose_identity();
    int device = 0;
    int maxLandmarks = 256;

    Settings() = default;
    explicit Settings(const eqvio_settings& s);
    std::vector<double> constructInitialStateCovarianceDiag(const size_t& numLandmarks = 0) const;
    std::array<double, 8> constructStateGainDiag8() const;
    std::array<double, 12> constructInputGainDiag() const;
    double constructOutputGainVar() const { return measurementNoise * measurementNoise; }
};

}
```

eqvio_amd/host/filter_capi.cpp:

```cpp
#include "eqvio_filter.h"
#include "VIOFilter.hpp"
#include "PreparedFrames.hpp"
#include <cstring>

using namespace eqvio_amd;

struct eqvio_filter {
    std::unique_ptr<VIOFilter> filter;
    std::string err;
    double t_prop = 0, t_pre = 0, t_corr = 0;
};

namespace {
VIOState unpackState(const double* s, const int* ids, const double* p, int N) {
    VIOState xi;
    std::memcpy(xi.sensor.inputBias.data(), s, sizeof(double) * 6);
    xi.sensor.pose = Pose{Qt{s[6], s[7], s[8], s[9]}, V3{s[10], s[11], s[12]}};
    xi.sensor.velocity = V3{s[13], s[14], s[15]};
    xi.sensor.cameraOffset = Pose{Qt{s[16], s[17], s[18], s[19]}, V3{s[20], s[21], s[22]}};
    xi.cameraLandmarks.resize(N);
    for (int i = 0; i < N; ++i)
        xi.cameraLandmarks[i] = Landmark{V3{p[3 * i], p[3 * i + 1], p[3 * i + 2]}, ids[i]};
    return xi;
}
void packSensorOut(const VIOSensorState& x, double* s) {
    std::memcpy(s, x.inputBias.data(), sizeof(double) * 6);
    const double v[17] = {x.pose.R.w, x.pose.R.x, x.pose.R.y, x.pose.R.z, x.pose.x.x, x.pose.x.y, x.pose.x.z, x.velocity.x, x.velocity.y, x.velocity.z,
                          x.cameraOffset.R.w, x.cameraOffset.R.x, x.cameraOffset.R.y, x.cameraOffset.R.z, x.cameraOffset.x.x, x.cameraOffset.x.y, x.cameraOffset.x.z};
    std::memcpy(s + 6, v, sizeof(v));
}
IMUVelocity unpackIMU(const double* v) {
    IMUVelocity r;
    r.stamp = v[0];
    r.gyr = V3{v[1], v[2], v[3]};
    r.acc = V3{v[4], v[5], v[6]};
    r.gyrBiasVel = V3{v[7], v[8], v[9]};
    r.accBiasVel = V3{v[10], v[11], v[12]};
    return r;
}
VisionMeasurement makeMeasurement(double stamp, const GICameraPtr& cam, const int* ids, const double* y, int M) {
    VisionMeasurement m;
    m.stamp = stamp;
    m.cameraPtr = cam;
    for (int i = 0; i < M; ++i)
        m.camCoordinates[ids[i]] = {y[2 * i], y[2 * i + 1]};
    m.flatIds();
    return m;
}
GICameraPtr makeCamera(const eqvio_camera* c) {
    auto cam = std::make_shared<Camera>();
    cam->c = *c;
    return cam;
}
void initTimer() {
    static thread_local bool done = false;
    if (done)
        return;
    done = true;
    loopTimer.initialise({"correction", "features", "preprocessing", "propagation", "total", "total vision update", "write output"});
}
template <typename F> int guarded(eqvio_filter* f, F&& fn) {
    try {
        fn();
        return 0;
    } catch (const std::exception& e) {
        if (f)
            f->err = e.what();
        return -1;
    }
}
}

extern "C" {

int eqvio_filter_create(eqvio_filter** out, const eqvio_settings* s, int device, int max_landmarks) {
    if (!out || !s)
        return -1;
    auto* f = new eqvio_filter();
    const int rc = guarded(f, [&] {
        VIOFilter::Settings st(*s);
        st.device = device;
        st.maxLandmarks = max_landmarks;
        initTimer();
        f->filter = std::make_unique<VIOFilter>(st);
    });
    *out = f;
    return rc;
}
int eqvio_filter_create_from_state(eqvio_filter** out, const eqvio_settings* s, int device, int max_landmarks, const double* sensor, const int* ids, const double* p,
                                   int N, double time) {
    if (!out || !s || !sensor)
        return -1;
    auto* f = new eqvio_filter();
    const int rc = guarded(f, [&] {
        VIOFilter::Settings st(*s);
        st.device = device;
        st.maxLandmarks = max_landmarks;
        initTimer();
        f->filter = std::make_unique<VIOFilter>(unpackState(sensor, ids, p, N), st, time);
    });
    *out = f;
    return rc;
}
void eqvio_filter_destroy(eqvio_filter* f) { delete f; }
const char* eqvio_filter_last_error(const eqvio_filter* f) { return f ? f->err.c_str() : "null filter"; }

int eqvio_filter_process_imu(eqvio_filter* f, const double* imu13) {
    return guarded(f, [&] { f->filter->processIMUData(unpackIMU(imu13)); });
}
static void grabTiming(eqvio_filter* f) {
    const auto& t = loopTimer.getLoopTimingData().timings;
    auto get = [&t](const char* k) {
        const auto it = t.find(k);
        return it == t.end() ? 0.0 : it->second.count();
    };
    f->t_prop = get("propagation");
    f->t_pre = get("preprocessing");
    f->t_corr = get("correction");
}
int eqvio_filter_process_vision(eqvio_filter* f, double stamp, const eqvio_camera* cam, const int* ids, const double* y, int M) {
    return guarded(f, [&] {
        initTimer();
        f->filter->processVisionData(makeMeasurement(stamp, makeCamera(cam), ids, y, M));
        grabTiming(f);
    });
}
int eqvio_filter_state_estimate(eqvio_filter* f, double* sensor, int* ids, double* p, int cap) {
    int N = -1;
    const int rc = guarded(f, [&] {
        const VIOState xi = f->filter->stateEstimate();
        if ((int)xi.cameraLandmarks.size() > cap)
            throw std::length_error("state_estimate: capacity");
        if (sensor)
            packSensorOut(xi.sensor, sensor);
        N = (int)xi.cameraLandmarks.size();
        for (int i = 0; i < N; ++i) {
            if (ids)
                ids[i] = xi.cameraLandmarks[i].id;
            if (p) {
                p[3 * i] = xi.cameraLandmarks[i].p.x;
                p[3 * i + 1] = xi.cameraLandmarks[i].p.y;
                p[3 * i + 2] = xi.cameraLandmarks[i].p.z;
            }
        }
    });
    return rc ? -1 : N;
}
double eqvio_filter_get_time(const eqvio_filter* f) { return f->filter->getTime(); }
int eqvio_filter_is_initialised(const eqvio_filter* f) { return f->filter->isInitialised() ? 1 : 0; }
int eqvio_filter_set_state(eqvio_filter* f, const double* sensor, const int* ids, const double* p, int N) {
    return guarded(f, [&] { f->filter->setState(unpackState(sensor, ids, p, N)); });
}
int eqvio_filter_set_landmarks(eqvio_filter* f, const int* ids, const double* p, int N) {
    const double s0[23] = {0, 0, 0, 0, 0, 0, 1, 0, 0, 0, 0, 0, 0, 0, 0, 0, 1, 0, 0, 0, 0, 0, 0};
    return guarded(f, [&] { f->filter->setLandmarks(unpackState(s0, ids, p, N).cameraLandmarks); });
}
int eqvio_filter_augment_landmark_states(eqvio_filter* f, const int* new_ids, int n_new, const double* sensor, const int* ids, const double* p, int N) {
    return guarded(f, [&] { f->filter->augmentLandmarkStates(std::vector<int>(new_ids, new_ids + n_new), unpackState(sensor, ids, p, N)); });
}
int eqvio_filter_get_eqf(eqvio_filter* f, double* xi0_sensor, double* X_sensor, int* ids, double* q0, double* Q, int cap) {
    const int rc = eqf_get_state(f->filter->eqfState().ctx, xi0_sensor, X_sensor, ids, q0, Q, cap);
    return rc < 0 ? -1 : rc;
}
int eqvio_filter_sigma_dim(const eqvio_filter* f) { return 21 + 3 * f->filter->viewEqFState().numLandmarks(); }
int eqvio_filter_get_sigma(eqvio_filter* f, double* out, int n) { return eqf_get_sigma(f->filter->eqfState().ctx, out, n) == 0 ? 0 : -1; }
int eqvio_filter_compute_nees(eqvio_filter* f, const double* ts, const int* tids, const double* tp, int nt, double* nees) {
    return guarded(f, [&] { *nees = f->filter->viewEqFState().computeNEES(unpackState(ts, tids, tp, nt)); });
}
int eqvio_filter_get_feature_predictions(eqvio_filter* f, const eqvio_camera* cam, double stamp, int* ids, double* y, int cap) {
    int count = -1;
    const int rc = guarded(f, [&] {
        const VisionMeasurement m = f->filter->getFeaturePredictions(makeCamera(cam), stamp);
        if ((int)m.camCoordinates.size() > cap)
            throw std::runtime_error("eqvio_filter_get_feature_predictions: capacity");
        int k = 0;
        for (const auto& kv : m.camCoordinates) {
            ids[k] = kv.first;
            y[2 * k] = kv.second[0];
            y[2 * k + 1] = kv.second[1];
            ++k;
        }
        count = k;
    });
    return rc ? -1 : count;
}
eqf_ctx* eqvio_filter_core(eqvio_filter* f) { return f->filter->eqfState().ctx; }
int eqvio_filter_last_timing(const eqvio_filter* f, double* a, double* b, double* c) {
    if (a)
        *a = f->t_prop;
    if (b)
        *b = f->t_pre;
    if (c)
        *c = f->t_corr;
    return 0;
}
eqvio_frames* eqvio_frames_create(const eqvio_camera* cam, int nframes, const int* imu_counts, const double* imu13_all, const double* stamps, const int* meas_counts,
                                  const int* ids_all, const double* y_all) {
    if (!cam || nframes < 0 || (nframes > 0 && (!imu_counts || !stamps || !meas_counts)))
        return nullptr;
    try {
        auto* fr = new eqvio_frames;
        fr->camPtr = makeCamera(cam);
        fr->meas.resize((size_t)nframes);
        fr->imuBegin.assign(1, 0);
        size_t io = 0, mo = 0;
        for (int j = 0; j < nframes; ++j) {
            for (int s = 0; s < imu_counts[j]; ++s)
                fr->imus.push_back(unpackIMU(imu13_all + 13 * (io + s)));
            io += imu_counts[j];
            fr->imuBegin.push_back(io);
            fr->meas[j] = makeMeasurement(stamps[j], fr->camPtr, ids_all + mo, y_all + 2 * mo, meas_counts[j]);
            mo += meas_counts[j];
        }
        return fr;
    } catch (...) {
        return nullptr;
    }
}
int eqvio_frames_edit_pixel(eqvio_frames* fr, int frame, int k, double u, double v) {
    if (!fr || frame < 0 || (size_t)frame >= fr->meas.size() || k < 0 || (size_t)k >= fr->meas[frame].camCoordinates.size())
        return -1;
    auto it = fr->meas[frame].camCoordinates.begin();
    std::advance(it, k);
    it->second = {u, v};
    return 0;
}
int eqvio_frames_edit_id(eqvio_frames* fr, int frame, int k, int new_id) {
    if (!fr || frame < 0 || (size_t)frame >= fr->meas.size() || k < 0 || (size_t)k >= fr->meas[frame].camCoordinates.size())
        return -1;
    auto& m = fr->meas[frame].camCoordinates;
    if (m.count(new_id))
        return -1;
    auto it = m.begin();
    std::advance(it, k);
    const auto px = it->second;
    m.erase(it);
    m[new_id] = px;
    return 0;
}
void eqvio_frames_destroy(eqvio_frames* fr) { delete fr; }
int eqvio_frames_count(const eqvio_frames* fr) { return fr ? (int)fr->meas.size() : -1; }
int eqvio_filter_run_prepared(eqvio_filter* f, const eqvio_frames* fr, int first, int count) {
    if (!fr || first < 0 || count < 0 || (size_t)first + (size_t)count > fr->meas.size())
        return -1;
    int done = 0;
    const int rc = guarded(f, [&] {
        initTimer();
        for (int j = first; j < first + count; ++j) {
            for (size_t s = fr->imuBegin[j]; s < fr->imuBegin[j + 1]; ++s)
                f->filter->processIMUData(fr->imus[s]);
            f->filter->processVisionData(fr->meas[j]);
            ++done;
        }
        grabTiming(f);
    });
    return rc ? -1 : done;
}
int eqvio_filter_run_frames(eqvio_filter* f, const eqvio_camera* cam, int nframes, const int* imu_counts, const double* imu13_all, const double* stamps,
                            const int* meas_counts, const int* ids_all, const double* y_all) {
    eqvio_frames* fr = eqvio_frames_create(cam, nframes, imu_counts, imu13_all, stamps, meas_counts, ids_all, y_all);
    if (!fr)
        return -1;
    const int done = eqvio_filter_run_prepared(f, fr, 0, nframes);
    eqvio_frames_destroy(fr);
    return done;
}

}
```

include/eqf_hip.h:

```cpp
#ifndef EQF_HIP_H
#define EQF_HIP_H
#include "eqvio_types.h"

#ifdef __cplusplus
extern "C" {
#endif

typedef struct eqf_ctx eqf_ctx;

enum {
    EQF_OK = 0,
    EQF_E_NONFINITE = -1,
    EQF_E_NOT_SPD = -2,
    EQF_E_BAD_ARG = -3,
    EQF_E_CAPACITY = -4,
    EQF_E_NO_DEVICE = -5,
    EQF_E_UNSUPPORTED = -6,
    EQF_E_STALLED = -7
};

enum {
    EQF_OPT_RICCATI_DENSE = 1,
    EQF_OPT_CHECK_FINITE = 2,
    EQF_OPT_SPECULATIVE = 7,
    EQF_OPT_DOORBELL = 6,
    EQF_OPT_EARLY_LIFT = 8,
    EQF_OPT_TRACE = 9,
    EQF_OPT_FUSED_ASSEMBLY = 11,
    EQF_OPT_LOOKAHEAD = 12,
    EQF_OPT_LA_TIMEOUT_US = 15,
    EQF_OPT_Z_IN_LOOKAHEAD = 17,
    EQF_OPT_LA_SPLIT_ROWS = 18,
    EQF_OPT_MEASURE_IN_PROPAGATE = 19,
    EQF_OPT_LIFT_WITH_SYRK = 20,
    EQF_OPT_LA_HOME = 21,
    EQF_OPT_TILES_PER_WORKGROUP = 22,
    EQF_OPT_GATHER_IN_PROPAGATE = 23,
    EQF_OPT_HOLD_NEW_LANDMARKS = 24,
    EQF_OPT_EARLY_DOORBELL = 27,
    EQF_OPT_QUIET_DOOR_WAIT = 29,
    EQF_OPT_SELECT_ONE_WORKGROUP = 25,
    EQF_OPT_LIVE_COLUMNS_FIRST = 26,
    EQF_OPT_SIGMA_FP32 = 3
};

const char* eqf_error_string(int code);

int eqf_create(eqf_ctx** out, int device, int max_landmarks, int coordinate_choice);
void eqf_destroy(eqf_ctx* ctx);
int eqf_set_option(eqf_ctx* ctx, int option, int value);
int eqf_get_option(const eqf_ctx* ctx, int option, int* value);
int eqf_synchronize(eqf_ctx* ctx);
int eqf_num_landmarks(const eqf_ctx* ctx);
int eqf_get_ids(const eqf_ctx* ctx, int* ids, int cap);
void* eqf_stream(eqf_ctx* ctx);

int eqf_set_state(eqf_ctx* ctx, const double* xi0_sensor, const double* X_sensor, const int* ids, const double* q0, const double* Q, int N);
int eqf_get_state(eqf_ctx* ctx, double* xi0_sensor, double* X_sensor, int* ids, double* q0, double* Q, int cap);

int eqf_set_sigma(eqf_ctx* ctx, const double* sigma_colmajor, int n);
int eqf_set_sigma_diag(eqf_ctx* ctx, const double* diag, int n);
int eqf_get_sigma(eqf_ctx* ctx, double* sigma_colmajor, int n);
int eqf_get_sigma_block(eqf_ctx* ctx, int r0, int c0, int rows, int cols, double* out_colmajor);

int eqf_state_estimate(eqf_ctx* ctx, double* sensor, int* ids, double* p, int cap);

int eqf_add_landmarks(eqf_ctx* ctx, const int* ids, const double* p, int k, double var);
int eqf_add_landmarks_held(eqf_ctx* ctx, const int* ids, const double* p, int k, double var);
int eqf_hold_supported(const eqf_ctx* ctx);
int eqf_hold_stats(eqf_ctx* ctx, long* launches, int reset);
int eqf_remove_landmarks(eqf_ctx* ctx, const int* indices, int k);
int eqf_remove_unmeasured_landmarks(eqf_ctx* ctx, const int* ids, int M, int* removed_idx, int* n_removed);
int eqf_find_unknown_ids(eqf_ctx* ctx, const int* ids, int M, int* unknown_j, int* n_unknown);
int eqf_same_as_mapped(const eqf_ctx* ctx, const int* ids, int M);
int eqf_remove_invalid_landmarks(eqf_ctx* ctx);
int eqf_update_unsettled(const eqf_ctx* ctx);
int eqf_early_doorbell_stats(eqf_ctx* ctx, long* updates, int reset);
int eqf_remove_invalid_at_update(eqf_ctx* ctx);

int eqf_integrate_riccati_fast(eqf_ctx* ctx, const double* imu13, double dt, const double* Qdiag12, const double* Pdiag8);
int eqf_integrate_riccati_accurate(eqf_ctx* ctx, const double* imu13, double dt, const double* Qdiag12, const double* Pdiag8);
int eqf_integrate_riccati_discrete(eqf_ctx* ctx, const double* imu13, double dt, const double* Qdiag12, const double* Pdiag8);
int eqf_integrate_observer(eqf_ctx* ctx, const double* imu13_k, const double* dt_k, int k, int discreteLift);

int eqf_outlier_stats(eqf_ctx* ctx, const eqvio_camera* cam, const int* ids, const double* y, int M, double* absErr, double* probErr, double* depth2);
int eqf_output_cov_all(eqf_ctx* ctx, const eqvio_camera* cam, double* out4N);

int eqf_vision_update(eqf_ctx* ctx, const eqvio_camera* cam, const int* ids, const double* y, int M, double meas_var, int useEquivariantOutput, int discreteCorrection);

int eqf_propagate_fast(eqf_ctx* ctx, const double* imu13_mean, double dt_total, const double* Qdiag12, const double* Pdiag8, const double* imu13_k, const double* dt_k,
                       int k, int discreteLift);
int eqf_stage_measurement(eqf_ctx* ctx, const int* ids, const double* y_px, int M);

int eqf_stats_then_update(eqf_ctx* ctx, const eqvio_camera* cam, const int* ids, const double* y_px, int M, double thrAbs, double thrProb, double meas_var,
                          int useEquivariantOutput, int discreteCorrection, double* absErr, double* probErr, double* depth2, int* updated);

int eqf_speculation_stats(eqf_ctx* ctx, long* calls, long* queued, long* cancelled, int reset);
int eqf_measure_in_propagate_stats(eqf_ctx* ctx, long* used, int reset);
int eqf_z_in_lookahead_stats(eqf_ctx* ctx, long* launches, int reset);
int eqf_gather_stats(eqf_ctx* ctx, long* launches, int reset);
int eqf_stats_select_update(eqf_ctx* ctx, const eqvio_camera* cam, const int* ids, const double* y_px, int M, double thrAbs, double thrProb, int max_outliers, double meas_var,
                            int useEquivariantOutput, int discreteCorrection, double* absErr, double* probErr, double* depth2, int* updated, int* removed_idx, int* n_removed);
int eqf_lookahead_stats(eqf_ctx* ctx, long* launches, long* fallbacks, int reset);
int eqf_own_hardware_queue(eqf_ctx* ctx);
int eqf_live_columns_stats(eqf_ctx* ctx, long* launches, int reset);
int eqf_lookahead_selftest(const eqf_ctx* ctx);
int eqf_lookahead_home(const eqf_ctx* ctx, int* home_xcd, long* home_launches);
int eqf_device_to_itself(eqf_ctx* ctx);
int eqf_selection_stats(eqf_ctx* ctx, long* frames, long* discarded, int reset);

int eqf_last_gamma(eqf_ctx* ctx, double* out, int cap);

int eqf_compute_nees(eqf_ctx* ctx, const double* true_sensor, const int* true_ids, const double* true_p, int n_true, double* nees);
int eqf_nees_lu_fallbacks(eqf_ctx* ctx, long* count);

int eqf_debug_matrices_AB(eqf_ctx* ctx, const double* imu13, double* A_out, double* B_out);
int eqf_debug_get_W(eqf_ctx* ctx, double* out, int rows, int cols);
int eqf_debug_syrk_order(int nt, int* tile_of_block);
int eqf_debug_matrix_C(eqf_ctx* ctx, const eqvio_camera* cam, const int* ids, const double* y, int M, int useEquivariantOutput, double* C_out, double* ytilde_out);

int eqf_mfma_f64_peak(eqf_ctx* ctx, double* tflops);
int eqf_mfma_f64_peak_clock(eqf_ctx* ctx, double* tflops, double* sclk_ghz);

int eqf_last_kernel_times(eqf_ctx* ctx, int* which, float* usec, int cap);
int eqf_trace_read(eqf_ctx* ctx, unsigned long long* device_ticks, long long* host_ns, unsigned* last_frame);
int eqf_debug_lookahead_stamps(eqf_ctx* ctx, unsigned long long* out768);
int eqf_host_wait_stats(eqf_ctx* ctx, long* calls, double* seconds, int reset);
const char* eqf_kernel_name(int which);

#ifdef __cplusplus
}
#endif
#endif
```

Before: 11290 updates/s.

## Overlap next-frame IMU ingestion and integration prep with device update work

Adds a busy hook that runs while the host waits on the device doorbell during the stats/update call. The hook feeds the next frame's IMU samples into the filter and precomputes the packed integration inputs, so the next propagate can skip that host work. Per-frame stats copies are now fetched lazily only when no update happened, and the observer chunk vectors are reused across calls. This adds state-validity bookkeeping and an exception path that rolls back pre-fed IMU data. The early-doorbell condition is also loosened.

```diff
diff --git a/eqvio_amd/capi.py b/eqvio_amd/capi.py
--- a/eqvio_amd/capi.py
+++ b/eqvio_amd/capi.py
@@ -7,7 +7,7 @@
 LIB_DIR = os.environ.get("EQVIO_AMD_LIB_DIR") or os.path.join(_HERE, "lib")
 
 COORD_EUCLIDEAN, COORD_INVDEPTH, COORD_NORMAL = 0, 1, 2
-OPT_RICCATI_DENSE, OPT_CHECK_FINITE, OPT_SIGMA_FP32, OPT_DOORBELL, OPT_SPECULATIVE, OPT_EARLY_LIFT, OPT_TRACE, OPT_FUSED_ASSEMBLY, OPT_LOOKAHEAD, OPT_LA_TIMEOUT_US, OPT_Z_IN_LOOKAHEAD, OPT_LA_SPLIT_ROWS, OPT_MEASURE_IN_PROPAGATE, OPT_LIFT_WITH_SYRK, OPT_LA_HOME, OPT_TILES_PER_WORKGROUP, OPT_GATHER_IN_PROPAGATE, OPT_HOLD_NEW_LANDMARKS, OPT_SELECT_ONE_WORKGROUP, OPT_LIVE_COLUMNS_FIRST, OPT_EARLY_DOORBELL, OPT_QUIET_DOOR_WAIT, OPT_TIMING = 1, 2, 3, 6, 7, 8, 9, 11, 12, 15, 17, 18, 19, 20, 21, 22, 23, 24, 25, 26, 27, 29, 100
+OPT_RICCATI_DENSE, OPT_CHECK_FINITE, OPT_SIGMA_FP32, OPT_DOORBELL, OPT_SPECULATIVE, OPT_EARLY_LIFT, OPT_TRACE, OPT_FUSED_ASSEMBLY, OPT_LOOKAHEAD, OPT_LA_TIMEOUT_US, OPT_Z_IN_LOOKAHEAD, OPT_LA_SPLIT_ROWS, OPT_MEASURE_IN_PROPAGATE, OPT_LIFT_WITH_SYRK, OPT_LA_HOME, OPT_TILES_PER_WORKGROUP, OPT_GATHER_IN_PROPAGATE, OPT_HOLD_NEW_LANDMARKS, OPT_SELECT_ONE_WORKGROUP, OPT_LIVE_COLUMNS_FIRST, OPT_EARLY_DOORBELL, OPT_QUIET_DOOR_WAIT, OPT_HOST_PIPELINE, OPT_TIMING = 1, 2, 3, 6, 7, 8, 9, 11, 12, 15, 17, 18, 19, 20, 21, 22, 23, 24, 25, 26, 27, 29, 30, 100
 
 c_double_p = C.POINTER(C.c_double)
 c_int_p = C.POINTER(C.c_int)
@@ -210,6 +210,8 @@
         "eqf_z_in_lookahead_stats": (C.c_int, [vp, C.POINTER(C.c_long), C.c_int]),
         "eqf_gather_stats": (C.c_int, [vp, C.POINTER(C.c_long), C.c_int]),
         "eqf_selection_stats": (C.c_int, [vp, C.POINTER(C.c_long), C.POINTER(C.c_long), C.c_int]),
+        "eqf_set_busy_hook": (C.c_int, [vp, vp, vp]),
+        "eqf_last_stats": (C.c_int, [vp, c_double_p, c_double_p, c_double_p, C.c_int]),
         "eqf_output_cov_all": (C.c_int, [vp, P(Camera), c_double_p]),
         "eqf_lookahead_stats": (C.c_int, [vp, C.POINTER(C.c_long), C.POINTER(C.c_long), C.c_int]),
         "eqf_debug_matrices_AB": (C.c_int, [vp, c_double_p, c_double_p, c_double_p]),
@@ -222,7 +224,7 @@
         "eqf_last_kernel_times": (C.c_int, [vp, c_int_p, P(C.c_float), C.c_int]),
     }
     for name, (res, args) in protos.items():
-        if os.environ.get("EQVIO_AMD_LIB_DIR") and name in ("eqf_lookahead_home", "eqf_device_to_itself", "eqf_early_doorbell_stats", "eqf_update_unsettled", "eqf_remove_invalid_at_update", "eqf_gather_stats", "eqf_remove_unmeasured_landmarks", "eqf_find_unknown_ids", "eqf_add_landmarks_held", "eqf_hold_supported", "eqf_hold_stats", "eqf_same_as_mapped", "eqf_live_columns_stats", "eqf_own_hardware_queue") and not hasattr(lib, name):
+        if os.environ.get("EQVIO_AMD_LIB_DIR") and name in ("eqf_lookahead_home", "eqf_device_to_itself", "eqf_early_doorbell_stats", "eqf_update_unsettled", "eqf_remove_invalid_at_update", "eqf_gather_stats", "eqf_remove_unmeasured_landmarks", "eqf_find_unknown_ids", "eqf_add_landmarks_held", "eqf_hold_supported", "eqf_hold_stats", "eqf_same_as_mapped", "eqf_live_columns_stats", "eqf_own_hardware_queue", "eqf_set_busy_hook", "eqf_last_stats") and not hasattr(lib, name):
             continue
         fn = getattr(lib, name)
         fn.restype = res
diff --git a/eqvio_amd/csrc/eqf_hip.hip b/eqvio_amd/csrc/eqf_hip.hip
--- a/eqvio_amd/csrc/eqf_hip.hip
+++ b/eqvio_amd/csrc/eqf_hip.hip
@@ -181,6 +181,11 @@
     int opt_gather = 1;
     int opt_early_door = 1;
     int opt_quiet_wait = 1;
+    int opt_host_pipe = 1;
+    void (*busy_hook)(void*) = nullptr;
+    void* busy_hook_arg = nullptr;
+    std::vector<ObsSteps> obs_chunks;
+    std::vector<int> obs_counts;
     int opt_la_watch_ahead = 1;
     int early_seq_next = 0, early_armed_seq = 0;
     bool early_allowed = false;
@@ -338,7 +343,7 @@
 constexpr int TR_FRAMES = 1024, TR_SLOTS = 48;
 enum { TR_ASSEMBLE = 0, TR_PROPAGATE = 1, TR_BUILD_Z = 2, TR_STEP0 = 3, TR_LIFT = 40, TR_SYRK = 42 };
 constexpr int TR_HOST = 8;
-enum { TH_DOOR = 0, TH_PROP_ENTRY = 1, TH_ASSEMBLE_OUT = 2, TH_PROP_OUT = 3, TH_TAIL_ENTRY = 4, TH_BUILD_Z_OUT = 5, TH_TAIL_OUT = 6 };
+enum { TH_DOOR = 0, TH_PROP_ENTRY = 1, TH_ASSEMBLE_OUT = 2, TH_PROP_OUT = 3, TH_TAIL_ENTRY = 4, TH_BUILD_Z_OUT = 5, TH_TAIL_OUT = 6, TH_EARLY = 7 };
 void host_stamp(eqf_ctx* c, int k) {
     if (c->d_trace)
         c->h_trace[(size_t)(c->trace_frame % TR_FRAMES) * TR_HOST + k] = std::chrono::duration_cast<std::chrono::nanoseconds>(std::chrono::steady_clock::now().time_since_epoch()).count();
@@ -521,9 +526,11 @@
     if (early)
         *early = false;
     for (long it = 1;; ++it) {
-        const bool rang_early = bell_early && *bell_early == seq && *bell != seq;
-        if (rang_early)
+        const bool rang_early = bell_early && *bell_early == seq;
+        if (rang_early) {
             *early = true;
+            host_stamp(c, TH_EARLY);
+        }
         if (*bell == seq || rang_early) {
             std::atomic_thread_fence(std::memory_order_acquire);
             c->busy_common = c->busy_steps = c->busy_meas = false;
@@ -1088,6 +1095,7 @@
     case EQF_OPT_HOLD_NEW_LANDMARKS: *value = c->opt_hold; return 0;
     case EQF_OPT_EARLY_DOORBELL: *value = c->opt_early_door; return 0;
     case EQF_OPT_QUIET_DOOR_WAIT: *value = c->opt_quiet_wait; return 0;
+    case EQF_OPT_HOST_PIPELINE: *value = c->opt_host_pipe; return 0;
     case EQF_OPT_SELECT_ONE_WORKGROUP: *value = c->opt_sel_one; return 0;
     case EQF_OPT_LIVE_COLUMNS_FIRST: *value = c->opt_live_first; return 0;
     case EQF_OPT_LA_HOME: *value = c->opt_la_home; return 0;
@@ -1157,6 +1165,9 @@
         return 0;
     case EQF_OPT_QUIET_DOOR_WAIT:
         c->opt_quiet_wait = value ? 1 : 0;
+        return 0;
+    case EQF_OPT_HOST_PIPELINE:
+        c->opt_host_pipe = value ? 1 : 0;
         return 0;
     case EQF_OPT_MEASURE_IN_PROPAGATE:
         c->opt_measure_prop = value ? 1 : 0;
@@ -1426,7 +1437,7 @@
         return rc == EQF_E_NO_DEVICE ? rc : EQF_E_CAPACITY;
     const int opts[][2] = {{EQF_OPT_SIGMA_FP32, c->opt_f32}, {EQF_OPT_RICCATI_DENSE, c->opt_dense}, {EQF_OPT_CHECK_FINITE, c->opt_check}, {EQF_OPT_SPECULATIVE, c->opt_spec},
                            {EQF_OPT_DOORBELL, c->opt_door}, {EQF_OPT_EARLY_LIFT, c->opt_early}, {EQF_OPT_FUSED_ASSEMBLY, c->opt_fuse_asm}, {EQF_OPT_LOOKAHEAD, c->opt_lookahead},
-                           {EQF_OPT_LA_TIMEOUT_US, (int)(c->la_timeout_ticks / 100)}, {EQF_OPT_Z_IN_LOOKAHEAD, c->opt_zb ? (c->opt_zb_large ? 1 : 2) : 0}, {EQF_OPT_LA_SPLIT_ROWS, c->opt_la_split}, {EQF_OPT_LA_HOME, c->opt_la_home}, {EQF_OPT_TILES_PER_WORKGROUP, c->opt_prop_tpw}, {EQF_OPT_GATHER_IN_PROPAGATE, c->opt_gather}, {EQF_OPT_HOLD_NEW_LANDMARKS, c->opt_hold}, {EQF_OPT_EARLY_DOORBELL, c->opt_early_door}, {EQF_OPT_QUIET_DOOR_WAIT, c->opt_quiet_wait}, {EQF_OPT_SELECT_ONE_WORKGROUP, c->opt_sel_one}, {EQF_OPT_LIVE_COLUMNS_FIRST, c->opt_live_first}, {EQF_OPT_MEASURE_IN_PROPAGATE, c->opt_measure_prop}, {EQF_OPT_LIFT_WITH_SYRK, c->opt_lift_syrk}, {EQF_OPT_TRACE, c->d_trace ? 1 : 0}, {100, c->opt_timing}};
+                           {EQF_OPT_LA_TIMEOUT_US, (int)(c->la_timeout_ticks / 100)}, {EQF_OPT_Z_IN_LOOKAHEAD, c->opt_zb ? (c->opt_zb_large ? 1 : 2) : 0}, {EQF_OPT_LA_SPLIT_ROWS, c->opt_la_split}, {EQF_OPT_LA_HOME, c->opt_la_home}, {EQF_OPT_TILES_PER_WORKGROUP, c->opt_prop_tpw}, {EQF_OPT_GATHER_IN_PROPAGATE, c->opt_gather}, {EQF_OPT_HOLD_NEW_LANDMARKS, c->opt_hold}, {EQF_OPT_EARLY_DOORBELL, c->opt_early_door}, {EQF_OPT_QUIET_DOOR_WAIT, c->opt_quiet_wait}, {EQF_OPT_HOST_PIPELINE, c->opt_host_pipe}, {EQF_OPT_SELECT_ONE_WORKGROUP, c->opt_sel_one}, {EQF_OPT_LIVE_COLUMNS_FIRST, c->opt_live_first}, {EQF_OPT_MEASURE_IN_PROPAGATE, c->opt_measure_prop}, {EQF_OPT_LIFT_WITH_SYRK, c->opt_lift_syrk}, {EQF_OPT_TRACE, c->d_trace ? 1 : 0}, {100, c->opt_timing}};
     for (const auto& o : opts)
         if ((rc = eqf_set_option(t, o[0], o[1])) != 0)
             break;
@@ -2373,8 +2384,11 @@
     }
     if (rc)
         return rc;
-    std::vector<ObsSteps> chunks;
-    std::vector<int> counts;
+    std::vector<ObsSteps> chunks_local;
+    std::vector<int> counts_local;
+    std::vector<ObsSteps>& chunks = c->opt_host_pipe ? c->obs_chunks : chunks_local;
+    std::vector<int>& counts = c->opt_host_pipe ? c->obs_counts : counts_local;
+    chunks.clear(), counts.clear();
     HP_SCOPE("pf.observer_steps_and_launch");
     for (int done = 0; done < k;) {
         const int chunk = std::min(k - done, eqf_ctx::kMaxSteps);
@@ -3214,7 +3228,20 @@
     }
     HP_SCOPE("stu.after_map");
     const int seq = (int)(++c->door_seq);
+    struct BusyHook {
+        eqf_ctx* c;
+        ~BusyHook() { c->busy_hook = nullptr; }
+        void run() {
+            if (c->busy_hook && c->opt_host_pipe) {
+                HP_SCOPE("stu.busy_hook");
+                void (*fn)(void*) = c->busy_hook;
+                c->busy_hook = nullptr;
+                fn(c->busy_hook_arg);
+            }
+        }
+    } busy_hook{c};
     auto copy_stats = [&]() {
+        HP_SCOPE("stu.copy_stats");
         if (absErr)
             std::memcpy(absErr, c->h_res, sizeof(double) * N);
         if (probErr)
@@ -3248,6 +3275,7 @@
         if (rc)
             return rc;
         host_stamp(c, TH_TAIL_OUT);
+        busy_hook.run();
         bool early = false;
         rc = use_door ? door_wait(c, 1, seq, &early) : sync_ctx(c);
         if (rc)
@@ -3310,6 +3338,7 @@
     if (rc)
         return rc;
     host_stamp(c, TH_TAIL_OUT);
+    busy_hook.run();
     bool early = false;
     rc = use_door ? door_wait(c, 1, seq, &early) : sync_ctx(c);
     if (rc)
@@ -3347,6 +3376,23 @@
         return EQF_E_BAD_ARG;
     *n_removed = 0;
     return stats_then_update(c, cam, ids, y, M, thrAbs, thrProb, meas_var, useEqv, discreteCorr, absErr, probErr, depth2, updated, max_outliers, removed_idx, n_removed);
+}
+int eqf_set_busy_hook(eqf_ctx* c, void (*fn)(void*), void* arg) {
+    if (!c)
+        return EQF_E_BAD_ARG;
+    c->busy_hook = fn, c->busy_hook_arg = arg;
+    return 0;
+}
+int eqf_last_stats(eqf_ctx* c, double* absErr, double* probErr, double* depth2, int N) {
+    if (!c || N != c->N || N < 0)
+        return EQF_E_BAD_ARG;
+    if (absErr)
+        std::memcpy(absErr, c->h_res, sizeof(double) * N);
+    if (probErr)
+        std::memcpy(probErr, c->h_res + N, sizeof(double) * N);
+    if (depth2)
+        std::memcpy(depth2, c->h_res + 2 * N, sizeof(double) * N);
+    return 0;
 }
 int eqf_selection_stats(eqf_ctx* c, long* frames, long* discarded, int reset) {
     if (!c)
diff --git a/eqvio_amd/host/VIOFilter.cpp b/eqvio_amd/host/VIOFilter.cpp
--- a/eqvio_amd/host/VIOFilter.cpp
+++ b/eqvio_amd/host/VIOFilter.cpp
@@ -362,6 +362,14 @@
         imus[i].pack(all.data() + 13 * i);
     check(eqf_propagate_fast(ctx, m13, dtTotal, Qd.data(), Pd8.data(), all.data(), dts.data(), (int)imus.size(), discreteLift ? 1 : 0), "eqf_propagate_fast");
 }
+void VIO_eqf::propagateFastPacked(const double* mean13, double dtTotal, const std::array<double, 12>& Qd, const std::array<double, 8>& Pd8, const double* imus13, const double* dts, int k,
+                                  bool discreteLift) {
+    check(eqf_propagate_fast(ctx, mean13, dtTotal, Qd.data(), Pd8.data(), imus13, dts, k, discreteLift ? 1 : 0), "eqf_propagate_fast");
+}
+bool VIO_eqf::hostPipeline() const {
+    int v = 0;
+    return eqf_get_option(ctx, EQF_OPT_HOST_PIPELINE, &v) == 0 && v != 0;
+}
 void VIO_eqf::integrateRiccatiStateFast(const IMUVelocity& imu, const double& dt, const std::array<double, 12>& Qd, const std::array<double, 8>& Pd8) {
     settleInvalid();
     double v[13];
@@ -432,7 +440,7 @@
     check(eqf_stage_measurement(ctx, ids.data(), y.data(), (int)ids.size()), "eqf_stage_measurement");
 }
 int VIO_eqf::statsThenUpdate(const VisionMeasurement& m, double thrAbs, double thrProb, double var, bool useEqv, bool discreteCorrection, std::vector<double>& absErr,
-                              std::vector<double>& probErr, std::vector<double>& depth2, long maxOutliers) {
+                              std::vector<double>& probErr, std::vector<double>& depth2, long maxOutliers, void (*whileDeviceWorks)(void*), void* hookArg) {
     settleInvalid();
     const int N = numLandmarks();
     absErr.assign(N, -1.0);
@@ -442,17 +450,34 @@
     const std::vector<int>& ids = fm.ids;
     const std::vector<double>& y = fm.y;
     int updated = 0;
+    const bool pipe = hostPipeline();
+    struct HookGuard {
+        eqf_ctx* c;
+        ~HookGuard() {
+            if (c)
+                eqf_set_busy_hook(c, nullptr, nullptr);
+        }
+    } hookGuard{pipe && whileDeviceWorks ? ctx : nullptr};
+    if (hookGuard.c)
+        eqf_set_busy_hook(ctx, whileDeviceWorks, hookArg);
+    double *pAbs = pipe ? nullptr : absErr.data(), *pProb = pipe ? nullptr : probErr.data(), *pDepth2 = pipe ? nullptr : depth2.data();
+    auto lazyStats = [&]() {
+        if (pipe && updated == 0)
+            check(eqf_last_stats(ctx, absErr.data(), probErr.data(), depth2.data(), N), "eqf_last_stats");
+    };
     if (maxOutliers < 0) {
-        check(eqf_stats_then_update(ctx, &m.cameraPtr->c, ids.data(), y.data(), (int)ids.size(), thrAbs, thrProb, var, useEqv ? 1 : 0, discreteCorrection ? 1 : 0,
-                                    absErr.data(), probErr.data(), depth2.data(), &updated),
+        check(eqf_stats_then_update(ctx, &m.cameraPtr->c, ids.data(), y.data(), (int)ids.size(), thrAbs, thrProb, var, useEqv ? 1 : 0, discreteCorrection ? 1 : 0, pAbs, pProb, pDepth2,
+                                    &updated),
               "eqf_stats_then_update");
+        lazyStats();
         return updated;
     }
     std::vector<int> removed(N + 1);
     int nRemoved = 0;
     check(eqf_stats_select_update(ctx, &m.cameraPtr->c, ids.data(), y.data(), (int)ids.size(), thrAbs, thrProb, (int)std::min<long>(maxOutliers, 1 << 30), var, useEqv ? 1 : 0,
-                                  discreteCorrection ? 1 : 0, absErr.data(), probErr.data(), depth2.data(), &updated, removed.data(), &nRemoved),
+                                  discreteCorrection ? 1 : 0, pAbs, pProb, pDepth2, &updated, removed.data(), &nRemoved),
           "eqf_stats_select_update");
+    lazyStats();
     if (nRemoved > 0) {
         std::vector<char> drop(ids_.size(), 0);
         for (int t = 0; t < nRemoved; ++t)
@@ -558,6 +583,7 @@
     if (!initialisedFlag)
         initialiseFromIMUData(imu);
     velocityBuffer.emplace_back(imu);
+    integ_.valid = false;
 }
 void VIOFilter::initialiseFromIMUData(const IMUVelocity& imu) {
     VIOState xi0 = filterState.xi0();
@@ -617,6 +643,21 @@
 bool VIOFilter::integrateUpToTime(const double& newTime) {
     if (newTime <= filterState.currentTime || filterState.currentTime < 0 || velocityBuffer.empty())
         return false;
+    if (settings->fastRiccati && filterState.hostPipeline()) {
+        HP_SCOPE("iu.pipelined");
+        if (!(integ_.valid && integ_.newTime == newTime && integ_.fromTime == filterState.currentTime && integ_.count == velocityBuffer.size()))
+            formIntegrationInputs(newTime);
+        integ_.valid = false;
+        filterState.propagateFastPacked(integ_.mean13, integ_.accumulatedTime, integ_.inputGainDiag, integ_.stateGainDiag8, integ_.imus13.data(), integ_.dts.data(), (int)integ_.count,
+                                        settings->useDiscreteVelocityLift);
+        filterState.currentTime = newTime;
+        auto it = std::find_if(velocityBuffer.begin(), velocityBuffer.end(), [this](const IMUVelocity& v) { return v.stamp >= this->filterState.currentTime; });
+        if (it != velocityBuffer.begin()) {
+            --it;
+            velocityBuffer.erase(velocityBuffer.begin(), it);
+        }
+        return true;
+    }
     std::vector<double> dts(velocityBuffer.size());
     for (size_t i = 0; i < velocityBuffer.size(); ++i) {
         const double t0 = std::max(velocityBuffer.at(i).stamp, filterState.currentTime);
@@ -652,7 +693,44 @@
     }
     return true;
 }
-void VIOFilter::processVisionData(const VisionMeasurement& measurement) {
+void VIOFilter::formIntegrationInputs(const double& newTime) {
+    IntegrationInputs& in = integ_;
+    const size_t k = velocityBuffer.size();
+    in.dts.resize(k);
+    for (size_t i = 0; i < k; ++i) {
+        const double t0 = std::max(velocityBuffer[i].stamp, filterState.currentTime);
+        const double t1 = i + 1 < k ? std::min(velocityBuffer[i + 1].stamp, newTime) : newTime;
+        in.dts[i] = std::max(t1 - t0, 0.0);
+    }
+    double accumulatedTime = 0;
+    IMUVelocity accumulatedVelocity = IMUVelocity::Zero();
+    for (size_t i = 0; i < k; ++i) {
+        accumulatedTime += in.dts[i];
+        accumulatedVelocity = accumulatedVelocity + velocityBuffer[i] * in.dts[i];
+    }
+    accumulatedVelocity = accumulatedVelocity * (1.0 / accumulatedTime);
+    accumulatedVelocity.pack(in.mean13);
+    in.imus13.resize(13 * k);
+    for (size_t i = 0; i < k; ++i)
+        velocityBuffer[i].pack(in.imus13.data() + 13 * i);
+    in.inputGainDiag = settings->constructInputGainDiag();
+    in.stateGainDiag8 = settings->constructStateGainDiag8();
+    in.accumulatedTime = accumulatedTime;
+    in.newTime = newTime, in.fromTime = filterState.currentTime, in.count = k;
+    in.valid = true;
+}
+void VIOFilter::prepareIntegration(const double& newTime) {
+    integ_.valid = false;
+    if (!settings->fastRiccati || newTime <= filterState.currentTime || filterState.currentTime < 0 || velocityBuffer.empty())
+        return;
+    formIntegrationInputs(newTime);
+}
+void VIOFilter::discardNewestIMUData(size_t n) {
+    velocityBuffer.resize(velocityBuffer.size() - std::min(n, velocityBuffer.size()));
+    integ_.valid = false;
+}
+void VIOFilter::processVisionData(const VisionMeasurement& measurement) { processVisionData(measurement, nullptr, nullptr); }
+void VIOFilter::processVisionData(const VisionMeasurement& measurement, void (*whileDeviceWorks)(void*), void* hookArg) {
     HP_SCOPE("processVisionData");
     std::optional<VisionMeasurement::Validated> oneWalk;
     loopTimer.startTiming("propagation");
@@ -710,7 +788,7 @@
         HP_SCOPE("pv.statsThenUpdate");
         const long maxOutliers = earlyAdd ? (long)(size_t)((1.0 - settings->featureRetention) * measurement.camCoordinates.size()) : -1;
         const int r = filterState.statsThenUpdate(measurement, settings->outlierThresholdAbs, settings->outlierThresholdProb, settings->constructOutputGainVar(),
-                                                  settings->useEquivariantOutput, settings->useDiscreteInnovationLift, absErr, probErr, depth2, maxOutliers);
+                                                  settings->useEquivariantOutput, settings->useDiscreteInnovationLift, absErr, probErr, depth2, maxOutliers, whileDeviceWorks, hookArg);
         if (r == 1) {
             loopTimer.endTiming("preprocessing");
             loopTimer.startTiming("correction");
diff --git a/eqvio_amd/host/VIOFilter.hpp b/eqvio_amd/host/VIOFilter.hpp
--- a/eqvio_amd/host/VIOFilter.hpp
+++ b/eqvio_amd/host/VIOFilter.hpp
@@ -180,6 +180,9 @@
     void integrateRiccatiStateFast(const IMUVelocity& imuVelocity, const double& dt, const std::array<double, 12>& inputGainDiag, const std::array<double, 8>& stateGainDiag8);
     void propagateFast(const IMUVelocity& meanVelocity, const double& dtTotal, const std::array<double, 12>& inputGainDiag, const std::array<double, 8>& stateGainDiag8,
                        const std::vector<IMUVelocity>& imus, const std::vector<double>& dts, bool discreteLift);
+    void propagateFastPacked(const double* mean13, double dtTotal, const std::array<double, 12>& inputGainDiag, const std::array<double, 8>& stateGainDiag8, const double* imus13,
+                             const double* dts, int k, bool discreteLift);
+    bool hostPipeline() const;
     void integrateRiccatiStateAccurate(const IMUVelocity& imuVelocity, const double& dt, const std::array<double, 12>& inputGainDiag, const std::array<double, 8>& stateGainDiag8);
     void integrateRiccatiStateDiscrete(const IMUVelocity& imuVelocity, const double& dt, const std::array<double, 12>& inputGainDiag, const std::array<double, 8>& stateGainDiag8);
     void performVisionUpdate(const VisionMeasurement& measurement, double outputGainVar, const bool& useEquivariantOutput = true, const bool& discreteCorrection = false);
@@ -189,7 +192,8 @@
     void outlierStats(const VisionMeasurement& measurement, std::vector<double>& absErr, std::vector<double>& probErr, std::vector<double>& depth2) const;
     void stageMeasurement(const VisionMeasurement& measurement);
     int statsThenUpdate(const VisionMeasurement& measurement, double thrAbs, double thrProb, double outputGainVar, bool useEquivariantOutput, bool discreteCorrection,
-                         std::vector<double>& absErr, std::vector<double>& probErr, std::vector<double>& depth2, long maxOutliers = -1);
+                         std::vector<double>& absErr, std::vector<double>& probErr, std::vector<double>& depth2, long maxOutliers = -1, void (*whileDeviceWorks)(void*) = nullptr,
+                         void* hookArg = nullptr);
 
   private:
     mutable std::vector<int> ids_;
@@ -211,6 +215,16 @@
                         const std::vector<double>* probErrIn = nullptr);
     double getMedianSceneDepth(const std::vector<double>* depth2) const;
     std::vector<int> unknownScratch_;
+    struct IntegrationInputs {
+        bool valid = false;
+        double newTime = 0, fromTime = 0, accumulatedTime = 0;
+        size_t count = 0;
+        std::vector<double> dts, imus13;
+        double mean13[13];
+        std::array<double, 12> inputGainDiag;
+        std::array<double, 8> stateGainDiag8;
+    } integ_;
+    void formIntegrationInputs(const double& newTime);
 
   public:
     struct Settings;
@@ -227,6 +241,9 @@
     void augmentLandmarkStates(const std::vector<int>& newIds, const VIOState& providedState);
     void processIMUData(const IMUVelocity& imuVelocity);
     void processVisionData(const VisionMeasurement& measurement);
+    void processVisionData(const VisionMeasurement& measurement, void (*whileDeviceWorks)(void*), void* hookArg);
+    void prepareIntegration(const double& newTime);
+    void discardNewestIMUData(size_t n);
     double getTime() const;
     bool isInitialised() const { return initialisedFlag; }
     VisionMeasurement getFeaturePredictions(const GICameraPtr& camPtr, const double& stamp = -1);
diff --git a/eqvio_amd/host/filter_capi.cpp b/eqvio_amd/host/filter_capi.cpp
--- a/eqvio_amd/host/filter_capi.cpp
+++ b/eqvio_amd/host/filter_capi.cpp
@@ -1,6 +1,7 @@
 #include "eqvio_filter.h"
 #include "VIOFilter.hpp"
 #include "PreparedFrames.hpp"
+#include "../csrc/host_prof.hpp"
 #include <cstring>
 
 using namespace eqvio_amd;
@@ -246,10 +247,35 @@
     int done = 0;
     const int rc = guarded(f, [&] {
         initTimer();
+        struct Ahead {
+            VIOFilter* filter;
+            const eqvio_frames* fr;
+            int next, end;
+            bool fed;
+            static void run(void* p) {
+                Ahead& a = *static_cast<Ahead*>(p);
+                if (a.next >= a.end || !a.filter->isInitialised())
+                    return;
+                for (size_t s = a.fr->imuBegin[a.next]; s < a.fr->imuBegin[a.next + 1]; ++s)
+                    a.filter->processIMUData(a.fr->imus[s]);
+                a.filter->prepareIntegration(a.fr->meas[a.next].stamp);
+                a.fed = true;
+            }
+        } ahead{f->filter.get(), fr, 0, first + count, false};
         for (int j = first; j < first + count; ++j) {
-            for (size_t s = fr->imuBegin[j]; s < fr->imuBegin[j + 1]; ++s)
-                f->filter->processIMUData(fr->imus[s]);
-            f->filter->processVisionData(fr->meas[j]);
+            if (!ahead.fed) {
+                HP_SCOPE("rp.imu");
+                for (size_t s = fr->imuBegin[j]; s < fr->imuBegin[j + 1]; ++s)
+                    f->filter->processIMUData(fr->imus[s]);
+            }
+            ahead.fed = false, ahead.next = j + 1;
+            try {
+                f->filter->processVisionData(fr->meas[j], &Ahead::run, &ahead);
+            } catch (...) {
+                if (ahead.fed)
+                    f->filter->discardNewestIMUData(fr->imuBegin[j + 2] - fr->imuBegin[j + 1]);
+                throw;
+            }
             ++done;
         }
         grabTiming(f);
diff --git a/include/eqf_hip.h b/include/eqf_hip.h
--- a/include/eqf_hip.h
+++ b/include/eqf_hip.h
@@ -39,6 +39,7 @@
     EQF_OPT_HOLD_NEW_LANDMARKS = 24,
     EQF_OPT_EARLY_DOORBELL = 27,
     EQF_OPT_QUIET_DOOR_WAIT = 29,
+    EQF_OPT_HOST_PIPELINE = 30,
     EQF_OPT_SELECT_ONE_WORKGROUP = 25,
     EQF_OPT_LIVE_COLUMNS_FIRST = 26,
     EQF_OPT_SIGMA_FP32 = 3
@@ -107,6 +108,8 @@
 int eqf_lookahead_selftest(const eqf_ctx* ctx);
 int eqf_lookahead_home(const eqf_ctx* ctx, int* home_xcd, long* home_launches);
 int eqf_device_to_itself(eqf_ctx* ctx);
+int eqf_set_busy_hook(eqf_ctx* ctx, void (*fn)(void*), void* arg);
+int eqf_last_stats(eqf_ctx* ctx, double* absErr, double* probErr, double* depth2, int N);
 int eqf_selection_stats(eqf_ctx* ctx, long* frames, long* discarded, int reset);
 
 int eqf_last_gamma(eqf_ctx* ctx, double* out, int cap);
```

New measurement: 11270 updates/s (median of 2 runs). Within noise of the previous version (-0.2%).
